# PeihaoChen/RSPNet

Measured on AMD Instinct MI355X. Metric: clips/sec pretext step (c3d 16x112x112, B=32/GPU), higher is better.
Workload: dtype f32

## Files before the change

include/rspnet_hip.h:

```cpp
#ifndef RSPNET_HIP_H
#define RSPNET_HIP_H

#include <stddef.h>
#include <stdint.h>

#ifdef __cplusplus
extern "C" {
#endif

#define RSP_OK 0
#define RSP_EINVAL (-1)
#define RSP_EWORKSPACE (-2)
#define RSP_ELAUNCH (-3)
#define RSP_EUNSUPPORTED (-4)

const char* rsp_strerror(int code);
const char* rsp_last_error(void);
const char* rsp_last_conv_kernel(void);
int rsp_version(void);

typedef struct rsp_conv3d_desc {
  int32_t N, Di, Hi, Wi, Cin;
  int32_t Do, Ho, Wo, Cout;
  int32_t kT, kH, kW;
  int32_t sT, sH, sW;
  int32_t pT, pH, pW;
  int32_t in_ld;
  int32_t out_ld;
} rsp_conv3d_desc;

size_t rsp_conv3d_packed_fwd_elems(const rsp_conv3d_desc* d);
int rsp_conv3d_pack_fwd(const rsp_conv3d_desc* d, const float* w_ref, float* w_packed, void* stream);

int32_t rsp_conv3d_stat_tiles(const rsp_conv3d_desc* d);
size_t rsp_conv3d_fwd_workspace(const rsp_conv3d_desc* d);
int rsp_conv3d_fwd(const rsp_conv3d_desc* d, const float* x, const float* w_packed, const float* bias, float* y,
                   float* stat_partials, void* workspace, size_t workspace_bytes, void* stream);

size_t rsp_conv3d_dgrad_workspace(const rsp_conv3d_desc* d);
int rsp_conv3d_dgrad(const rsp_conv3d_desc* d, const float* dy, const float* w_ref, float* dx, void* workspace,
                     size_t workspace_bytes, void* stream);

size_t rsp_conv3d_packed_dgrad_elems(const rsp_conv3d_desc* d);
int rsp_conv3d_dgrad_packed(const rsp_conv3d_desc* d, const float* dy, const float* w_packed, float* dx, void* workspace,
                            size_t workspace_bytes, void* stream);

typedef struct rsp_pack_job {
  const void* src;
  void* dst;
  int64_t total;
  int32_t kind, Cout_src, Cin_src, kT, kH, kW;
  int32_t transpose, O, C, Kld, nTd, nTh, nTw, k0d, k0h, k0w, kstepd, ksteph, kstepw, ntaps;
  int32_t blocks, reserved;
} rsp_pack_job;
int32_t rsp_conv3d_pack_jobs(const rsp_conv3d_desc* d, int32_t which, int32_t Cout_src, int32_t Cin_src, const float* w_ref,
                             float* w_packed, rsp_pack_job* jobs, int32_t max_jobs);
int rsp_pack_run(const rsp_pack_job* jobs_device, int32_t n_jobs, int32_t max_blocks, void* stream);
void rsp_conv3d_pack_forget(const void* w_packed);

size_t rsp_conv3d_wgrad_workspace(const rsp_conv3d_desc* d);
size_t rsp_conv3d_rowgeom_bytes(const rsp_conv3d_desc* d);
int rsp_conv3d_rowgeom(const rsp_conv3d_desc* d, void* table, void* stream);
int rsp_conv3d_wgrad(const rsp_conv3d_desc* d, const float* x, const float* dy, float* dw_ref, float* dbias, int32_t cout_valid,
                     int32_t cin_valid, const void* rowgeom_table, void* workspace, size_t workspace_bytes, void* stream);

const char* rsp_conv3d_kernel_name(const rsp_conv3d_desc* d, int which);

double rsp_conv3d_executed_fraction(const rsp_conv3d_desc* d, int which);

int rsp_conv3d_set_option(const char* name, int32_t value);

int rsp_fastdiv_check(int d, int n);

typedef struct rsp_bn_ema_job {
  float* running_mean;
  float* running_var;
  const float* batch_stats;
  int32_t C;
  float momentum;
} rsp_bn_ema_job;
size_t rsp_bn_finalize_workspace(int32_t tiles, int32_t C);
int rsp_bn_finalize(const float* stat_partials, int32_t tiles, int32_t C, int32_t c_valid, int32_t stat_ld, int64_t count,
                    const float* conv_bias, const float* gamma, const float* beta, float eps, float momentum, float* running_mean,
                    float* running_var, float* batch_stats_out, float* mean_invstd , float* scale_shift ,
                    void* workspace, size_t workspace_bytes, void* stream);
int rsp_bn_running_update(const rsp_bn_ema_job* jobs_device, int32_t n_jobs, int32_t max_c, void* stream);

typedef struct rsp_pool3d_desc {
  int32_t N, Di, Hi, Wi, C;
  int32_t Do, Ho, Wo;
  int32_t kT, kH, kW, sT, sH, sW, pT, pH, pW;
  int32_t in_ld, out_ld, res_ld;
} rsp_pool3d_desc;

int rsp_bn_act_pool_fwd(const rsp_pool3d_desc* d, const float* y, const float* scale_shift, const float* residual,
                        int relu, const float* gate, float* out, void* stream);

int rsp_bn_act_maxpool_applicable(const rsp_pool3d_desc* d);
int rsp_bn_act_maxpool_fwd(const rsp_pool3d_desc* d, const float* y, const float* scale_shift, int relu, const float* gate, float* out,
                           int32_t* argmax, void* stream);

size_t rsp_bn_bwd_workspace(const rsp_pool3d_desc* d);
int rsp_bn_act_pool_bwd(const rsp_pool3d_desc* d, const float* y, const float* residual, const float* dout,
                        const float* gamma, const float* mean_invstd, const float* scale_shift, int relu, float* dy,
                        float* dres, float* dgamma, float* dbeta, int32_t c_valid, const float* gate, const float* dmean,
                        void* workspace, size_t workspace_bytes, void* stream);

size_t rsp_bn_eval_bwd_workspace(const rsp_pool3d_desc* d);
int rsp_bn_eval_act_pool_bwd(const rsp_pool3d_desc* d, const float* y, const float* residual, const float* dout,
                             const float* mean_invstd, const float* scale_shift, int relu, float* dy, float* dres,
                             float* dgamma, float* dbeta, int32_t c_valid, void* workspace, size_t workspace_bytes,
                             void* stream);

int rsp_maxpool3d_fwd(const rsp_pool3d_desc* d, const float* x, float* out, int32_t* argmax, void* stream);
int rsp_maxpool3d_bwd(const rsp_pool3d_desc* d, const float* dout, const int32_t* argmax, float* dx, void* stream);

size_t rsp_gate_fwd_workspace(int32_t N, int32_t P, int32_t C);
int rsp_gate_fwd(const float* x, int32_t N, int32_t P, int32_t C, int32_t in_ld, const float* w, const float* b,
                 float* out, int32_t out_ld, float* mean, float* gate, void* workspace, size_t workspace_bytes,
                 void* stream);
int rsp_bn_gate_sums(const float* y, int32_t N, int32_t P, int32_t C, int32_t y_ld, const float* scale_shift, int relu,
                     float* act, int32_t act_ld, const float* w, const float* b, float* mean, float* gate, void* workspace,
                     size_t workspace_bytes, void* stream);
int rsp_gate_apply(const float* x, int32_t N, int32_t P, int32_t C, int32_t in_ld, const float* gate, float* out, int32_t out_ld,
                   void* stream);
int rsp_gate_bwd_params(const float* y, const float* scale_shift, int relu, const float* dout, int32_t N, int32_t P, int32_t C,
                        int32_t y_ld, int32_t dout_ld, const float* w, const float* mean, const float* gate, float* dw, float* db,
                        float* dmean, void* workspace, size_t workspace_bytes, void* stream);
size_t rsp_gate_bwd_workspace(int32_t N, int32_t P, int32_t C);
int rsp_gate_bwd(const float* x, const float* dout, int32_t N, int32_t P, int32_t C, int32_t x_ld, int32_t dout_ld,
                 const float* w, const float* mean, const float* gate, float* dx, int32_t dx_ld, float* dw, float* db,
                 void* workspace, size_t workspace_bytes, void* stream);

int rsp_head_fwd(const float* feat, int32_t B, int32_t P, int32_t C, int32_t feat_ld, const float* w1,
                 const float* b1, const float* w2, const float* b2, int32_t dim, float* out1, float* out2,
                 float* pooled, float* raw, void* stream);
size_t rsp_head_bwd_workspace(int32_t B, int32_t dim);
int rsp_head_bwd(const float* dout1, const float* dout2, const float* pooled, const float* raw, const float* w1,
                 const float* w2, int32_t B, int32_t P, int32_t C, int32_t feat_ld, int32_t dim, float* dw1,
                 float* db1, float* dw2, float* db2, float* dfeat, void* workspace, size_t workspace_bytes,
                 void* stream);

int rsp_spatial_mean_fwd(const float* x, int32_t N, int32_t P, int32_t C, int32_t ld, float* mean, void* stream);
int rsp_spatial_mean_bwd(const float* dmean, int32_t N, int32_t P, int32_t C, int32_t ld, float* dx, void* stream);
int rsp_linear_fwd(const float* x, int32_t B, int32_t Cin, const float* w, const float* bias, int32_t Cout, int relu,
                   float* y, void* stream);
size_t rsp_linear_bwd_workspace(int32_t B, int32_t Cout);
int rsp_linear_bwd(const float* x, const float* y, const float* dy, const float* w, int32_t B, int32_t Cin, int32_t Cout,
                   int relu, float* dx, float* dw, float* db, void* workspace, size_t workspace_bytes, void* stream);
int rsp_l2norm_fwd(const float* x, int32_t B, int32_t dim, float* y, void* stream);
int rsp_l2norm_bwd(const float* x, const float* dy, int32_t B, int32_t dim, float* dx, void* stream);

int rsp_logits_fwd(const float* qA, const float* qM, const float* kA, const float* kM, const float* knegA,
                   const float* knegM, const float* queue, int32_t B, int32_t dim, int32_t dim_m, int32_t K, float inv_T,
                   float* logits1, float* logits2, float* lposM, float* lnegM, void* stream);
size_t rsp_logits_bwd_workspace(int32_t B, int32_t dim, int32_t K);
int rsp_logits_bwd(const float* dlogits1, const float* dlogits2, const float* dlposM, const float* dlnegM,
                   const float* kA, const float* kM, const float* knegA, const float* knegM, const float* queue,
                   int32_t B, int32_t dim, int32_t dim_m, int32_t K, float inv_T, float* dqA, float* dqM, void* workspace,
                   size_t workspace_bytes, void* stream);

int rsp_loss_fwd_bwd(const float* logits1, const float* logits2, const float* lposM, const float* lnegM, int32_t B,
                     int32_t K1 , float margin, float A, float M, float* losses, float* dlogits1,
                     float* dlogits2, float* dlposM, float* dlnegM, float* row_scratch , void* stream);

int rsp_queue_enqueue(float* queue, int32_t dim, int32_t K, int32_t ptr, const float* keys, int32_t n, void* stream);
int rsp_queue_enqueue_dev(float* queue, int32_t dim, int32_t K, int64_t* ptr_dev, const float* keys, int32_t n, void* stream);

int rsp_clip_gather(const float* im, int32_t B_in, int32_t C, int32_t T_in, int32_t H, int32_t W, const int32_t* src,
                    const int32_t* step, int32_t B_out, int32_t T_out, int32_t C_out, float* out, void* stream);
int rsp_clip_gather_multi(int32_t n_jobs, const float* const* ims, const int32_t* const* srcs, const int32_t* const* steps,
                          float* const* outs, int32_t B_in, int32_t C, int32_t T_in, int32_t H, int32_t W, int32_t B_out, int32_t T_out,
                          int32_t C_out, void* stream);

int rsp_momentum_update(float* k, const float* q, int64_t n, float m, void* stream);

int rsp_sgd_step(float* p, const float* g, float* buf, int64_t n, float lr, float mu, float wd, float gscale,
                 int first, void* stream);

#define RSP_ELT_RELU_FWD 0
#define RSP_ELT_RELU_BWD 1
#define RSP_ELT_SIGMOID_FWD 2
#define RSP_ELT_SIGMOID_BWD 3
#define RSP_ELT_ADD 4
int rsp_eltwise(int32_t op, const float* a, const float* b , float* y, int64_t n, void* stream);

int rsp_rows_gather(const float* in, const int32_t* idx, int32_t n, int32_t width, float* out, void* stream);

#define RSP_AUG_BRIGHTNESS 0
#define RSP_AUG_CONTRAST 1
#define RSP_AUG_SATURATION 2
#define RSP_AUG_HUE 3
typedef struct rsp_augment_clip_desc {
  const uint8_t* src;
  int64_t frame_pitch;
  int32_t row_pitch;
  int32_t h, w;
  int32_t gray, flip;
  int32_t n_ops;
  int32_t op[4];
  float factor[4];
  float one_minus[4];
} rsp_augment_clip_desc;
size_t rsp_augment_workspace(int32_t n_clips, int32_t T, int32_t size);
int rsp_augment_batch(const rsp_augment_clip_desc* descs, int32_t n_clips, int32_t T, int32_t size, const float* mean3,
                      const float* std3, const float* blur9, float* out, int64_t out_clip_stride, void* workspace,
                      size_t workspace_bytes, void* stream);

int32_t rsp_cosine_topk_splits(int32_t Nq, int32_t Ng, int32_t splits);
size_t rsp_cosine_topk_workspace(int32_t Nq, int32_t Ng, int32_t D, int32_t k, int32_t splits);
int rsp_cosine_topk(const float* q, int32_t ldq, int32_t Nq, const float* g, int32_t ldg, int32_t Ng, int32_t D, int32_t k,
                    int32_t splits, int32_t* idx, float* dist, void* workspace, size_t workspace_bytes, void* stream);
int rsp_topk_hits(const int32_t* idx, int32_t Nq, int32_t k, const int64_t* y_q, const int64_t* y_g, int32_t Ng,
                  const int32_t* ks_host, int32_t nks, int32_t* counts, void* stream);

typedef struct rsp_cls_meters {
  float val[3];
  float sum[3];
  int32_t count[3];
} rsp_cls_meters;
size_t rsp_xent_metrics_workspace(int32_t rows, int32_t n_crop);
int rsp_xent_metrics(const float* logits, int32_t rows, int32_t classes, int32_t ld, int32_t n_crop, const int64_t* target,
                     int32_t valid, float* avg_logits, float* dlogits, float* loss, float* acc, rsp_cls_meters* meters,
                     void* workspace, size_t workspace_bytes, void* stream);

typedef struct rsp_pretext_meters {
  float val[8];
  float sum[8];
  int32_t count[8];
} rsp_pretext_meters;
size_t rsp_pretext_metrics_workspace(int32_t B);
int rsp_pretext_metrics(const float* logits1, const float* logits2, const float* lposM, const float* lnegM, int32_t B, int32_t K1,
                        const float* losses, float* acc, rsp_pretext_meters* meters, void* workspace, size_t workspace_bytes,
                        void* stream);

size_t rsp_cam_maps_workspace(int32_t B, int32_t C);
int rsp_cam_maps(const float* feat_q, int32_t ld_q, const float* feat_k, int32_t ld_k, const int32_t* k_row, int32_t B, int32_t P,
                 int32_t C, const float* w_qA, const float* w_qM, const float* w_kA, const float* w_kM, int32_t dim_A, int32_t dim_M,
                 float* out, void* workspace, size_t workspace_bytes, void* stream);
int rsp_cam_overlay(const float* maps, int32_t N, int32_t Tp, int32_t Hp, int32_t Wp, const float* clip_a, const float* clip_b,
                    int32_t B, int32_t T, int32_t t, int32_t size, uint8_t* out, void* stream);

#ifdef __cplusplus
}
#endif
#endif
```

rspnet_amd/_lib.py:

```python
from __future__ import annotations

import ctypes as C
import os
from typing import Optional

_HERE = os.path.dirname(os.path.abspath(__file__))
LIB_PATH = os.environ.get("RSPNET_HIP_LIB") or os.path.join(_HERE, "librspnet_hip.so")

c_f32p = C.c_void_p
c_i32p = C.c_void_p
c_stream = C.c_void_p


class ConvDesc(C.Structure):
    _fields_ = [(n, C.c_int32) for n in (
        "N", "Di", "Hi", "Wi", "Cin", "Do", "Ho", "Wo", "Cout", "kT", "kH", "kW", "sT", "sH", "sW",
        "pT", "pH", "pW", "in_ld", "out_ld")]


class PoolDesc(C.Structure):
    _fields_ = [(n, C.c_int32) for n in (
        "N", "Di", "Hi", "Wi", "C", "Do", "Ho", "Wo", "kT", "kH", "kW", "sT", "sH", "sW", "pT", "pH", "pW",
        "in_ld", "out_ld", "res_ld")]


class PackJob(C.Structure):
    _fields_ = [("src", C.c_void_p), ("dst", C.c_void_p), ("total", C.c_int64)] + [(n, C.c_int32) for n in (
        "kind", "Cout_src", "Cin_src", "kT", "kH", "kW", "transpose", "O", "C", "Kld", "nTd", "nTh", "nTw", "k0d", "k0h", "k0w",
        "kstepd", "ksteph", "kstepw", "ntaps", "blocks", "reserved")]


class BnEmaJob(C.Structure):
    _fields_ = [("running_mean", C.c_void_p), ("running_var", C.c_void_p), ("batch_stats", C.c_void_p), ("C", C.c_int32),
                ("momentum", C.c_float)]


class AugmentClipDesc(C.Structure):
    _fields_ = [("src", C.c_void_p), ("frame_pitch", C.c_int64), ("row_pitch", C.c_int32), ("h", C.c_int32), ("w", C.c_int32),
                ("gray", C.c_int32), ("flip", C.c_int32), ("n_ops", C.c_int32), ("op", C.c_int32 * 4),
                ("factor", C.c_float * 4), ("one_minus", C.c_float * 4)]


class ClsMeters(C.Structure):
    _fields_ = [("val", C.c_float * 3), ("sum", C.c_float * 3), ("count", C.c_int32 * 3)]


class PretextMeters(C.Structure):
    _fields_ = [("val", C.c_float * 8), ("sum", C.c_float * 8), ("count", C.c_int32 * 8)]


_PD = C.POINTER(ConvDesc)
_PP = C.POINTER(PoolDesc)
_sz = C.c_size_t
_i32 = C.c_int32
_i64 = C.c_int64
_f = C.c_float
_p = C.c_void_p

SIGNATURES = {
    "rsp_strerror": (C.c_char_p, [C.c_int]),
    "rsp_last_error": (C.c_char_p, []),
    "rsp_last_conv_kernel": (C.c_char_p, []),
    "rsp_version": (C.c_int, []),
    "rsp_conv3d_packed_fwd_elems": (_sz, [_PD]),
    "rsp_conv3d_pack_fwd": (C.c_int, [_PD, _p, _p, _p]),
    "rsp_conv3d_stat_tiles": (_i32, [_PD]),
    "rsp_conv3d_fwd_workspace": (_sz, [_PD]),
    "rsp_conv3d_fwd": (C.c_int, [_PD, _p, _p, _p, _p, _p, _p, _sz, _p]),
    "rsp_conv3d_dgrad_workspace": (_sz, [_PD]),
    "rsp_conv3d_dgrad": (C.c_int, [_PD, _p, _p, _p, _p, _sz, _p]),
    "rsp_conv3d_packed_dgrad_elems": (_sz, [_PD]),
    "rsp_conv3d_dgrad_packed": (C.c_int, [_PD, _p, _p, _p, _p, _sz, _p]),
    "rsp_conv3d_pack_jobs": (_i32, [_PD, _i32, _i32, _i32, _p, _p, _p, _i32]),
    "rsp_pack_run": (C.c_int, [_p, _i32, _i32, _p]),
    "rsp_conv3d_pack_forget": (None, [_p]),
    "rsp_conv3d_wgrad_workspace": (_sz, [_PD]),
    "rsp_conv3d_rowgeom_bytes": (_sz, [_PD]),
    "rsp_conv3d_rowgeom": (C.c_int, [_PD, _p, _p]),
    "rsp_conv3d_wgrad": (C.c_int, [_PD, _p, _p, _p, _p, _i32, _i32, _p, _p, _sz, _p]),
    "rsp_conv3d_kernel_name": (C.c_char_p, [_PD, C.c_int]),
    "rsp_conv3d_executed_fraction": (C.c_double, [_PD, C.c_int]),
    "rsp_conv3d_set_option": (C.c_int, [C.c_char_p, _i32]),
    "rsp_fastdiv_check": (C.c_int, [C.c_int, C.c_int]),
    "rsp_bn_finalize_workspace": (_sz, [_i32, _i32]),
    "rsp_bn_finalize": (C.c_int, [_p, _i32, _i32, _i32, _i32, _i64, _p, _p, _p, _f, _f, _p, _p, _p, _p, _p, _p, _sz, _p]),
    "rsp_bn_running_update": (C.c_int, [_p, _i32, _i32, _p]),
    "rsp_bn_act_pool_fwd": (C.c_int, [_PP, _p, _p, _p, C.c_int, _p, _p, _p]),
    "rsp_bn_act_maxpool_applicable": (C.c_int, [_PP]),
    "rsp_bn_act_maxpool_fwd": (C.c_int, [_PP, _p, _p, C.c_int, _p, _p, _p, _p]),
    "rsp_bn_bwd_workspace": (_sz, [_PP]),
    "rsp_bn_act_pool_bwd": (C.c_int, [_PP, _p, _p, _p, _p, _p, _p, C.c_int, _p, _p, _p, _p, _i32, _p, _p, _p, _sz, _p]),
    "rsp_bn_eval_bwd_workspace": (_sz, [_PP]),
    "rsp_bn_eval_act_pool_bwd": (C.c_int, [_PP, _p, _p, _p, _p, _p, C.c_int, _p, _p, _p, _p, _i32, _p, _sz, _p]),
    "rsp_maxpool3d_fwd": (C.c_int, [_PP, _p, _p, _p, _p]),
    "rsp_maxpool3d_bwd": (C.c_int, [_PP, _p, _p, _p, _p]),
    "rsp_gate_fwd_workspace": (_sz, [_i32, _i32, _i32]),
    "rsp_gate_fwd": (C.c_int, [_p, _i32, _i32, _i32, _i32, _p, _p, _p, _i32, _p, _p, _p, _sz, _p]),
    "rsp_bn_gate_sums": (C.c_int, [_p, _i32, _i32, _i32, _i32, _p, C.c_int, _p, _i32, _p, _p, _p, _p, _p, _sz, _p]),
    "rsp_gate_apply": (C.c_int, [_p, _i32, _i32, _i32, _i32, _p, _p, _i32, _p]),
    "rsp_gate_bwd_params": (C.c_int, [_p, _p, C.c_int, _p, _i32, _i32, _i32, _i32, _i32, _p, _p, _p, _p, _p, _p, _p, _sz, _p]),
    "rsp_gate_bwd_workspace": (_sz, [_i32, _i32, _i32]),
    "rsp_gate_bwd": (C.c_int, [_p, _p, _i32, _i32, _i32, _i32, _i32, _p, _p, _p, _p, _i32, _p, _p, _p, _sz, _p]),
    "rsp_head_fwd": (C.c_int, [_p, _i32, _i32, _i32, _i32, _p, _p, _p, _p, _i32, _p, _p, _p, _p, _p]),
    "rsp_head_bwd_workspace": (_sz, [_i32, _i32]),
    "rsp_head_bwd": (C.c_int, [_p, _p, _p, _p, _p, _p, _i32, _i32, _i32, _i32, _i32, _p, _p, _p, _p, _p, _p, _sz, _p]),
    "rsp_spatial_mean_fwd": (C.c_int, [_p, _i32, _i32, _i32, _i32, _p, _p]),
    "rsp_spatial_mean_bwd": (C.c_int, [_p, _i32, _i32, _i32, _i32, _p, _p]),
    "rsp_linear_fwd": (C.c_int, [_p, _i32, _i32, _p, _p, _i32, C.c_int, _p, _p]),
    "rsp_linear_bwd_workspace": (_sz, [_i32, _i32]),
    "rsp_linear_bwd": (C.c_int, [_p, _p, _p, _p, _i32, _i32, _i32, C.c_int, _p, _p, _p, _p, _sz, _p]),
    "rsp_l2norm_fwd": (C.c_int, [_p, _i32, _i32, _p, _p]),
    "rsp_l2norm_bwd": (C.c_int, [_p, _p, _i32, _i32, _p, _p]),
    "rsp_logits_fwd": (C.c_int, [_p, _p, _p, _p, _p, _p, _p, _i32, _i32, _i32, _i32, _f, _p, _p, _p, _p, _p]),
    "rsp_logits_bwd_workspace": (_sz, [_i32, _i32, _i32]),
    "rsp_logits_bwd": (C.c_int, [_p, _p, _p, _p, _p, _p, _p, _p, _p, _i32, _i32, _i32, _i32, _f, _p, _p, _p, _sz, _p]),
    "rsp_loss_fwd_bwd": (C.c_int, [_p, _p, _p, _p, _i32, _i32, _f, _f, _f, _p, _p, _p, _p, _p, _p, _p]),
    "rsp_queue_enqueue": (C.c_int, [_p, _i32, _i32, _i32, _p, _i32, _p]),
    "rsp_queue_enqueue_dev": (C.c_int, [_p, _i32, _i32, _p, _p, _i32, _p]),
    "rsp_clip_gather": (C.c_int, [_p, _i32, _i32, _i32, _i32, _i32, _p, _p, _i32, _i32, _i32, _p, _p]),
    "rsp_clip_gather_multi": (C.c_int, [_i32, _p, _p, _p, _p, _i32, _i32, _i32, _i32, _i32, _i32, _i32, _i32, _p]),
    "rsp_momentum_update": (C.c_int, [_p, _p, _i64, _f, _p]),
    "rsp_sgd_step": (C.c_int, [_p, _p, _p, _i64, _f, _f, _f, _f, C.c_int, _p]),
    "rsp_rows_gather": (C.c_int, [_p, _p, _i32, _i32, _p, _p]),
    "rsp_eltwise": (C.c_int, [_i32, _p, _p, _p, _i64, _p]),
    "rsp_augment_workspace": (_sz, [_i32, _i32, _i32]),
    "rsp_augment_batch": (C.c_int, [_p, _i32, _i32, _i32, C.POINTER(C.c_float), C.POINTER(C.c_float), C.POINTER(C.c_float), _p, _i64,
                                    _p, _sz, _p]),
    "rsp_cosine_topk_splits": (_i32, [_i32, _i32, _i32]),
    "rsp_cosine_topk_workspace": (_sz, [_i32, _i32, _i32, _i32, _i32]),
    "rsp_cosine_topk": (C.c_int, [_p, _i32, _i32, _p, _i32, _i32, _i32, _i32, _i32, _p, _p, _p, _sz, _p]),
    "rsp_topk_hits": (C.c_int, [_p, _i32, _i32, _p, _p, _i32, C.POINTER(C.c_int32), _i32, _p, _p]),
    "rsp_xent_metrics_workspace": (_sz, [_i32, _i32]),
    "rsp_xent_metrics": (C.c_int, [_p, _i32, _i32, _i32, _i32, _p, _i32, _p, _p, _p, _p, _p, _p, _sz, _p]),
    "rsp_pretext_metrics_workspace": (_sz, [_i32]),
    "rsp_pretext_metrics": (C.c_int, [_p, _p, _p, _p, _i32, _i32, _p, _p, _p, _p, _sz, _p]),
    "rsp_cam_maps_workspace": (_sz, [_i32, _i32]),
    "rsp_cam_maps": (C.c_int, [_p, _i32, _p, _i32, _p, _i32, _i32, _i32, _p, _p, _p, _p, _i32, _i32, _p, _p, _sz, _p]),
    "rsp_cam_overlay": (C.c_int, [_p, _i32, _i32, _i32, _i32, _p, _p, _i32, _i32, _i32, _i32, _p, _p]),
}

_lib: Optional[C.CDLL] = None


class RspError(RuntimeError):
    pass


def load(init_gpu: bool = False) -> C.CDLL:
    global _lib
    if init_gpu:
        _init_gpu()
    if _lib is not None:
        return _lib
    if not os.path.exists(LIB_PATH):
        raise RspError(
            f"{LIB_PATH} not found: build it with rspnet_amd/csrc/build.sh (or __graft_entry__.build()). "
            "rspnet_amd has no CPU or eager fallback.")
    try:
        import torch
    except ImportError:
        pass
    lib = C.CDLL(LIB_PATH)
    for name, (res, args) in SIGNATURES.items():
        fn = getattr(lib, name)
        fn.restype = res
        fn.argtypes = args
    _lib = lib
    return lib


_gpu_ready = False


def _init_gpu():
    global _gpu_ready
    if _gpu_ready:
        return
    import torch
    if torch.cuda.is_available():
        torch.cuda.init()
        _gpu_ready = True


def check(rc: int, what: str):
    if rc != 0:
        lib = load()
        raise RspError(f"{what} failed: {lib.rsp_strerror(rc).decode()} ({lib.rsp_last_error().decode()})")


def source_hash() -> str:
    import glob
    import hashlib
    here = os.path.dirname(os.path.abspath(__file__))
    files = sorted(glob.glob(os.path.join(here, "csrc", "*.hip")) + glob.glob(os.path.join(here, "csrc", "*.h"))
                   + glob.glob(os.path.join(os.path.dirname(here), "include", "*.h")))
    h = hashlib.sha256()
    for f in files:
        h.update(os.path.basename(f).encode())
        with open(f, "rb") as fh:
            h.update(fh.read())
    return h.hexdigest()
```

rspnet_amd/csrc/bn_pool.hip:

```cpp
#include "common.h"

namespace {

__global__ __launch_bounds__(256) void bn_finalize_stage1(const float* __restrict__ part, int tiles, int C, int ld, int S,
                                                          double* __restrict__ out) {
  __shared__ double red[4][64][2];
  const int c = blockIdx.x * 64 + (threadIdx.x & 63);
  const int rl = threadIdx.x >> 6;
  const int per = (tiles + S - 1) / S;
  const int t0 = blockIdx.y * per, t1 = min(tiles, t0 + per);
  double s = 0.0, ss = 0.0;
  if (c < C)
    for (int t = t0 + rl; t < t1; t += 4) {
      const float2 v = *reinterpret_cast<const float2*>(part + ((long long)t * ld + c) * 2);
      s += (double)v.x;
      ss += (double)v.y;
    }
  red[rl][threadIdx.x & 63][0] = s;
  red[rl][threadIdx.x & 63][1] = ss;
  __syncthreads();
  if (rl == 0 && c < C) {
    const int l = threadIdx.x;
    out[((long long)blockIdx.y * C + c) * 2 + 0] = red[0][l][0] + red[1][l][0] + red[2][l][0] + red[3][l][0];
    out[((long long)blockIdx.y * C + c) * 2 + 1] = red[0][l][1] + red[1][l][1] + red[2][l][1] + red[3][l][1];
  }
}

__global__ __launch_bounds__(1024) void bn_finalize_stage2(const double* __restrict__ part, int S, int C, int Cv, long long count,
                                                           const float* __restrict__ conv_bias, const float* __restrict__ gamma,
                                                           const float* __restrict__ beta, float eps, float momentum,
                                                           float* __restrict__ running_mean, float* __restrict__ running_var,
                                                           float* __restrict__ mean_invstd, float* __restrict__ scale_shift,
                                                           float* __restrict__ bstat) {
  __shared__ double red[16][64][2];
  const int cl = threadIdx.x & 63, rl = threadIdx.x >> 6;
  const int c = blockIdx.x * 64 + cl;
  double s = 0.0, ss = 0.0;
  if (c < C)
    for (int i = rl; i < S; i += 16) {
      s += part[((long long)i * C + c) * 2 + 0];
      ss += part[((long long)i * C + c) * 2 + 1];
    }
  red[rl][cl][0] = s;
  red[rl][cl][1] = ss;
  __syncthreads();
  if (rl != 0 || c >= C) return;
  s = 0.0;
  ss = 0.0;
#pragma unroll
  for (int i = 0; i < 16; ++i) {
    s += red[i][cl][0];
    ss += red[i][cl][1];
  }
  const double n = (double)count;
  const double mean0 = s / n;
  double var = ss / n - mean0 * mean0;
  var = var > 0.0 ? var : 0.0;
  const bool valid = c < Cv;
  const double mean = mean0 + ((conv_bias && valid) ? (double)conv_bias[c] : 0.0);
  const float invstd = (float)(1.0 / sqrt(var + (double)eps));
  mean_invstd[c] = (float)mean;
  mean_invstd[C + c] = invstd;
  const float g = valid ? (gamma ? gamma[c] : 1.f) : 0.f, b = (valid && beta) ? beta[c] : 0.f;
  const float sc = g * invstd;
  scale_shift[c] = sc;
  scale_shift[C + c] = b - (float)mean * sc;
  if (!valid) return;
  const double unbiased = count > 1 ? var * n / (n - 1.0) : var;
  if (bstat) {
    bstat[c] = (float)mean;
    bstat[Cv + c] = (float)unbiased;
    return;
  }
  if (running_mean) running_mean[c] = (1.f - momentum) * running_mean[c] + momentum * (float)mean;
  if (running_var) running_var[c] = (1.f - momentum) * running_var[c] + momentum * (float)unbiased;
}

constexpr int FIN_CH = 16, FIN_LANES = 1024 / FIN_CH;

__device__ __forceinline__ bool fin_sum_partials(const float* __restrict__ part, int n, int C, int ld, double& s, double& ss) {
  __shared__ double red[FIN_LANES][FIN_CH][2];
  const int cl = threadIdx.x & (FIN_CH - 1), rl = threadIdx.x / FIN_CH;
  const int c = blockIdx.x * FIN_CH + cl;
  s = 0.0;
  ss = 0.0;
  if (c < C)
    for (int t = rl; t < n; t += FIN_LANES) {
      const float2 v = *reinterpret_cast<const float2*>(part + ((long long)t * ld + c) * 2);
      s += (double)v.x;
      ss += (double)v.y;
    }
  red[rl][cl][0] = s;
  red[rl][cl][1] = ss;
  __syncthreads();
  if (rl < 8) {
    s = 0.0;
    ss = 0.0;
#pragma unroll
    for (int i = 0; i < FIN_LANES / 8; ++i) {
      s += red[rl * (FIN_LANES / 8) + i][cl][0];
      ss += red[rl * (FIN_LANES / 8) + i][cl][1];
    }
  }
  __syncthreads();
  if (rl < 8) {
    red[rl][cl][0] = s;
    red[rl][cl][1] = ss;
  }
  __syncthreads();
  if (rl != 0 || c >= C) return false;
  s = 0.0;
  ss = 0.0;
#pragma unroll
  for (int i = 0; i < 8; ++i) {
    s += red[i][cl][0];
    ss += red[i][cl][1];
  }
  return true;
}

__global__ __launch_bounds__(1024) void bn_finalize_one_kernel(const float* __restrict__ part, int tiles, int C, int Cv, int ld, long long count,
                                                               const float* __restrict__ conv_bias, const float* __restrict__ gamma,
                                                               const float* __restrict__ beta, float eps, float momentum,
                                                               float* __restrict__ running_mean, float* __restrict__ running_var,
                                                               float* __restrict__ mean_invstd, float* __restrict__ scale_shift,
                                                               float* __restrict__ bstat) {
  const int c = blockIdx.x * FIN_CH + (threadIdx.x & (FIN_CH - 1));
  double s, ss;
  if (!fin_sum_partials(part, tiles, C, ld, s, ss)) return;
  const double n = (double)count;
  const double mean0 = s / n;
  double var = ss / n - mean0 * mean0;
  var = var > 0.0 ? var : 0.0;
  const bool valid = c < Cv;
  const double mean = mean0 + ((conv_bias && valid) ? (double)conv_bias[c] : 0.0);
  const float invstd = (float)(1.0 / sqrt(var + (double)eps));
  mean_invstd[c] = (float)mean;
  mean_invstd[C + c] = invstd;
  const float g = valid ? (gamma ? gamma[c] : 1.f) : 0.f, b = (valid && beta) ? beta[c] : 0.f;
  const float sc = g * invstd;
  scale_shift[c] = sc;
  scale_shift[C + c] = b - (float)mean * sc;
  if (!valid) return;
  const double unbiased = count > 1 ? var * n / (n - 1.0) : var;
  if (bstat) {
    bstat[c] = (float)mean;
    bstat[Cv + c] = (float)unbiased;
    return;
  }
  if (running_mean) running_mean[c] = (1.f - momentum) * running_mean[c] + momentum * (float)mean;
  if (running_var) running_var[c] = (1.f - momentum) * running_var[c] + momentum * (float)unbiased;
}

// ... 335 lines not shown
#pragma unroll
          for (int e = 0; e < VEC; ++e) { best[e] = -INFINITY; by[e] = 0.f; }
#pragma unroll
          for (int w = 0; w < NW; ++w)
#pragma unroll
            for (int e = 0; e < VEC; ++e) {
              float z = fmaf(yv[w][e], sc[e], sh[e]);
              if (p.res) z += r[w][e];
              const float zz = p.relu ? fmaxf(z, 0.f) : z;
              if (zz > best[e]) { best[e] = zz; by[e] = yv[w][e]; }
            }
#pragma unroll
          for (int e = 0; e < VEC; ++e) {
            const float dz = (p.relu && !(best[e] > 0.f)) ? 0.f : g[e];
            s1[e] += dz;
            s2[e] = fmaf(dz, (by[e] - mean[e]) * invstd[e], s2[e]);
          }
        }
      }
      op_end = 0;
    }
    for (; op < op_end; op += stride) {
      const int q1 = fastdiv((int)op, p.dWo), ow = (int)op - q1 * d.Wo;
      const int q2 = fastdiv(q1, p.dHo), oh = q1 - q2 * d.Ho;
      const int n = fastdiv(q2, p.dDo), od = q2 - n * d.Do;
      float best[VEC], by[VEC];
#pragma unroll
      for (int e = 0; e < VEC; ++e) { best[e] = -INFINITY; by[e] = 0.f; }
      for (int kt = 0; kt < d.kT; ++kt) {
        const int id = od * d.sT - d.pT + kt;
        if ((unsigned)id >= (unsigned)d.Di) continue;
        for (int kh = 0; kh < d.kH; ++kh) {
          const int ih = oh * d.sH - d.pH + kh;
          if ((unsigned)ih >= (unsigned)d.Hi) continue;
          for (int kw = 0; kw < d.kW; ++kw) {
            const int iw = ow * d.sW - d.pW + kw;
            if ((unsigned)iw >= (unsigned)d.Wi) continue;
            const long long pos = (((long long)n * d.Di + id) * d.Hi + ih) * d.Wi + iw;
            float yv[VEC], z[VEC];
            zval<VEC>(p, pos, c, sc, sh, yv, z);
#pragma unroll
            for (int e = 0; e < VEC; ++e) {
              const float zz = p.relu ? fmaxf(z[e], 0.f) : z[e];
              if (zz > best[e]) { best[e] = zz; by[e] = yv[e]; }
            }
          }
        }
      }
      float g[VEC];
      load_vec<VEC>(p.dout + op * d.out_ld + c, g);
      if (p.gate) gated_grad<VEC>(p, n, c, g);
#pragma unroll
      for (int e = 0; e < VEC; ++e) {
        const float dz = (p.relu && !(best[e] > 0.f)) ? 0.f : g[e];
        s1[e] += dz;
        s2[e] = fmaf(dz, (by[e] - mean[e]) * invstd[e], s2[e]);
      }
    }
  }
#pragma unroll
  for (int e = 0; e < VEC; ++e) { red[t][e] = s1[e]; red[t][VEC + e] = s2[e]; }
  __syncthreads();
  if (t < cgc) {
    float a1[VEC], a2[VEC];
#pragma unroll
    for (int e = 0; e < VEC; ++e) a1[e] = a2[e] = 0.f;
    for (int l = 0; l < ppi; ++l)
#pragma unroll
      for (int e = 0; e < VEC; ++e) { a1[e] += red[l * cgc + t][e]; a2[e] += red[l * cgc + t][VEC + e]; }
    float* o = p.partial + ((long long)blockIdx.x * d.C + (cg0 + t) * VEC) * 2;
#pragma unroll
    for (int e = 0; e < VEC; ++e) { o[2 * e] = a1[e]; o[2 * e + 1] = a2[e]; }
  }
}

__global__ __launch_bounds__(1024) void bn_bwd_finalize_kernel(const float* __restrict__ partial, int nblocks, int C, int Cv,
                                                               double* __restrict__ sums, float* __restrict__ dgamma,
                                                               float* __restrict__ dbeta) {
  const int c = blockIdx.x * FIN_CH + (threadIdx.x & (FIN_CH - 1));
  double a, b;
  if (!fin_sum_partials(partial, nblocks, C, C, a, b)) return;
  sums[2 * c] = a;
  sums[2 * c + 1] = b;
  if (dbeta && c < Cv) dbeta[c] = (float)a;
  if (dgamma && c < Cv) dgamma[c] = (float)b;
}

template <int VEC>
__global__ __launch_bounds__(256) void bn_bwd_apply_kernel(const BwdParams p) {
  const rsp_pool3d_desc& d = p.d;
  const long long total = (long long)d.N * d.Di * d.Hi * d.Wi * p.cg;
  const double invn = 1.0 / (double)p.count;
  for (long long idx = blockIdx.x * 256ll + threadIdx.x; idx < total; idx += 256ll * gridDim.x) {
    const int cgi = (int)(idx % p.cg);
    long long q = idx / p.cg;
    const long long pos = q;
    const int iw = (int)(q % d.Wi); q /= d.Wi;
    const int ih = (int)(q % d.Hi); q /= d.Hi;
    const int id = (int)(q % d.Di);
    const int n = (int)(q / d.Di);
    const int c = cgi * VEC;
    float sc[VEC], sh[VEC], mean[VEC], invstd[VEC], gam[VEC];
    load_vec<VEC>(p.ss + c, sc);
    load_vec<VEC>(p.ss + d.C + c, sh);
    load_vec<VEC>(p.mi + c, mean);
    load_vec<VEC>(p.mi + d.C + c, invstd);
    load_gamma<VEC>(p, c, gam);
    float yv[VEC], z[VEC], dz[VEC];
    zval<VEC>(p, pos, c, sc, sh, yv, z);
#pragma unroll
    for (int e = 0; e < VEC; ++e) dz[e] = 0.f;
    const int od = id / d.sT, oh = ih / d.sH, ow = iw / d.sW;
    if (od < d.Do && oh < d.Ho && ow < d.Wo) {
      bool win[VEC];
      float mine[VEC];
#pragma unroll
      for (int e = 0; e < VEC; ++e) { mine[e] = p.relu ? fmaxf(z[e], 0.f) : z[e]; win[e] = true; }
      const int my = ((id - od * d.sT) * d.kH + (ih - oh * d.sH)) * d.kW + (iw - ow * d.sW);
      if (d.kT * d.kH * d.kW > 1) {
        for (int kt = 0; kt < d.kT; ++kt)
          for (int kh = 0; kh < d.kH; ++kh)
            for (int kw = 0; kw < d.kW; ++kw) {
              const int o = (kt * d.kH + kh) * d.kW + kw;
              if (o == my) continue;
              const long long pp = (((long long)n * d.Di + od * d.sT + kt) * d.Hi + oh * d.sH + kh) * d.Wi + ow * d.sW + kw;
              float y2[VEC], z2[VEC];
              zval<VEC>(p, pp, c, sc, sh, y2, z2);
#pragma unroll
              for (int e = 0; e < VEC; ++e) {
                const float v = p.relu ? fmaxf(z2[e], 0.f) : z2[e];
                if (o < my ? (v >= mine[e]) : (v > mine[e])) win[e] = false;
              }
            }
      }
      const long long op = (((long long)n * d.Do + od) * d.Ho + oh) * d.Wo + ow;
      float g[VEC];
      load_vec<VEC>(p.dout + op * d.out_ld + c, g);
#pragma unroll
      for (int e = 0; e < VEC; ++e) dz[e] = (win[e] && !(p.relu && !(mine[e] > 0.f))) ? g[e] : 0.f;
    }
    float o[VEC];
#pragma unroll
    for (int e = 0; e < VEC; ++e) {
      const float m1 = (float)(p.sums[2 * (c + e)] * invn);
      const float m2 = (float)(p.sums[2 * (c + e) + 1] * invn);
      const float xhat = (yv[e] - mean[e]) * invstd[e];
      o[e] = gam[e] * invstd[e] * (dz[e] - m1 - xhat * m2);
    }
    store_vec<VEC>(p.dy + pos * d.in_ld + c, o);
    if (p.dres) store_vec<VEC>(p.dres + pos * d.res_ld + c, dz);
  }
}

template <int VEC, int MODE>
__global__ __launch_bounds__(256) void bn_bwd_apply_win_kernel(const BwdParams p) {
  const rsp_pool3d_desc& d = p.d;
  const int t = threadIdx.x;
  const int pl = fastdiv(t, p.dcgc);
  const int cgi = blockIdx.y * 256 + (t - pl * p.cgc);
  if (pl >= p.ppi || cgi >= p.cg) return;
  const int c = cgi * VEC;
  const int nwin = d.kT * d.kH * d.kW;
  float sc[VEC], sh[VEC], mean[VEC], invstd[VEC], gam[VEC], m1[VEC], m2[VEC];
  load_vec<VEC>(p.ss + c, sc);
  load_vec<VEC>(p.ss + d.C + c, sh);
  load_vec<VEC>(p.mi + c, mean);
  load_vec<VEC>(p.mi + d.C + c, invstd);
  load_gamma<VEC>(p, c, gam);
  const double invn = 1.0 / (double)p.count;
#pragma unroll
  for (int e = 0; e < VEC; ++e) {
    m1[e] = (float)(p.sums[2 * (c + e)] * invn);
    m2[e] = (float)(p.sums[2 * (c + e) + 1] * invn);
  }
  long long o = (long long)blockIdx.x * p.ppi + pl;
  long long stride = (long long)gridDim.x * p.ppi;
  long long o_end = p.npos;
  if constexpr (MODE == 1) {
    const long long step = p.ppi;
    stride *= 4;
    o = (long long)blockIdx.x * p.ppi * 4 + pl;
    for (; o + 3 * step < p.npos; o += stride) {
      float yv[4][VEC], r[4][VEC], g[4][VEC];
#pragma unroll
      for (int u = 0; u < 4; ++u) {
        load_vec<VEC>(p.y + (o + u * step) * d.in_ld + c, yv[u]);
        if (p.res) load_vec<VEC>(p.res + (o + u * step) * d.res_ld + c, r[u]);
        load_vec<VEC>(p.dout + (o + u * step) * d.out_ld + c, g[u]);
      }
#pragma unroll
      for (int u = 0; u < 4; ++u) {
        float ov[VEC], dz[VEC];
#pragma unroll
        for (int e = 0; e < VEC; ++e) {
          float z = fmaf(yv[u][e], sc[e], sh[e]);
          if (p.res) z += r[u][e];
          dz[e] = (p.relu && !(z > 0.f)) ? 0.f : g[u][e];
          const float xhat = (yv[u][e] - mean[e]) * invstd[e];
          ov[e] = gam[e] * invstd[e] * (dz[e] - m1[e] - xhat * m2[e]);
        }
        store_vec<VEC>(p.dy + (o + u * step) * d.in_ld + c, ov);
        if (p.dres) store_vec<VEC>(p.dres + (o + u * step) * d.res_ld + c, dz);
      }
    }
    stride = step;
    o_end = min(p.npos, o + 4 * step);
  }
  if constexpr (MODE == 2 || MODE == 3) {
    {
      constexpr int NW = MODE == 2 ? 4 : 8;
      long long off[NW];
      window_offsets<NW>(d, off);
      for (; o < o_end; o += stride) {
        const int op = (int)o;
        const int q1 = fastdiv(op, p.dWo), ow = op - q1 * d.Wo;
        const int q2 = fastdiv(q1, p.dHo), oh = q1 - q2 * d.Ho;
        const int n = fastdiv(q2, p.dDo), od = q2 - n * d.Do;
        const long long base = (((long long)n * d.Di + od * d.sT) * d.Hi + oh * d.sH) * d.Wi + ow * d.sW;
        float yv[NW][VEC], r[NW][VEC], g[VEC], best[VEC];
        int bi[VEC];
#pragma unroll
        for (int w = 0; w < NW; ++w) {
          load_vec<VEC>(p.y + (base + off[w]) * d.in_ld + c, yv[w]);
          if (p.res) load_vec<VEC>(p.res + (base + off[w]) * d.res_ld + c, r[w]);
        }
        load_vec<VEC>(p.dout + o * d.out_ld + c, g);
#pragma unroll
        for (int e = 0; e < VEC; ++e) { best[e] = -INFINITY; bi[e] = 0; }
#pragma unroll
        for (int w = 0; w < NW; ++w)
#pragma unroll
          for (int e = 0; e < VEC; ++e) {
            float z = fmaf(yv[w][e], sc[e], sh[e]);
            if (p.res) z += r[w][e];
            const float v = p.relu ? fmaxf(z, 0.f) : z;
            if (v > best[e]) { best[e] = v; bi[e] = w; }
          }
#pragma unroll
        for (int w = 0; w < NW; ++w) {
          float ov[VEC], dz[VEC];
#pragma unroll
          for (int e = 0; e < VEC; ++e) {
            dz[e] = (bi[e] == w && !(p.relu && !(best[e] > 0.f))) ? g[e] : 0.f;
            const float xhat = (yv[w][e] - mean[e]) * invstd[e];
            ov[e] = gam[e] * invstd[e] * (dz[e] - m1[e] - xhat * m2[e]);
          }
          store_vec<VEC>(p.dy + (base + off[w]) * d.in_ld + c, ov);
          if (p.dres) store_vec<VEC>(p.dres + (base + off[w]) * d.res_ld + c, dz);
        }
      }
    }
    return;
  }
  for (; o < o_end; o += stride) {
    float g[VEC];
    load_vec<VEC>(p.dout + o * d.out_ld + c, g);
    if (MODE == 1 || nwin == 1) {
      if (p.gate) gated_grad<VEC>(p, fastdiv(fastdiv(fastdiv((int)o, p.dWo), p.dHo), p.dDo), c, g);
      float yv[VEC], z[VEC], ov[VEC], dz[VEC];
      zval<VEC>(p, o, c, sc, sh, yv, z);
#pragma unroll
      for (int e = 0; e < VEC; ++e) {
        dz[e] = (p.relu && !(z[e] > 0.f)) ? 0.f : g[e];
        const float xhat = (yv[e] - mean[e]) * invstd[e];
        ov[e] = gam[e] * invstd[e] * (dz[e] - m1[e] - xhat * m2[e]);
      }
      store_vec<VEC>(p.dy + o * d.in_ld + c, ov);
      if (p.dres) store_vec<VEC>(p.dres + o * d.res_ld + c, dz);
      continue;
    }
    const int op = (int)o;
    const int q1 = fastdiv(op, p.dWo), ow = op - q1 * d.Wo;
    const int q2 = fastdiv(q1, p.dHo), oh = q1 - q2 * d.Ho;
    const int n = fastdiv(q2, p.dDo), od = q2 - n * d.Do;
    const long long base = (((long long)n * d.Di + od * d.sT) * d.Hi + oh * d.sH) * d.Wi + ow * d.sW;
    float yv[8][VEC], zv[8][VEC], best[VEC];
    int bi[VEC];
#pragma unroll
    for (int e = 0; e < VEC; ++e) { best[e] = -INFINITY; bi[e] = 0; }
    int kw = 0, kh = 0, kt = 0;
#pragma unroll
    for (int wdx = 0; wdx < 8; ++wdx) {
      if (wdx < nwin) {
        const long long pos = base + ((long long)kt * d.Hi + kh) * d.Wi + kw;
        zval<VEC>(p, pos, c, sc, sh, yv[wdx], zv[wdx]);
#pragma unroll
        for (int e = 0; e < VEC; ++e) {
          const float v = p.relu ? fmaxf(zv[wdx][e], 0.f) : zv[wdx][e];
          if (v > best[e]) { best[e] = v; bi[e] = wdx; }
        }
        if (++kw == d.kW) { kw = 0; if (++kh == d.kH) { kh = 0; ++kt; } }
      }
    }
    kw = 0; kh = 0; kt = 0;
#pragma unroll
    for (int wdx = 0; wdx < 8; ++wdx) {
      if (wdx < nwin) {
        const long long pos = base + ((long long)kt * d.Hi + kh) * d.Wi + kw;
        float ov[VEC], dz[VEC];
#pragma unroll
        for (int e = 0; e < VEC; ++e) {
          dz[e] = (bi[e] == wdx && !(p.relu && !(best[e] > 0.f))) ? g[e] : 0.f;
          const float xhat = (yv[wdx][e] - mean[e]) * invstd[e];
          ov[e] = gam[e] * invstd[e] * (dz[e] - m1[e] - xhat * m2[e]);
        }
        store_vec<VEC>(p.dy + pos * d.in_ld + c, ov);
        if (p.dres) store_vec<VEC>(p.dres + pos * d.res_ld + c, dz);
        if (++kw == d.kW) { kw = 0; if (++kh == d.kH) { kh = 0; ++kt; } }
      }
    }
  }
}

struct EvalBwdParams {
  rsp_pool3d_desc d;
  const float* __restrict__ y;
  const float* __restrict__ res;
  const float* __restrict__ dout;
  const float* __restrict__ mi;
  const float* __restrict__ ss;
  float* __restrict__ partial;
  float* __restrict__ dy;
  float* __restrict__ dres;
  int relu;
  int cg;
  int Cv;
  int cgc, ppi;
  long long npos;
  int De, He, We;
  FastDiv dcgc, dW, dH, dD;
};

template <int VEC, int MODE, bool SUMS>
__global__ __launch_bounds__(256) void bn_eval_bwd_kernel(const EvalBwdParams p) {
  const rsp_pool3d_desc& d = p.d;
  const int cg0 = blockIdx.y * 256;
  const int cgc = min(p.cg - cg0, 256);
  const int t = threadIdx.x;
  const int pl = fastdiv(t, p.dcgc);
  const int cl = t - pl * p.cgc;
  const bool active = pl < p.ppi && cl < cgc;
  const int c = (cg0 + cl) * VEC;
  float s1[VEC], s2[VEC];
#pragma unroll
  for (int e = 0; e < VEC; ++e) s1[e] = s2[e] = 0.f;
  if (active) {
    float sc[VEC], sh[VEC], scd[VEC], mean[VEC], invstd[VEC];
    load_vec<VEC>(p.ss + c, sc);
    load_vec<VEC>(p.ss + d.C + c, sh);
#pragma unroll
    for (int e = 0; e < VEC; ++e) { scd[e] = c + e < p.Cv ? sc[e] : 0.f; mean[e] = 0.f; invstd[e] = 0.f; }
    if constexpr (SUMS) {
      load_vec<VEC>(p.mi + c, mean);
      load_vec<VEC>(p.mi + d.C + c, invstd);
    }
    long long o = (long long)blockIdx.x * p.ppi + pl;
    const long long stride = (long long)gridDim.x * p.ppi;
    if constexpr (MODE == 1) {
      const long long step = p.ppi;
      o = (long long)blockIdx.x * p.ppi * 4 + pl;
      for (; o + 3 * step < p.npos; o += stride * 4) {
        float yv[4][VEC], r[4][VEC], g[4][VEC];
#pragma unroll
        for (int u = 0; u < 4; ++u) {
          load_vec<VEC>(p.y + (o + u * step) * d.in_ld + c, yv[u]);
          if (p.res) load_vec<VEC>(p.res + (o + u * step) * d.res_ld + c, r[u]);
          load_vec<VEC>(p.dout + (o + u * step) * d.out_ld + c, g[u]);
        }
#pragma unroll
        for (int u = 0; u < 4; ++u) {
          float ov[VEC], dz[VEC];
#pragma unroll
          for (int e = 0; e < VEC; ++e) {
            float z = fmaf(yv[u][e], sc[e], sh[e]);
            if (p.res) z += r[u][e];
            dz[e] = (p.relu && !(z > 0.f)) ? 0.f : g[u][e];
            ov[e] = scd[e] * dz[e];
            if constexpr (SUMS) {
              s1[e] += dz[e];
              s2[e] = fmaf(dz[e], (yv[u][e] - mean[e]) * invstd[e], s2[e]);
            }
          }
          store_vec<VEC>(p.dy + (o + u * step) * d.in_ld + c, ov);
          if (p.dres) store_vec<VEC>(p.dres + (o + u * step) * d.res_ld + c, dz);
        }
      }
      for (int u = 0; u < 4 && o < p.npos; ++u, o += step) {
        float yv[VEC], z[VEC], g[VEC], ov[VEC], dz[VEC];
        load_vec<VEC>(p.y + o * d.in_ld + c, yv);
        if (p.res) load_vec<VEC>(p.res + o * d.res_ld + c, z);
        load_vec<VEC>(p.dout + o * d.out_ld + c, g);
#pragma unroll
        for (int e = 0; e < VEC; ++e) {
          const float zz = fmaf(yv[e], sc[e], sh[e]) + (p.res ? z[e] : 0.f);
          dz[e] = (p.relu && !(zz > 0.f)) ? 0.f : g[e];
          ov[e] = scd[e] * dz[e];
          if constexpr (SUMS) {
            s1[e] += dz[e];
            s2[e] = fmaf(dz[e], (yv[e] - mean[e]) * invstd[e], s2[e]);
          }
        }
        store_vec<VEC>(p.dy + o * d.in_ld + c, ov);
        if (p.dres) store_vec<VEC>(p.dres + o * d.res_ld + c, dz);
      }
    } else if constexpr (MODE == 2 || MODE == 3) {
      constexpr int NW = MODE == 2 ? 4 : 8;
      long long off[NW];
      window_offsets<NW>(d, off);
      for (; o < p.npos; o += stride) {
        const int op = (int)o;
        const int q1 = fastdiv(op, p.dW), ow = op - q1 * d.Wo;
        const int q2 = fastdiv(q1, p.dH), oh = q1 - q2 * d.Ho;
        const int n = fastdiv(q2, p.dD), od = q2 - n * d.Do;
        const long long base = (((long long)n * d.Di + od * d.sT) * d.Hi + oh * d.sH) * d.Wi + ow * d.sW;
        float yv[NW][VEC], r[NW][VEC], g[VEC], best[VEC], by[VEC];
        int bi[VEC];
#pragma unroll
        for (int w = 0; w < NW; ++w) {
          load_vec<VEC>(p.y + (base + off[w]) * d.in_ld + c, yv[w]);
          if (p.res) load_vec<VEC>(p.res + (base + off[w]) * d.res_ld + c, r[w]);
        }
        load_vec<VEC>(p.dout + o * d.out_ld + c, g);
#pragma unroll
        for (int e = 0; e < VEC; ++e) { best[e] = -INFINITY; bi[e] = 0; by[e] = 0.f; }
#pragma unroll
        for (int w = 0; w < NW; ++w)
#pragma unroll
          for (int e = 0; e < VEC; ++e) {
            float z = fmaf(yv[w][e], sc[e], sh[e]);
            if (p.res) z += r[w][e];
            const float v = p.relu ? fmaxf(z, 0.f) : z;
            if (v > best[e]) { best[e] = v; bi[e] = w; by[e] = yv[w][e]; }
          }
        float dzo[VEC];
#pragma unroll
        for (int e = 0; e < VEC; ++e) {
          dzo[e] = (p.relu && !(best[e] > 0.f)) ? 0.f : g[e];
          if constexpr (SUMS) {
            s1[e] += dzo[e];
            s2[e] = fmaf(dzo[e], (by[e] - mean[e]) * invstd[e], s2[e]);
          }
        }
#pragma unroll
        for (int w = 0; w < NW; ++w) {
          float ov[VEC], dz[VEC];
#pragma unroll
          for (int e = 0; e < VEC; ++e) {
            dz[e] = bi[e] == w ? dzo[e] : 0.f;
            ov[e] = scd[e] * dz[e];
          }
          store_vec<VEC>(p.dy + (base + off[w]) * d.in_ld + c, ov);
          if (p.dres) store_vec<VEC>(p.dres + (base + off[w]) * d.res_ld + c, dz);
        }
      }
    } else {
      for (; o < p.npos; o += stride) {
        const int op = (int)o;
        const int q1 = fastdiv(op, p.dW), ow = op - q1 * p.We;
        const int q2 = fastdiv(q1, p.dH), oh = q1 - q2 * p.He;
        const int n = fastdiv(q2, p.dD), od = q2 - n * p.De;
        const bool whole = od < d.Do && oh < d.Ho && ow < d.Wo;
        const int t0 = od * d.sT, h0 = oh * d.sH, w0 = ow * d.sW;
        const int nt = min(d.kT, d.Di - t0), nh = min(d.kH, d.Hi - h0), nw = min(d.kW, d.Wi - w0);
        float best[VEC], by[VEC], dzo[VEC];
// ... 52 lines not shown
    __syncthreads();
    if (t < cgc) {
      float a1[VEC], a2[VEC];
#pragma unroll
      for (int e = 0; e < VEC; ++e) a1[e] = a2[e] = 0.f;
      for (int l = 0; l < p.ppi; ++l)
#pragma unroll
        for (int e = 0; e < VEC; ++e) { a1[e] += red[l * p.cgc + t][e]; a2[e] += red[l * p.cgc + t][VEC + e]; }
      float* o = p.partial + ((long long)blockIdx.x * d.C + (cg0 + t) * VEC) * 2;
#pragma unroll
      for (int e = 0; e < VEC; ++e) { o[2 * e] = a1[e]; o[2 * e + 1] = a2[e]; }
    }
  }
}

__global__ __launch_bounds__(1024) void bn_eval_bwd_finalize_kernel(const float* __restrict__ partial, int nblocks, int C, int Cv,
                                                                    float* __restrict__ dgamma, float* __restrict__ dbeta) {
  const int c = blockIdx.x * FIN_CH + (threadIdx.x & (FIN_CH - 1));
  double a, b;
  if (!fin_sum_partials(partial, nblocks, C, C, a, b)) return;
  if (dbeta && c < Cv) dbeta[c] = (float)a;
  if (dgamma && c < Cv) dgamma[c] = (float)b;
}

constexpr int EVAL_BWD_MAX_BLOCKS = 4096;

bool pool_ok(const rsp_pool3d_desc* d, bool need_disjoint) {
  if (!d) return false;
  if (d->N <= 0 || d->C <= 0 || d->kT <= 0 || d->kH <= 0 || d->kW <= 0) return false;
  if (d->sT <= 0 || d->sH <= 0 || d->sW <= 0 || d->pT < 0 || d->pH < 0 || d->pW < 0) return false;
  if (d->Do != (d->Di + 2 * d->pT - d->kT) / d->sT + 1) return false;
  if (d->Ho != (d->Hi + 2 * d->pH - d->kH) / d->sH + 1) return false;
  if (d->Wo != (d->Wi + 2 * d->pW - d->kW) / d->sW + 1) return false;
  if (d->in_ld < d->C || d->out_ld < d->C) return false;
  if (need_disjoint) {
    if (d->kT != d->sT || d->kH != d->sH || d->kW != d->sW || d->pT || d->pH || d->pW) return false;
  }
  return true;
}

int bn_mode(const rsp_pool3d_desc* d, bool gated) {
  const int nwin = d->kT * d->kH * d->kW;
  const bool unit = nwin == 1 && d->sT == 1 && d->sH == 1 && d->sW == 1 && !(d->pT | d->pH | d->pW);
  if (unit) return gated ? 0 : 1;
  const bool tile = d->kT == d->sT && d->kH == d->sH && d->kW == d->sW && !(d->pT | d->pH | d->pW);
  return tile && nwin == 4 ? 2 : (tile && nwin == 8 ? 3 : 0);
}

#define RSP_BN_LAUNCH_V(K, V, mode, grid, stream, p)                                                   \
  do {                                                                                                 \
    switch (mode) {                                                                                    \
      case 1: hipLaunchKernelGGL((K<V, 1>), grid, dim3(256), 0, stream, p); break;                     \
      case 2: hipLaunchKernelGGL((K<V, 2>), grid, dim3(256), 0, stream, p); break;                     \
      case 3: hipLaunchKernelGGL((K<V, 3>), grid, dim3(256), 0, stream, p); break;                     \
      default: hipLaunchKernelGGL((K<V, 0>), grid, dim3(256), 0, stream, p); break;                    \
    }                                                                                                  \
  } while (0)
#define RSP_BN_LAUNCH(K, vec, mode, grid, stream, p)                                                   \
  do {                                                                                                 \
    if (vec) RSP_BN_LAUNCH_V(K, 4, mode, grid, stream, p);                                             \
    else RSP_BN_LAUNCH_V(K, 1, mode, grid, stream, p);                                                 \
  } while (0)

int grid_for(long long total) {
  long long b = (total + 255) / 256;
  return (int)(b > 8192 ? 8192 : (b < 1 ? 1 : b));
}

int reduce_blocks(const rsp_pool3d_desc* d, int cg) {
  const int cgc = cg < 256 ? cg : 256;
  const int ppi = 256 / cgc;
  const long long npos = (long long)d->N * d->Do * d->Ho * d->Wo;
  long long b = (npos + (long long)ppi * 8 - 1) / ((long long)ppi * 8);
  return (int)(b > 2048 ? 2048 : (b < 1 ? 1 : b));
}

}

extern "C" {

static int finalize_slices(int tiles) { return tiles >= 8192 ? 256 : (tiles >= 4096 ? 64 : (tiles >= 64 ? 16 : 1)); }

size_t rsp_bn_finalize_workspace(int32_t tiles, int32_t C) {
  const int S = finalize_slices(tiles);
  return (size_t)S * C * 2 * sizeof(double);
}

__global__ __launch_bounds__(256) void bn_ema_kernel(const rsp_bn_ema_job* __restrict__ jobs) {
  const rsp_bn_ema_job j = jobs[blockIdx.y];
  const int c = blockIdx.x * 256 + threadIdx.x;
  if (c >= j.C) return;
  j.running_mean[c] = (1.f - j.momentum) * j.running_mean[c] + j.momentum * j.batch_stats[c];
  j.running_var[c] = (1.f - j.momentum) * j.running_var[c] + j.momentum * j.batch_stats[j.C + c];
}

int rsp_bn_running_update(const rsp_bn_ema_job* jobs_device, int32_t n_jobs, int32_t max_c, void* stream) {
  RSP_REQUIRE(jobs_device && n_jobs > 0 && n_jobs <= 65535 && max_c > 0, "rsp_bn_running_update: bad argument");
  hipLaunchKernelGGL(bn_ema_kernel, dim3(rsp_cdiv(max_c, 256), n_jobs), dim3(256), 0, (hipStream_t)stream, jobs_device);
  return rsp_check_launch("bn_ema_kernel");
}

int rsp_bn_finalize(const float* stat_partials, int32_t tiles, int32_t C, int32_t c_valid, int32_t stat_ld, int64_t count,
                    const float* conv_bias, const float* gamma, const float* beta, float eps, float momentum, float* running_mean,
                    float* running_var, float* batch_stats_out, float* mean_invstd, float* scale_shift, void* workspace,
                    size_t workspace_bytes, void* stream) {
  RSP_REQUIRE(stat_partials && mean_invstd && scale_shift && workspace, "rsp_bn_finalize: null pointer");
  RSP_REQUIRE(tiles > 0 && C > 0 && count > 0 && stat_ld >= C && c_valid > 0 && c_valid <= C, "rsp_bn_finalize: bad size");
  const int S = finalize_slices(tiles);
  if (workspace_bytes < (size_t)S * C * 2 * sizeof(double)) {
    rsp_set_error("rsp_bn_finalize: workspace too small");
    return RSP_EWORKSPACE;
  }
  hipStream_t s = (hipStream_t)stream;
  if (tiles <= 2048) {
    hipLaunchKernelGGL(bn_finalize_one_kernel, dim3(rsp_cdiv(C, FIN_CH)), dim3(1024), 0, s, stat_partials, tiles, C, c_valid, stat_ld, (long long)count,
                       conv_bias, gamma, beta, eps, momentum, running_mean, running_var, mean_invstd, scale_shift, batch_stats_out);
    return rsp_check_launch("bn_finalize_one_kernel");
  }
  double* part = reinterpret_cast<double*>(workspace);
  hipLaunchKernelGGL(bn_finalize_stage1, dim3(rsp_cdiv(C, 64), S), dim3(256), 0, s, stat_partials, tiles, C, stat_ld, S, part);
  int rc = rsp_check_launch("bn_finalize_stage1");
  if (rc != RSP_OK) return rc;
  hipLaunchKernelGGL(bn_finalize_stage2, dim3(rsp_cdiv(C, 64)), dim3(1024), 0, s, part, S, C, c_valid, (long long)count, conv_bias,
                     gamma, beta, eps, momentum, running_mean, running_var, mean_invstd, scale_shift, batch_stats_out);
  return rsp_check_launch("bn_finalize_stage2");
}

int rsp_bn_act_pool_fwd(const rsp_pool3d_desc* d, const float* y, const float* scale_shift, const float* residual,
                        int relu, const float* gate, float* out, void* stream) {
  RSP_REQUIRE(pool_ok(d, false), "rsp_bn_act_pool_fwd: bad descriptor");
  RSP_REQUIRE(y && scale_shift && out, "rsp_bn_act_pool_fwd: null pointer");
  if (!residual && (d->kT != d->sT || d->kH != d->sH || d->kW != d->sW || d->pT || d->pH || d->pW) &&
      rsp_bn_act_maxpool_applicable(d) && rsp_aligned16(y) && rsp_aligned16(out) && rsp_aligned16(scale_shift) &&
      (!gate || rsp_aligned16(gate)))
    return rsp_bn_act_maxpool_fwd(d, y, scale_shift, relu, gate, out, nullptr, stream);
  PoolParams p;
  p.d = *d; p.y = y; p.ss = scale_shift; p.res = residual; p.gate = gate; p.out = out; p.relu = relu;
  const bool vec = d->C % 4 == 0 && d->in_ld % 4 == 0 && d->out_ld % 4 == 0 && rsp_aligned16(y) && rsp_aligned16(out) &&
                   rsp_aligned16(scale_shift) && (!residual || (d->res_ld % 4 == 0 && rsp_aligned16(residual))) &&
                   (!gate || rsp_aligned16(gate));
  p.cg = vec ? d->C / 4 : d->C;
  const Layout L = make_layout(d, p.cg, 4);
  RSP_REQUIRE(L.npos < (1ll << 31), "rsp_bn_act_pool_fwd: more than 2^31 - 1 output positions");
  set_layout(p, L);
  RSP_BN_LAUNCH(bn_act_pool_fwd_kernel, vec, bn_mode(d, gate != nullptr), L.grid, (hipStream_t)stream, p);
  return rsp_check_launch("bn_act_pool_fwd_kernel");
}

size_t rsp_bn_bwd_workspace(const rsp_pool3d_desc* d) {
  if (!pool_ok(d, true)) return 0;
  return rsp_align_up((size_t)2048 * d->C * 2 * sizeof(float), 256) + (size_t)d->C * 2 * sizeof(double);
}

int rsp_bn_act_pool_bwd(const rsp_pool3d_desc* d, const float* y, const float* residual, const float* dout,
                        const float* gamma, const float* mean_invstd, const float* scale_shift, int relu, float* dy,
                        float* dres, float* dgamma, float* dbeta, int32_t c_valid, const float* gate, const float* dmean,
                        void* workspace, size_t workspace_bytes, void* stream) {
  RSP_REQUIRE(pool_ok(d, true), "rsp_bn_act_pool_bwd: needs disjoint windows (kernel == stride, no padding)");
  RSP_REQUIRE(!gate || (dmean && d->kT * d->kH * d->kW == 1 && d->sT * d->sH * d->sW == 1 && !residual),
              "rsp_bn_act_pool_bwd: a gated unit has a unit window, no residual, and needs dmean");
  RSP_REQUIRE(c_valid > 0 && c_valid <= d->C, "rsp_bn_act_pool_bwd: bad valid channel count");
  RSP_REQUIRE(y && dout && mean_invstd && scale_shift && dy && workspace, "rsp_bn_act_pool_bwd: null pointer");
  if (workspace_bytes < rsp_bn_bwd_workspace(d)) {
    rsp_set_error("rsp_bn_act_pool_bwd: workspace too small");
    return RSP_EWORKSPACE;
  }
  hipStream_t s = (hipStream_t)stream;
  BwdParams p;
  memset(&p, 0, sizeof p);
  p.d = *d; p.y = y; p.res = residual; p.dout = dout; p.gamma = gamma; p.mi = mean_invstd; p.ss = scale_shift;
  p.dy = dy; p.dres = dres; p.relu = relu;
  p.Cv = c_valid;
  p.gate = gate; p.dmean = dmean;
  p.invP = 1.f / (float)((long long)d->Di * d->Hi * d->Wi);
  p.count = (long long)d->N * d->Di * d->Hi * d->Wi;
  const bool vec = d->C % 4 == 0 && d->in_ld % 4 == 0 && d->out_ld % 4 == 0 && rsp_aligned16(y) && rsp_aligned16(dout) &&
                   rsp_aligned16(dy) && rsp_aligned16(scale_shift) && rsp_aligned16(mean_invstd) &&
                   (!gamma || c_valid != d->C || rsp_aligned16(gamma)) &&
                   (!residual || (d->res_ld % 4 == 0 && rsp_aligned16(residual) && (!dres || rsp_aligned16(dres)))) &&
                   (!gate || (rsp_aligned16(gate) && rsp_aligned16(dmean)));
  p.cg = vec ? d->C / 4 : d->C;
  p.partial = reinterpret_cast<float*>(workspace);
  double* sums = reinterpret_cast<double*>(reinterpret_cast<unsigned char*>(workspace) +
                                           rsp_align_up((size_t)2048 * d->C * 2 * sizeof(float), 256));
  p.sums = sums;
  const Layout L = make_layout(d, p.cg, 4);
  RSP_REQUIRE(L.npos < (1ll << 31), "rsp_bn_act_pool_bwd: more than 2^31 - 1 output positions");
  set_layout(p, L);
  p.nblocks = reduce_blocks(d, p.cg);
  dim3 rgrid(p.nblocks, rsp_cdiv(p.cg, 256));
  const int mode = bn_mode(d, gate != nullptr);
  RSP_BN_LAUNCH(bn_bwd_reduce_kernel, vec, mode, rgrid, s, p);
  int rc = rsp_check_launch("bn_bwd_reduce_kernel");
  if (rc != RSP_OK) return rc;
  hipLaunchKernelGGL(bn_bwd_finalize_kernel, dim3(rsp_cdiv(d->C, FIN_CH)), dim3(1024), 0, s, p.partial, p.nblocks, d->C, c_valid, sums,
                     dgamma, dbeta);
  rc = rsp_check_launch("bn_bwd_finalize_kernel");
  if (rc != RSP_OK) return rc;
  const bool exact = d->Di % d->sT == 0 && d->Hi % d->sH == 0 && d->Wi % d->sW == 0 && d->kT * d->kH * d->kW <= 8;
  if (exact) {
    RSP_BN_LAUNCH(bn_bwd_apply_win_kernel, vec, mode, L.grid, s, p);
    return rsp_check_launch("bn_bwd_apply_win_kernel");
  }
  const long long total = (long long)d->N * d->Di * d->Hi * d->Wi * p.cg;
  if (vec) hipLaunchKernelGGL(bn_bwd_apply_kernel<4>, dim3(grid_for(total)), dim3(256), 0, s, p);
  else hipLaunchKernelGGL(bn_bwd_apply_kernel<1>, dim3(grid_for(total)), dim3(256), 0, s, p);
  return rsp_check_launch("bn_bwd_apply_kernel");
}

static int eval_bwd_mode(const rsp_pool3d_desc* d) {
  const int m = bn_mode(d, false);
  if (m == 1) return 1;
  const bool exact = d->Di % d->sT == 0 && d->Hi % d->sH == 0 && d->Wi % d->sW == 0;
  return exact ? m : 0;
}

static long long eval_bwd_npos(const rsp_pool3d_desc* d, int mode) {
  if (mode != 0) return (long long)d->N * d->Do * d->Ho * d->Wo;
  return (long long)d->N * rsp_cdiv(d->Di, d->sT) * rsp_cdiv(d->Hi, d->sH) * rsp_cdiv(d->Wi, d->sW);
}

size_t rsp_bn_eval_bwd_workspace(const rsp_pool3d_desc* d) {
  if (!pool_ok(d, true)) return 0;
  const long long npos = eval_bwd_npos(d, eval_bwd_mode(d));
  const long long rows = npos < EVAL_BWD_MAX_BLOCKS ? npos : EVAL_BWD_MAX_BLOCKS;
  return (size_t)rows * d->C * 2 * sizeof(float);
}

#define RSP_BN_EVAL_LAUNCH_S(V, M, grid, stream, p)                                                                       \
  do {                                                                                                                    \
    if (sums) hipLaunchKernelGGL((bn_eval_bwd_kernel<V, M, true>), grid, dim3(256), 0, stream, p);                        \
    else hipLaunchKernelGGL((bn_eval_bwd_kernel<V, M, false>), grid, dim3(256), 0, stream, p);                            \
  } while (0)
#define RSP_BN_EVAL_LAUNCH_V(V, mode, grid, stream, p)                                                                    \
  do {                                                                                                                    \
    switch (mode) {                                                                                                       \
      case 1: RSP_BN_EVAL_LAUNCH_S(V, 1, grid, stream, p); break;                                                         \
      case 2: RSP_BN_EVAL_LAUNCH_S(V, 2, grid, stream, p); break;                                                         \
      case 3: RSP_BN_EVAL_LAUNCH_S(V, 3, grid, stream, p); break;                                                         \
      default: RSP_BN_EVAL_LAUNCH_S(V, 0, grid, stream, p); break;                                                        \
    }                                                                                                                     \
  } while (0)

int rsp_bn_eval_act_pool_bwd(const rsp_pool3d_desc* d, const float* y, const float* residual, const float* dout,
                             const float* mean_invstd, const float* scale_shift, int relu, float* dy, float* dres,
                             float* dgamma, float* dbeta, int32_t c_valid, void* workspace, size_t workspace_bytes,
                             void* stream) {
  RSP_REQUIRE(pool_ok(d, true), "rsp_bn_eval_act_pool_bwd: needs disjoint windows (kernel == stride, no padding)");
  RSP_REQUIRE(c_valid > 0 && c_valid <= d->C, "rsp_bn_eval_act_pool_bwd: bad valid channel count");
  RSP_REQUIRE(y && dout && scale_shift && dy, "rsp_bn_eval_act_pool_bwd: null pointer");
  RSP_REQUIRE(!dres || residual, "rsp_bn_eval_act_pool_bwd: dres without a residual");
  RSP_REQUIRE(d->res_ld >= d->C || !residual, "rsp_bn_eval_act_pool_bwd: bad residual pitch");
  const bool sums = dgamma || dbeta;
  RSP_REQUIRE(!sums || (mean_invstd && workspace), "rsp_bn_eval_act_pool_bwd: parameter gradients need mean_invstd and a workspace");
  if (sums && workspace_bytes < rsp_bn_eval_bwd_workspace(d)) {
    rsp_set_error("rsp_bn_eval_act_pool_bwd: workspace too small");
    return RSP_EWORKSPACE;
  }
  hipStream_t s = (hipStream_t)stream;
  EvalBwdParams p;
  memset(&p, 0, sizeof p);
  p.d = *d; p.y = y; p.res = residual; p.dout = dout; p.mi = mean_invstd; p.ss = scale_shift;
  p.partial = sums ? reinterpret_cast<float*>(workspace) : nullptr;
  p.dy = dy; p.dres = dres; p.relu = relu; p.Cv = c_valid;
  const bool vec = d->C % 4 == 0 && d->in_ld % 4 == 0 && d->out_ld % 4 == 0 && rsp_aligned16(y) && rsp_aligned16(dout) &&
                   rsp_aligned16(dy) && rsp_aligned16(scale_shift) && (!sums || rsp_aligned16(mean_invstd)) &&
                   (!residual || (d->res_ld % 4 == 0 && rsp_aligned16(residual) && (!dres || rsp_aligned16(dres))));
  p.cg = vec ? d->C / 4 : d->C;
  const int mode = eval_bwd_mode(d);
  p.npos = eval_bwd_npos(d, mode);
  RSP_REQUIRE(p.npos < (1ll << 31), "rsp_bn_eval_act_pool_bwd: more than 2^31 - 1 positions");
  p.cgc = p.cg < 256 ? p.cg : 256;
  p.ppi = 256 / p.cgc;
  p.dcgc = fastdiv_make(p.cgc);
  p.De = rsp_cdiv(d->Di, d->sT); p.He = rsp_cdiv(d->Hi, d->sH); p.We = rsp_cdiv(d->Wi, d->sW);
  if (mode == 0) { p.dW = fastdiv_make(p.We); p.dH = fastdiv_make(p.He); p.dD = fastdiv_make(p.De); }
  else { p.dW = fastdiv_make(d->Wo); p.dH = fastdiv_make(d->Ho); p.dD = fastdiv_make(d->Do); }
  long long b = (p.npos + (long long)p.ppi * 16 - 1) / ((long long)p.ppi * 16);
  b = b > EVAL_BWD_MAX_BLOCKS ? EVAL_BWD_MAX_BLOCKS : (b < 1 ? 1 : b);
  const dim3 grid((unsigned)b, (unsigned)rsp_cdiv(p.cg, 256));
  if (vec) RSP_BN_EVAL_LAUNCH_V(4, mode, grid, s, p);
  else RSP_BN_EVAL_LAUNCH_V(1, mode, grid, s, p);
  int rc = rsp_check_launch("bn_eval_bwd_kernel");
  if (rc != RSP_OK || !sums) return rc;
  hipLaunchKernelGGL(bn_eval_bwd_finalize_kernel, dim3(rsp_cdiv(d->C, FIN_CH)), dim3(1024), 0, s, p.partial, (int)b, d->C, c_valid,
                     dgamma, dbeta);
  return rsp_check_launch("bn_eval_bwd_finalize_kernel");
}

}
```

rspnet_amd/csrc/common.h:

```cpp
#pragma once
#include <hip/hip_runtime.h>
#include <stdint.h>
#include <stdio.h>
#include <stdlib.h>
#include <string.h>
#include <tuple>

#include "rspnet_hip.h"

typedef float floatx16 __attribute__((ext_vector_type(16)));
typedef float floatx4 __attribute__((ext_vector_type(4)));

#define RSP_WAVE 64

void rsp_set_error(const char* msg);
void rsp_note_reset(void);
void rsp_note_kernel(const char* fmt, ...);

static inline int rsp_check_launch(const char* what) {
  hipError_t e = hipGetLastError();
  if (e != hipSuccess) {
    char buf[256];
    snprintf(buf, sizeof buf, "%.*s: %s", (int)strcspn(what, "<"), what, hipGetErrorString(e));
    rsp_set_error(buf);
    return RSP_ELAUNCH;
  }
  return RSP_OK;
}

#define RSP_CONV_OPTIONS(X)                                                             \
  X(OPT_NARROW_MAX_TILES, "narrow_max_tiles", "RSP_NARROW_MAX_TILES", 0, 512)           \
  X(OPT_NARROW32_MAX_UNITS, "narrow32_max_units", "RSP_NARROW32_MAX_UNITS", 0, 256)     \
  X(OPT_TALL_MIN_TILES, "tall_min_tiles", "RSP_TALL_MIN_TILES", 0, 0)                   \
  X(OPT_TWO_LEVEL_MIN_CHUNKS, "two_level_min_chunks", "RSP_TWO_LEVEL_MIN_CHUNKS", 0, 0) \
  X(OPT_DIRECT_MAX_TILES, "direct_max_tiles", "RSP_DIRECT_MAX_TILES", 0, 0)             \
  X(OPT_NO_PERSIST, "no_persist", "RSP_NO_PERSIST", 1, 0)                               \
  X(OPT_NO_HALF_BLOCK, "no_half_block", "RSP_NO_HALF_BLOCK", 1, 0)                      \
  X(OPT_NO_PAD_SKIP, "no_pad_skip", "RSP_NO_PAD_SKIP", 1, 0)                            \
  X(OPT_NO_DMAJOR, "no_dmajor", "RSP_NO_DMAJOR", 1, 0)                                  \
  X(OPT_NO_TM_SKIP, "no_tm_skip", "RSP_NO_TM_SKIP", 1, 0)                               \
  X(OPT_NO_MULTI_SPLIT, "no_multi_split", "RSP_NO_MULTI_SPLIT", 1, 0)
#define RSP_OPTION_ID(id, name, env, flag, dflt) id,
enum RspConvOption { RSP_CONV_OPTIONS(RSP_OPTION_ID) RSP_OPT_COUNT };
#undef RSP_OPTION_ID
int rsp_conv_option(RspConvOption id);

template <auto KERNEL, class... Args, class... Note>
int rsp_launch_lds(dim3 grid, size_t lds, size_t lds_max, hipStream_t s, const std::tuple<Args...>& args, const char* fmt, Note... note) {
  static bool attr_set = false;
  if (!attr_set) {
    (void)hipFuncSetAttribute(reinterpret_cast<const void*>(KERNEL), hipFuncAttributeMaxDynamicSharedMemorySize, (int)lds_max);
    attr_set = true;
  }
  rsp_note_kernel(fmt, note...);
  std::apply([&](const auto&... a) { hipLaunchKernelGGL(KERNEL, grid, dim3(256), lds, s, a...); }, args);
  return rsp_check_launch(fmt);
}

#define RSP_REQUIRE(cond, msg)     \
  do {                             \
    if (!(cond)) {                 \
      rsp_set_error(msg);          \
      return RSP_EINVAL;           \
    }                              \
  } while (0)

static inline size_t rsp_align_up(size_t v, size_t a) { return (v + a - 1) / a * a; }
static inline int rsp_cdiv(int64_t a, int64_t b) { return (int)((a + b - 1) / b); }
static inline bool rsp_aligned16(const void* p) { return (((uintptr_t)p) & 15) == 0; }

__device__ __forceinline__ int rsp_xcd_remap(int bid, int nwg) {
  const int q = nwg >> 3, r = nwg & 7;
  const int xcd = bid & 7;
  const int base = xcd < r ? xcd * (q + 1) : r * (q + 1) + (xcd - r) * q;
  return base + (bid >> 3);
}

__device__ __forceinline__ float rsp_wave_sum(float v) {
#pragma unroll
  for (int o = 32; o > 0; o >>= 1) v += __shfl_xor(v, o);
  return v;
}
__device__ __forceinline__ double rsp_wave_sum_d(double v) {
#pragma unroll
  for (int o = 32; o > 0; o >>= 1) v += __shfl_xor(v, o);
  return v;
}
__device__ __forceinline__ float rsp_wave_max(float v) {
#pragma unroll
  for (int o = 32; o > 0; o >>= 1) v = fmaxf(v, __shfl_xor(v, o));
  return v;
}

struct FastDiv {
  unsigned mul;
  unsigned shr;
  int d;
};

static inline FastDiv fastdiv_make(int d) {
  FastDiv f = {0u, 0u, d};
  if (d <= 1) return f;
  int s = 0;
  while ((1ll << s) < d) ++s;
  const unsigned long long pw = 1ull << (31 + s);
  f.mul = (unsigned)((pw + (unsigned long long)d - 1) / (unsigned long long)d);
  f.shr = (unsigned)(s - 1);
  return f;
}

__device__ __forceinline__ int fastdiv(int n, const FastDiv f) {
  return f.mul ? (int)(__umulhi((unsigned)n, f.mul) >> f.shr) : n;
}
```

rspnet_amd/csrc/conv_stem.h:

```cpp
#pragma once
#include "common.h"

bool rsp_conv_desc_ok(const rsp_conv3d_desc* d);
bool rsp_stem_applicable(const rsp_conv3d_desc* d);
int rsp_stem_tiles(const rsp_conv3d_desc* d);
size_t rsp_stem_packed_elems(const rsp_conv3d_desc* d);
int rsp_stem_pack(const rsp_conv3d_desc* d, const float* w_ref, float* w_packed, hipStream_t s);
int rsp_stem_fwd(const rsp_conv3d_desc* d, const float* x, const float* w_packed, const float* bias, float* y,
                 float* stat_partials, hipStream_t s);
const char* rsp_stem_kernel_name(const rsp_conv3d_desc* d);
void rsp_stem_note_packed(const void* w_packed, bool three_channels);
void rsp_stem_forget_packed(const void* w_packed);
const char* rsp_wgrad_kernel_name(const rsp_conv3d_desc* d);
double rsp_wgrad_executed_fraction(const rsp_conv3d_desc* d);
```

rspnet_amd/csrc/conv_wgrad.hip:

```cpp
#include "common.h"
#include "conv_stem.h"

namespace {

constexpr int RK = 32;
constexpr int MAX_TAPS = 343;

__device__ __attribute__((aligned(64))) float g_wzero[16];

struct WgradParams {
  const float* __restrict__ x;
  const float* __restrict__ dy;
  float* __restrict__ partial;
  int M, Gd, Gh, Gw;
  int Di, Hi, Wi, in_ld, Cin;
  int sD, sH, sW;
  int kT, kH, kW, pT, pH, pW;
  int dy_ld, Cout;
  int K, Kld;
  int rows_per_split, splitm;
  int co_tiles, k_tiles;
  const float* __restrict__ zero;
  unsigned x_bytes, dy_bytes;
  const uint2* __restrict__ rowgeom;
// ... 386 lines not shown
  const int r16 = lane & 15, g16 = lane >> 4;

  const int nchunk = (row_end - row_begin + RK - 1) / RK;
  const int khw = p.kH * p.kW;
  const int kt_lo = (k0 / p.Cin) / khw, kt_hi = ((min(k0 + BN, p.K) - 1) / p.Cin) / khw;
  auto frame_live = [&](int q) {
    const int g = q - fastdiv(q, p.dGd) * p.Gd;
    const int lo = g * p.sD - p.pT + kt_lo, hi = g * p.sD - p.pT + kt_hi;
    return hi >= 0 && lo < p.Di;
  };
  auto next_live = [&](int c) {
    if (!p.skip_pad) return c < nchunk ? c : nchunk;
    for (; c < nchunk; ++c) {
      const int r0 = row_begin + c * RK, r1 = min(r0 + RK, row_end) - 1;
      const int q0 = fastdiv(r0, p.dP), q1 = fastdiv(r1, p.dP);
      if (q1 - q0 > 1 || frame_live(q0) || frame_live(q1)) break;
    }
    return c;
  };
  int buf = 0;
  auto chunk = [&](int slot_next, int slot_fetch, int c_fetch, int c_issue, bool more, auto beside) {
    if (more) read_rowtab(slot_next);
    const float* a = At + buf * RK * BM + wm * WM + TM * l32;
    const float* b = Bt + buf * RK * BN + wn * WN + TN * l32;
    typename FragVec<TM>::type af[RK / 2];
    typename FragVec<TN>::type bf[RK / 2];
    float a16[RK / 4], b16[2][RK / 4];
    if (H16) {
      const float* ah = At + buf * RK * BM + r16;
      const float* bh = Bt + buf * RK * BN + wn * WN + r16;
#pragma unroll
      for (int s4 = 0; s4 < RK / 4; ++s4) {
        a16[s4] = ah[(4 * s4 + g16) * BM];
        b16[0][s4] = bh[(4 * s4 + g16) * BN];
        b16[1][s4] = bh[(4 * s4 + g16) * BN + 16];
      }
    } else {
#pragma unroll
      for (int s2 = 0; s2 < RK / 2; ++s2) {
        af[s2] = *reinterpret_cast<const typename FragVec<TM>::type*>(a + (2 * s2 + h) * BM);
        bf[s2] = *reinterpret_cast<const typename FragVec<TN>::type*>(b + (2 * s2 + h) * BN);
      }
    }
    fetch_rows(c_fetch, slot_fetch);
    if (more) issue(c_issue, buf ^ 1);
    beside();
    if (H16) {
#pragma unroll
      for (int s4 = 0; s4 < RK / 4; ++s4)
#pragma unroll
        for (int j = 0; j < 2; ++j) acc16[j] = __builtin_amdgcn_mfma_f32_16x16x4f32(a16[s4], b16[j][s4], acc16[j], 0, 0, 0);
    } else {
#pragma unroll
      for (int s2 = 0; s2 < RK / 2; ++s2)
#pragma unroll
        for (int i = 0; i < TM; ++i)
#pragma unroll
          for (int j = 0; j < TN; ++j)
            acc[i][j] = __builtin_amdgcn_mfma_f32_32x32x2f32(FragVec<TM>::get(af[s2], i), FragVec<TN>::get(bf[s2], j), acc[i][j], 0, 0, 0);
    }
    __builtin_amdgcn_sched_barrier(0);
    __syncthreads();
    buf ^= 1;
  };
  if (!p.skip_pad) {
    fetch_rows(0, 0);
    fetch_rows(1, 1);
    __syncthreads();
    if (nchunk > 0) {
      read_rowtab(0);
      issue(0, 0);
    }
    __syncthreads();
    for (int c = 0; c < nchunk; ++c) chunk((c + 1) % 3, (c + 2) % 3, c + 2, c + 1, c + 1 < nchunk, [] {});
  } else {
    int c0 = next_live(0);
    int c1 = next_live(c0 + 1);
    int c2 = next_live(c1 + 1);
    fetch_rows(c0, 0);
    fetch_rows(c1, 1);
    __syncthreads();
    if (c0 < nchunk) {
      read_rowtab(0);
      issue(c0, 0);
    }
    __syncthreads();
    int slot = 0;
    for (int c3 = 0; c0 < nchunk; c0 = c1, c1 = c2, c2 = c3, slot = slot == 2 ? 0 : slot + 1)
      chunk(slot == 2 ? 0 : slot + 1, slot == 0 ? 2 : slot - 1, c2, c1, c1 < nchunk, [&] { c3 = next_live(c2 + 1); });
  }

  float* dst = p.partial + (long long)z * p.Cout * p.Kld;
  if (H16) {
#pragma unroll
    for (int j = 0; j < 2; ++j) {
      const int kc = k0 + wn * WN + 16 * j + r16;
#pragma unroll
      for (int r = 0; r < 4; ++r) {
        const int co = co0 + 4 * g16 + r;
        if (kc < p.Kld && co < p.Cout) dst[(long long)co * p.Kld + kc] = acc16[j][r];
      }
    }
    return;
  }
  const int k = k0 + wn * WN + TN * l32;
  if (k < p.Kld) {
#pragma unroll
    for (int i = 0; i < TM; ++i)
#pragma unroll
      for (int e = 0; e < 16; ++e) {
        const int co = co0 + wm * WM + TM * ((e >> 2) * 8 + h * 4 + (e & 3)) + i;
        if (co < p.Cout) {
          typename FragVec<TN>::type v;
#pragma unroll
          for (int j = 0; j < TN; ++j) FragVec<TN>::set(v, j, acc[i][j][e]);
          *reinterpret_cast<typename FragVec<TN>::type*>(dst + (long long)co * p.Kld + k) = v;
        }
      }
  }
}

template <int BM, int BN, int WAVES_M, int WAVES_N>
__global__ __launch_bounds__(256, 2) void wgrad_dma_kernel(const WgradParams p) {
  wgrad_dma_body<BM, BN, WAVES_M, WAVES_N, false>(p);
}
__global__ __launch_bounds__(256, 2) void wgrad_dma_h16_kernel(const WgradParams p) { wgrad_dma_body<32, 128, 1, 4, true>(p); }

__global__ __launch_bounds__(256) void wgrad_reduce_kernel(const float* __restrict__ partial, float* __restrict__ dw,
                                                           int splitm, int Cout, int Cin, int taps, int Kld, int Cin_v) {
  extern __shared__ float wr_tile[];
  const int cit = Cin < 32 ? Cin : 32;
  const int ci0 = blockIdx.x * cit, co = blockIdx.y;
  const int nci = min(cit, Cin_v - ci0);
  if (nci <= 0) return;
  const long long slab = (long long)Cout * Kld;
  const float* base = partial + (long long)co * Kld;
  for (int e = threadIdx.x; e < nci * taps; e += 256) {
    const int tap = e / nci, cil = e - tap * nci;
    const float* src = base + tap * Cin + ci0 + cil;
    float s0 = 0.f, s1 = 0.f, s2 = 0.f, s3 = 0.f;
    int z = 0;
    for (; z + 4 <= splitm; z += 4) {
      s0 += src[(long long)z * slab];
      s1 += src[(long long)(z + 1) * slab];
      s2 += src[(long long)(z + 2) * slab];
      s3 += src[(long long)(z + 3) * slab];
    }
    for (; z < splitm; ++z) s0 += src[(long long)z * slab];
    wr_tile[cil * taps + tap] = (s0 + s1) + (s2 + s3);
  }
  __syncthreads();
  float* out = dw + ((long long)co * Cin_v + ci0) * taps;
  for (int e = threadIdx.x; e < nci * taps; e += 256) out[e] = wr_tile[e];
}

__global__ __launch_bounds__(256) void colsum_stage1(const float* __restrict__ a, long long rows, int C, int ld,
                                                     float* __restrict__ part, int rows_per_block) {
  __shared__ float red[4][64];
  const int c = blockIdx.y * 64 + (threadIdx.x & 63);
  const int rl = threadIdx.x >> 6;
  const long long r0 = (long long)blockIdx.x * rows_per_block;
  const long long r1 = r0 + rows_per_block < rows ? r0 + rows_per_block : rows;
  float s = 0.f;
  if (c < C)
    for (long long r = r0 + rl; r < r1; r += 4) s += a[r * ld + c];
  red[rl][threadIdx.x & 63] = s;
  __syncthreads();
  if (rl == 0 && c < C) part[(long long)blockIdx.x * C + c] = red[0][threadIdx.x] + red[1][threadIdx.x] + red[2][threadIdx.x] + red[3][threadIdx.x];
}
__global__ void colsum_stage2(const float* __restrict__ part, int nblk, int C, float* __restrict__ out) {
  const int c = blockIdx.x * blockDim.x + threadIdx.x;
  if (c >= C) return;
  double s = 0.0;
  for (int b = 0; b < nblk; ++b) s += (double)part[(long long)b * C + c];
  out[c] = (float)s;
}

constexpr size_t wgrad_lds(int bm, int bn, bool dma) { return (size_t)2 * RK * (bm + bn) * sizeof(float) + (dma ? 3 * RK * sizeof(uint2) : 0); }
inline dim3 wgrad_grid(const WgradParams& p) { return dim3((unsigned)(p.co_tiles * p.k_tiles) * (unsigned)p.splitm); }

template <int BM, int BN, int WAVES_M, int WAVES_N, bool VECA, bool VECB>
int launch_w(const WgradParams& p, hipStream_t s) {
  constexpr size_t lds = wgrad_lds(BM, BN, false);
  return rsp_launch_lds<&wgrad_kernel<BM, BN, WAVES_M, WAVES_N, VECA, VECB>>(wgrad_grid(p), lds, lds, s, std::tie(p),
                                                                             "wgrad_kernel<%d, %d, %d, %d, *>", BM, BN, WAVES_M, WAVES_N);
}

template <int BM, int BN, int WAVES_M, int WAVES_N>
int launch_w_dma(const WgradParams& p, hipStream_t s) {
  constexpr size_t lds = wgrad_lds(BM, BN, true);
  return rsp_launch_lds<&wgrad_dma_kernel<BM, BN, WAVES_M, WAVES_N>>(wgrad_grid(p), lds, lds, s, std::tie(p),
                                                                     "wgrad_dma_kernel<%d, %d, %d, %d>", BM, BN, WAVES_M, WAVES_N);
}

int launch_w_dma_h16(const WgradParams& p, hipStream_t s) {
  rsp_note_kernel("wgrad_dma_h16_kernel");
  hipLaunchKernelGGL(wgrad_dma_h16_kernel, wgrad_grid(p), dim3(256), wgrad_lds(32, 128, true), s, p);
  return rsp_check_launch("wgrad_dma_h16_kernel");
}

static bool wgrad_h16(int cout) { return !rsp_conv_option(OPT_NO_HALF_BLOCK) && cout <= 16; }

template <int BM, int BN, int WAVES_M, int WAVES_N>
int launch_w_vec(const WgradParams& p, bool va, bool vb, hipStream_t s) {
  if (va && vb) return launch_w<BM, BN, WAVES_M, WAVES_N, true, true>(p, s);
  if (va) return launch_w<BM, BN, WAVES_M, WAVES_N, true, false>(p, s);
  if (vb) return launch_w<BM, BN, WAVES_M, WAVES_N, false, true>(p, s);
  return launch_w<BM, BN, WAVES_M, WAVES_N, false, false>(p, s);
}

bool wdesc_ok(const rsp_conv3d_desc* d) { return rsp_conv_desc_ok(d); }

struct WPlan {
  int bm, bn, co_tiles, k_tiles, splitm, rows_per_split, Kld;
  size_t partial_bytes, colsum_bytes, rowgeom_bytes;
  bool dma;
  bool h16;
};

WPlan wplan(const rsp_conv3d_desc* d) {
  WPlan w;
  const long long M = (long long)d->N * d->Do * d->Ho * d->Wo;
  const int K = d->kT * d->kH * d->kW * d->Cin;
  w.Kld = (int)rsp_align_up((size_t)K, 4);
  w.bm = d->Cout > 64 ? 128 : (d->Cout > 32 ? 64 : 32);
  w.bn = K > 64 ? 128 : 64;
  if (w.bm == 32 && w.bn == 64) w.bm = 64;
  w.co_tiles = rsp_cdiv(d->Cout, w.bm);
  w.k_tiles = rsp_cdiv(K, w.bn);
  const int tiles = w.co_tiles * w.k_tiles;
  const long long max_sp = M / 256 > 0 ? M / 256 : 1;
  long long sp = 1;
  {
    const long long lds = 2ll * RK * (w.bm + w.bn) * 4 + 1024;
    const long long slots = 256 * (160 * 1024 / lds > 4 ? 4 : 160 * 1024 / lds);
    double best = -1.0;
    for (long long c = 1; c <= max_sp && c * tiles <= 8192; ++c) {
      const long long units = c * tiles, rounds = (units + slots - 1) / slots;
      const double score = (double)units / (double)(rounds * slots) - 0.004 * (double)rounds;
      if (score > best) {
        best = score;
        sp = c;
      }
    }
    if (sp > max_sp) sp = max_sp;
  }
  long long rps = (M + sp - 1) / sp;
  rps = (rps + RK - 1) / RK * RK;
  w.rows_per_split = (int)rps;
  w.splitm = (int)((M + rps - 1) / rps);
  w.partial_bytes = rsp_align_up((size_t)w.splitm * d->Cout * w.Kld * sizeof(float), 256);
  w.colsum_bytes = rsp_align_up((size_t)rsp_cdiv(M, 1024) * d->Cout * sizeof(float), 256);
  w.rowgeom_bytes = rsp_align_up((size_t)M * sizeof(uint2), 256);
  w.dma = d->Cout % 4 == 0 && d->out_ld % 4 == 0 && d->Cin % 4 == 0 && d->in_ld % 4 == 0 && d->kT <= 8 && d->kH <= 8 && d->kW <= 8;
  w.h16 = w.bm == 32 && wgrad_h16(d->Cout);
  return w;
}

}

struct WSegs { int n, at[2], width[2]; };
WSegs wgrad_segments(const rsp_conv3d_desc* d);

const char* rsp_wgrad_kernel_name(const rsp_conv3d_desc* d0) {
  if (!wdesc_ok(d0)) return "invalid";
  rsp_conv3d_desc first = *d0;
  first.Cout = wgrad_segments(d0).width[0];
  const rsp_conv3d_desc* d = &first;
  const WPlan w = wplan(d);
  if (w.bm == 32) return w.dma ? (w.h16 ? "wgrad_dma_h16_kernel" : "wgrad_dma_kernel<32, 128, 1, 4>") : "wgrad_kernel<32, 128, 1, 4, *>";
  if (w.dma) return w.bm == 128 ? (w.bn == 128 ? "wgrad_dma_kernel<128, 128, 2, 2>" : "wgrad_dma_kernel<128, 64, 2, 2>")
                              : (w.bn == 128 ? "wgrad_dma_kernel<64, 128, 2, 2>" : "wgrad_dma_kernel<64, 64, 2, 2>");
  return w.bm == 128 ? (w.bn == 128 ? "wgrad_kernel<128, 128, 2, 2, *>" : "wgrad_kernel<128, 64, 2, 2, *>")
                     : (w.bn == 128 ? "wgrad_kernel<64, 128, 2, 2, *>" : "wgrad_kernel<64, 64, 2, 2, *>");
}

WSegs wgrad_segments(const rsp_conv3d_desc* d) {
  WSegs g;
  memset(&g, 0, sizeof g);
  const int C = d->Cout;
  int full = C / 128 * 128, r = C - full;
  if (r > 64) { full = C; r = 0; }
  if (full > 0) { g.at[g.n] = 0; g.width[g.n++] = full; }
  if (r > 0) { g.at[g.n] = full; g.width[g.n++] = r; }
  return g;
}

namespace {

size_t wgrad_ws_one(const rsp_conv3d_desc* d) {
  const WPlan w = wplan(d);
  return w.partial_bytes + w.colsum_bytes + w.rowgeom_bytes;
}

struct WSkip {
  int skip_pad, kh0, kh1, lpt;
  long long dead_frames;
};

WSkip wgrad_skip_plan(const rsp_conv3d_desc* d, const WPlan& w) {
  WSkip k = {0, 0, 0, 0, 0};
  const bool no_skip = rsp_conv_option(OPT_NO_PAD_SKIP);
  k.skip_pad = (!no_skip && d->kT > 1 && d->pT > 0 && d->Ho * d->Wo >= RK) ? 1 : 0;
  const int K = d->kT * d->kH * d->kW * d->Cin;
  const int khw = d->kH * d->kW;
  bool open = false;
  for (int j = 0; j < w.k_tiles; ++j) {
    const int k0 = j * w.bn, k1 = (k0 + w.bn < K ? k0 + w.bn : K) - 1;
    const int kt_lo = (k0 / d->Cin) / khw, kt_hi = (k1 / d->Cin) / khw;
    int dead = 0;
    for (int g = 0; g < d->Do; ++g) dead += (g * d->sT - d->pT + kt_hi < 0 || g * d->sT - d->pT + kt_lo >= d->Di) ? 1 : 0;
    k.dead_frames += dead;
    if (!dead && !open) { k.kh0 = j; open = true; }
    if (!dead) k.kh1 = j + 1;
  }
  if (k.dead_frames * 100 < 6ll * w.k_tiles * d->Do) k.skip_pad = 0;
  if (k.kh0 == 0 && k.kh1 == w.k_tiles) k.skip_pad = 0;
  const long long lds = 2ll * RK * (w.bm + w.bn) * 4 + 1024;
  const long long slots = 256 * (160 * 1024 / lds > 4 ? 4 : 160 * 1024 / lds);
  k.lpt = (k.skip_pad && (long long)w.splitm * w.co_tiles * w.k_tiles * 2 > slots * 3) ? 1 : 0;
  k.skip_pad = k.lpt;
  return k;
}

int wgrad_one(const rsp_conv3d_desc* d, const float* x, const float* dy, float* dw_ref, float* dbias, void* workspace,
              size_t workspace_bytes, void* stream, bool rowgeom_ready, int cout_valid, int cin_valid, const uint2* ext_rowgeom);
int rowgeom_fill(const rsp_conv3d_desc* d, void* table, hipStream_t s);

}

double rsp_wgrad_executed_fraction(const rsp_conv3d_desc* d0) {
  if (!wdesc_ok(d0)) return 1.0;
  const WSegs g = wgrad_segments(d0);
  double live = 0.0, tot = 0.0;
  for (int i = 0; i < g.n; ++i) {
    rsp_conv3d_desc seg = *d0;
    seg.Cout = g.width[i];
    const WPlan w = wplan(&seg);
    const WSkip k = wgrad_skip_plan(&seg, w);
    const double f = (w.dma && k.skip_pad) ? 1.0 - (double)k.dead_frames / ((double)w.k_tiles * seg.Do) : 1.0;
    live += f * seg.Cout;
    tot += seg.Cout;
  }
  return tot > 0 ? live / tot : 1.0;
}


extern "C" {

size_t rsp_conv3d_wgrad_workspace(const rsp_conv3d_desc* d) {
  if (!wdesc_ok(d)) return 0;
  const WSegs g = wgrad_segments(d);
  size_t best = 0;
  for (int i = 0; i < g.n; ++i) {
    rsp_conv3d_desc a = *d;
    a.Cout = g.width[i];
    const size_t b = wgrad_ws_one(&a);
    best = b > best ? b : best;
  }
  return best;
}

static int wgrad_all(const rsp_conv3d_desc* d, const float* x, const float* dy, float* dw_ref, float* dbias, int cout_valid,
                     int cin_valid, void* workspace, size_t workspace_bytes, void* stream, const uint2* ext_rowgeom) {
  rsp_note_reset();
  const WSegs g = wgrad_segments(d);
  const long long per_co = (long long)cin_valid * d->kT * d->kH * d->kW;
  for (int i = 0; i < g.n; ++i) {
    rsp_conv3d_desc a = *d;
    a.Cout = g.width[i];
    const int at = g.at[i];
    int cov = cout_valid - at;
    cov = cov < 0 ? 0 : (cov > a.Cout ? a.Cout : cov);
    if (cov == 0) continue;
    const int rc = wgrad_one(&a, x, dy + at, dw_ref + at * per_co, dbias ? dbias + at : nullptr, workspace, workspace_bytes, stream,
                             i > 0, cov, cin_valid, ext_rowgeom);
    if (rc != RSP_OK) return rc;
  }
  return RSP_OK;
}

size_t rsp_conv3d_rowgeom_bytes(const rsp_conv3d_desc* d) {
  if (!wdesc_ok(d)) return 0;
  return (size_t)d->N * d->Do * d->Ho * d->Wo * sizeof(uint2);
}

int rsp_conv3d_rowgeom(const rsp_conv3d_desc* d, void* table, void* stream) {
  RSP_REQUIRE(wdesc_ok(d) && table && rsp_aligned16(table), "rsp_conv3d_rowgeom: bad argument");
  RSP_REQUIRE(d->kT <= 8 && d->kH <= 8 && d->kW <= 8, "rsp_conv3d_rowgeom: kernel dims above 8 take the table-free path");
  return rowgeom_fill(d, table, (hipStream_t)stream);
}

int rsp_conv3d_wgrad(const rsp_conv3d_desc* d, const float* x, const float* dy, float* dw_ref, float* dbias, int32_t cout_valid,
                     int32_t cin_valid, const void* rowgeom_table, void* workspace, size_t workspace_bytes, void* stream) {
  RSP_REQUIRE(wdesc_ok(d), "rsp_conv3d_wgrad: bad descriptor");
  RSP_REQUIRE(x && dy && dw_ref && workspace, "rsp_conv3d_wgrad: null pointer");
  RSP_REQUIRE(rsp_aligned16(workspace) && (!rowgeom_table || rsp_aligned16(rowgeom_table)), "rsp_conv3d_wgrad: workspace / table must be 16-byte aligned");
  RSP_REQUIRE(cout_valid > 0 && cout_valid <= d->Cout && cin_valid > 0 && cin_valid <= d->Cin, "rsp_conv3d_wgrad: bad valid channel counts");
  RSP_REQUIRE(!dbias || (cout_valid == d->Cout && cin_valid == d->Cin), "rsp_conv3d_wgrad: a bias gradient needs unpadded channels");
  return wgrad_all(d, x, dy, dw_ref, dbias, cout_valid, cin_valid, workspace, workspace_bytes, stream,
                   reinterpret_cast<const uint2*>(rowgeom_table));
}

}

namespace {

int rowgeom_fill(const rsp_conv3d_desc* d, void* table, hipStream_t s) {
  RowGeomParams g;
  g.out = reinterpret_cast<uint2*>(table);
  g.M = d->N * d->Do * d->Ho * d->Wo; g.Gd = d->Do; g.Gh = d->Ho; g.Gw = d->Wo; g.Di = d->Di; g.Hi = d->Hi; g.Wi = d->Wi; g.in_ld = d->in_ld;
  g.sD = d->sT; g.sH = d->sH; g.sW = d->sW; g.kT = d->kT; g.kH = d->kH; g.kW = d->kW; g.pT = d->pT; g.pH = d->pH; g.pW = d->pW;
  hipLaunchKernelGGL(rowgeom_kernel, dim3(rsp_cdiv(g.M, 256)), dim3(256), 0, s, g);
  return rsp_check_launch("rowgeom_kernel");
}

int wgrad_one(const rsp_conv3d_desc* d, const float* x, const float* dy, float* dw_ref, float* dbias, void* workspace,
              size_t workspace_bytes, void* stream, bool rowgeom_ready, int cout_valid, int cin_valid, const uint2* ext_rowgeom) {
  const WPlan w = wplan(d);
  if (workspace_bytes < w.partial_bytes + w.colsum_bytes + w.rowgeom_bytes) {
    rsp_set_error("rsp_conv3d_wgrad: workspace too small");
    return RSP_EWORKSPACE;
  }
  hipStream_t s = (hipStream_t)stream;
  static const float* zero_cache[64] = {nullptr};
  int dev_id = 0;
  if (hipGetDevice(&dev_id) != hipSuccess || dev_id < 0 || dev_id >= 64) dev_id = 0;
  if (!zero_cache[dev_id]) {
    void* z = nullptr;
    if (hipGetSymbolAddress(&z, HIP_SYMBOL(g_wzero)) != hipSuccess || !z) {
      rsp_set_error("hipGetSymbolAddress(g_wzero) failed");
      return RSP_ELAUNCH;
    }
    zero_cache[dev_id] = reinterpret_cast<const float*>(z);
  }
  const float* zero_page = zero_cache[dev_id];
  WgradParams p;
  memset(&p, 0, sizeof p);
  p.zero = zero_page;
  p.x = x; p.dy = dy; p.partial = reinterpret_cast<float*>(reinterpret_cast<unsigned char*>(workspace) + w.rowgeom_bytes);
  p.M = d->N * d->Do * d->Ho * d->Wo;
  p.Gd = d->Do; p.Gh = d->Ho; p.Gw = d->Wo;
  p.Di = d->Di; p.Hi = d->Hi; p.Wi = d->Wi; p.in_ld = d->in_ld; p.Cin = d->Cin;
  p.sD = d->sT; p.sH = d->sH; p.sW = d->sW;
  p.kT = d->kT; p.kH = d->kH; p.kW = d->kW; p.pT = d->pT; p.pH = d->pH; p.pW = d->pW;
  p.dy_ld = d->out_ld; p.Cout = d->Cout;
  p.K = d->kT * d->kH * d->kW * d->Cin;
  p.Kld = w.Kld;
  p.rows_per_split = w.rows_per_split; p.splitm = w.splitm;
  p.co_tiles = w.co_tiles; p.k_tiles = w.k_tiles;
  p.dP = fastdiv_make(d->Ho * d->Wo);
  p.dGd = fastdiv_make(d->Do);
  {
    const WSkip sk = wgrad_skip_plan(d, w);
    p.skip_pad = sk.skip_pad; p.kh0 = sk.kh0; p.kh1 = sk.kh1; p.lpt = sk.lpt;
  }
  const bool va = (d->Cout % 4 == 0) && (d->out_ld % 4 == 0) && rsp_aligned16(dy);
  const bool vb = (d->Cin % 4 == 0) && (d->in_ld % 4 == 0) && rsp_aligned16(x);
  const unsigned long long xb = (unsigned long long)d->N * d->Di * d->Hi * d->Wi * d->in_ld * 4ull;
  const unsigned long long dyb = (unsigned long long)p.M * d->out_ld * 4ull;
  p.x_bytes = (unsigned)xb;
  p.dy_bytes = (unsigned)dyb;
  bool dma = w.dma && va && vb && xb < (1ull << 32) && dyb < (1ull << 32) &&
             (unsigned long long)p.M * sizeof(uint2) < (1ull << 32);
  int rc;
  if (dma) {
    if (ext_rowgeom) {
      p.rowgeom = ext_rowgeom;
    } else {
      if (!rowgeom_ready) {
        rc = rowgeom_fill(d, workspace, s);
        if (rc != RSP_OK) return rc;
      }
      p.rowgeom = reinterpret_cast<const uint2*>(workspace);
    }
  }
  if (dma && w.bm == 32) rc = w.h16 ? launch_w_dma_h16(p, s) : launch_w_dma<32, 128, 1, 4>(p, s);
  else if (w.bm == 32) rc = launch_w_vec<32, 128, 1, 4>(p, va, vb, s);
  else if (dma && w.bm == 128 && w.bn == 128) rc = launch_w_dma<128, 128, 2, 2>(p, s);
  else if (dma && w.bm == 128) rc = launch_w_dma<128, 64, 2, 2>(p, s);
  else if (dma && w.bn == 128) rc = launch_w_dma<64, 128, 2, 2>(p, s);
  else if (dma) rc = launch_w_dma<64, 64, 2, 2>(p, s);
  else if (w.bm == 128 && w.bn == 128) rc = launch_w_vec<128, 128, 2, 2>(p, va, vb, s);
// ... 28 lines not shown
```

rspnet_amd/engine.py:

```python
from __future__ import annotations

import contextlib
import os
from dataclasses import dataclass, field
from typing import Dict, List, Optional, Tuple

import torch
from torch import nn

from . import ops as _ops
from .ops import ConvGeom, PoolGeom

Triple = Tuple[int, int, int]


@dataclass
class ConvBN:
    conv: nn.Module
    bn: nn.Module
    src: int
    dst: int
    k: Triple
    s: Triple = (1, 1, 1)
    p: Triple = (0, 0, 0)
# ... 515 lines not shown
            if pnode is not None:
                slots[pnode.dst] = o
                skipped.add(pi)
            elif gnode.into is None:
                slots[gnode.dst] = o
            skipped.add(gi)
            if keep:
                ctx.saved[key] = _Saved(xin, y, mi, ss, cg, pg, None)
                ctx.saved[gi] = (a, mean, gate) if keep_act else ("fused", key, mean, gate)
            return
        pg, res = bn_apply(node, y, ss, cg.Cout, N, do, ho, wo, xin, key)
        if keep:
            ctx.saved[key] = _Saved(xin, y, mi, ss, cg, pg, res, eval_mode=not training)

    def convbn_group(node, ni):
        ms = node.members
        wcat = _adjacent_cat([m.conv.weight.data for m in ms]) if training else None
        if wcat is None:
            for j, m in enumerate(ms):
                convbn(m, (ni, j))
            return
        xin = slots[ms[0].src]
        N, D, H, W, Cin = xin.shape
        if getattr(node, "_cat", None) is None:
            node._cat = _CatConv()
        node._cat.weight = wcat
        cg = ConvGeom(N, D, H, W, Cin, wcat.shape[0], ms[0].k, ms[0].s, ms[0].p)
        y, stats = be.conv_fwd(cg, xin, packed.get(node._cat_node(), cg), None, True)
        do, ho, wo = cg.out_dims
        off, per = 0, []
        for m in ms:
            C = m.conv.weight.shape[0]
            bn = m.bn
            mi, ss = finalize(bn, stats[:, off:off + C], cg.rows, None)
            pg, _ = bn_apply(m, y[..., off:off + C], ss, C, N, do, ho, wo, xin)
            per.append((off, C, mi, ss, pg))
            off += C
        if keep:
            ctx.saved[ni] = ("group", xin, y, cg, per)

    fusion = _gate_fusion(plan) if training else {}

    def run_node(ni, node):
        if ni in skipped:
            return
        if isinstance(node, ConvBN):
            convbn(node, ni, fusion.get(ni))
        elif isinstance(node, ConvBNGroup):
            convbn_group(node, ni)
        elif isinstance(node, ConvBias):
            xin = slots[node.src]
            N, D, H, W, Cin = xin.shape
            w = node.conv.weight
            cg = ConvGeom(N, D, H, W, Cin, w.shape[0], node.k, node.s, node.p)
            y, _ = be.conv_fwd(cg, xin, packed.get(node, cg), node.conv.bias.data, False)
            if node.relu:
                y = be.eltwise("relu_fwd", y, out=y)
            slots[node.dst] = y
            if keep:
                ctx.saved[ni] = (xin, y, cg)
        elif isinstance(node, Pool):
            xin = slots[node.src]
            N, D, H, W, Cc = xin.shape
            pg = PoolGeom(N, D, H, W, Cc, node.k, node.s, node.p)
            slots[node.dst], idx = be.maxpool_fwd(pg, xin, keep)
            if keep:
                ctx.saved[ni] = (pg, idx)
        elif isinstance(node, Gate):
            xin = slots[node.src]
            out = (_view(_slice_of(slots, node.into, tuple(xin.shape[:4]), xin.device), node.into, xin.shape[4])
                   if node.into is not None else None)
            o, mean, gate = be.gate_fwd(xin, node.conv.weight.data, node.conv.bias.data, out=out)
            if node.into is None:
                slots[node.dst] = o
            if keep:
                ctx.saved[ni] = (xin, mean, gate)
        else:
            raise NotImplementedError(f"plan node {type(node).__name__}")

    branches = BranchStreams(x)
    for ni, node in enumerate(plan.nodes):
        branches.run(node, lambda: run_node(ni, node))
    branches.finish()
    out = slots[plan.output_slot]
    if keep:
        ctx.feat_shape = tuple(out.shape)
    return out, ctx


def run_backward(plan: Plan, ctx: ForwardCtx, dfeat: torch.Tensor, grad_of, after_param_grads=None,
                 want_input_grad: bool = False, packed: Optional[PackedWeights] = None):
    it = run_backward_iter(plan, ctx, dfeat, grad_of, after_param_grads, want_input_grad, packed)
    try:
        while True:
            next(it)
    except StopIteration as done:
        return done.value


def run_backward_iter(plan: Plan, ctx: ForwardCtx, dfeat: torch.Tensor, grad_of, after_param_grads=None,
                      want_input_grad: bool = False, packed: Optional[PackedWeights] = None):
    be = _ops.backend()
    packed = packed if packed is not None else ctx.packed
    dslots: Dict[int, torch.Tensor] = {plan.output_slot: dfeat}
    branches = BranchStreams(dfeat)
    fused_gates: Dict[int, Tuple] = {}

    def add_grad(slot, g):
        if g is None:
            return
        if slot in dslots:
            dslots[slot] = be.eltwise("add", dslots[slot].contiguous(), g, out=g)
        else:
            dslots[slot] = g

    def convbn_virtual_bwd(node, sv, ni):
        _, x_e, x_o, y, mi, ss, cg, pg, vs = sv
        assert node.src == plan.input_slot and not want_input_grad, "a virtual-pixel stem reads the clip: no input gradient"
        dout = dslots.pop(node.dst)
        bn = node.bn
        dy, _ = be.bn_act_pool_bwd(pg, y, None, dout, bn.weight.data, mi, ss, node.relu, False, grad_of(bn.weight), grad_of(bn.bias))
        gw = grad_of(node.conv.weight)
        if gw is not None:
            N, do, ho, Wo, Cp = dy.shape
            dyv = dy.view(N, do, ho, Wo // 2, 2 * Cp)
            gflat = gw.view(-1)
            gflat.zero_()
            for c, xc in enumerate((x_e, x_o)):
                gv = torch.empty_like(vs.holders[c].conv.weight)
                be.conv_wgrad(cg, xc, dyv[..., c * Cp:(c + 1) * Cp], gv)
                gflat.index_add_(0, vs.dst[c], gv.view(-1).index_select(0, vs.src[c]))
        if after_param_grads is not None:
            after_param_grads(ni, branches.grads_ready)

    def convbn_bwd(node, key, ni):
        sv = ctx.saved.pop(key)
        if isinstance(sv, tuple) and sv[0] == "vstem":
            return convbn_virtual_bwd(node, sv, ni)
        bn = node.bn
        gated = fused_gates.pop(key, None)
        if gated is not None:
            gi, mean, gate = gated
            gnode = plan.nodes[gi]
            dout = _view(dslots[gnode.into[0]], gnode.into, sv.cg.Cout) if gnode.into is not None else dslots.pop(gnode.dst)
            dy = be.bn_act_gate_bwd(sv.pg, sv.y, dout, bn.weight.data, sv.mi, sv.ss, node.relu, gnode.conv.weight.data, mean, gate,
                                    grad_of(bn.weight), grad_of(bn.bias), grad_of(gnode.conv.weight), grad_of(gnode.conv.bias))
            dres = None
            if after_param_grads is not None:
                after_param_grads(gi, branches.grads_ready)
        elif sv.eval_mode:
            return convbn_eval_bwd(node, sv, ni)
        else:
            dout = _view(dslots[node.into[0]], node.into, sv.cg.Cout) if node.into is not None else dslots.pop(node.dst)
            dy, dres = be.bn_act_pool_bwd(sv.pg, sv.y, sv.res, dout, bn.weight.data, sv.mi, sv.ss, node.relu,
                                          node.residual is not None, grad_of(bn.weight), grad_of(bn.bias))
        convbn_tail(node, sv, ni, dy, dres, True)

    def convbn_eval_bwd(node, sv, ni):
        if not hasattr(be, "bn_eval_act_pool_bwd"):
            raise RuntimeError(EVAL_BACKWARD_MISSING)
        bn = node.bn
        dout = _view(dslots[node.into[0]], node.into, sv.cg.Cout) if node.into is not None else dslots.pop(node.dst)
        bias = getattr(node.conv, "bias", None)
        gbias = grad_of(bias) if bias is not None else None
        dgamma, dbeta = grad_of(bn.weight), grad_of(bn.bias)
        sums = dbeta if (dbeta is not None or gbias is None) else torch.empty_like(bn.bias.data)
        dy, dres = be.bn_eval_act_pool_bwd(sv.pg, sv.y, sv.res, dout, sv.mi, sv.ss, node.relu, node.residual is not None, dgamma, sums)
        if gbias is not None:
            torch.mul(sv.ss[0][:gbias.shape[0]], sums, out=gbias)
        convbn_tail(node, sv, ni, dy, dres, False)

    def convbn_tail(node, sv, ni, dy, dres, zero_bias):
        if node.residual is not None:
            add_grad(node.residual, dres)
        bias = getattr(node.conv, "bias", None)
        if bias is not None and zero_bias:
            gb = grad_of(bias)
            if gb is not None:
                gb.zero_()
        gw = grad_of(node.conv.weight)
        if (sv.cg.flops < BranchStreams.SMALL_WGRAD_FLOPS or
                (sv.cg.flops < BranchStreams.MID_WGRAD_FLOPS and sv.cg.bytes < BranchStreams.MID_WGRAD_BYTES)):
            branches.side_task(lambda: be.conv_wgrad(sv.cg, sv.x, dy, gw), (sv.x, dy), cost=float(sv.cg.flops))
        else:
            be.conv_wgrad(sv.cg, sv.x, dy, gw)
        if after_param_grads is not None:
            after_param_grads(ni, branches.grads_ready)
        if node.src != plan.input_slot or want_input_grad:
            add_grad(node.src, be.conv_dgrad_packed(sv.cg, dy, packed.get_dgrad(node, sv.cg)))

    def convbn_group_bwd(node, ni):
        sv = ctx.saved.pop(ni, None)
        ms = node.members
        if sv is None:
            for j in range(len(ms) - 1, -1, -1):
                convbn_bwd(ms[j], (ni, j), ni)
            return
        _, xin, y, cg, per = sv
        dy_cat = torch.empty_like(y)
        for m, (off, C, mi, ss, pg) in zip(ms, per):
            dout = _view(dslots[m.into[0]], m.into, C) if m.into is not None else dslots.pop(m.dst)
            be.bn_act_pool_bwd(pg, y[..., off:off + C], None, dout, m.bn.weight.data, mi, ss, m.relu, False,
                               grad_of(m.bn.weight), grad_of(m.bn.bias), dy_out=dy_cat[..., off:off + C])
        gws = [grad_of(m.conv.weight) for m in ms]
        gcat = _adjacent_cat(gws) if all(g is not None for g in gws) else None
        if gcat is not None:
            be.conv_wgrad(cg, xin, dy_cat, gcat)
        else:
            tmp = torch.empty_like(node._cat.weight)
            be.conv_wgrad(cg, xin, dy_cat, tmp)
            off = 0
            for m, g in zip(ms, gws):
                if g is not None:
                    g.copy_(tmp[off:off + g.shape[0]])
                off += m.conv.weight.shape[0]
        if after_param_grads is not None:
            after_param_grads(ni, branches.grads_ready)
        if ms[0].src != plan.input_slot or want_input_grad:
            add_grad(ms[0].src, be.conv_dgrad_packed(cg, dy_cat, packed.get_dgrad(node._cat_node(), cg)))

    def run_node(ni, node):
        if isinstance(node, ConvBN):
            convbn_bwd(node, ni, ni)
        elif isinstance(node, ConvBNGroup):
            convbn_group_bwd(node, ni)
        elif isinstance(node, ConvBias):
            xin, y, cg = ctx.saved.pop(ni)
            dout = dslots.pop(node.dst)
            dz = be.eltwise("relu_bwd", y, dout.contiguous()) if node.relu else dout.contiguous()
            be.conv_wgrad(cg, xin, dz, grad_of(node.conv.weight), grad_of(node.conv.bias))
            if after_param_grads is not None:
                after_param_grads(ni, branches.grads_ready)
            if node.src != plan.input_slot or want_input_grad:
                add_grad(node.src, be.conv_dgrad_packed(cg, dz, packed.get_dgrad(node, cg)))
            del dz, dout
        elif isinstance(node, Pool):
            pg, idx = ctx.saved.pop(ni)
            add_grad(node.src, be.maxpool_bwd(pg, dslots.pop(node.dst), idx))
        elif isinstance(node, Gate):
            sv = ctx.saved.pop(ni)
            if sv[0] == "fused":
                fused_gates[sv[1]] = (ni, sv[2], sv[3])
                return
            xin, mean, gate = sv
            dout = (_view(dslots[node.into[0]], node.into, xin.shape[4]) if node.into is not None
                    else dslots.pop(node.dst))
            add_grad(node.src, be.gate_bwd(xin, dout, node.conv.weight.data, mean, gate, grad_of(node.conv.weight),
                                           grad_of(node.conv.bias)))
            if after_param_grads is not None:
                after_param_grads(ni, branches.grads_ready)
        else:
            raise NotImplementedError(f"plan node {type(node).__name__}")

    for ni in range(len(plan.nodes) - 1, -1, -1):
        node = plan.nodes[ni]
        branches.run(node, lambda: run_node(ni, node))
        yield ni
    branches.finish()
    return dslots.get(plan.input_slot) if want_input_grad else None
```

rspnet_amd/ops.py:

```python
from __future__ import annotations

import collections
import contextlib
import ctypes as C
import functools
from dataclasses import dataclass
from typing import Optional, Tuple

import torch

from . import _lib


@dataclass(frozen=True)
class ConvGeom:
    N: int
    Di: int
    Hi: int
    Wi: int
    Cin: int
    Cout: int
    k: Tuple[int, int, int]
    s: Tuple[int, int, int]
    p: Tuple[int, int, int]
    Cin_alg: float = 0

    @property
    def out_dims(self):
        return tuple((i + 2 * p - k) // s + 1 for i, k, s, p in zip((self.Di, self.Hi, self.Wi), self.k, self.s, self.p))

    @property
    def rows(self):
        d, h, w = self.out_dims
        return self.N * d * h * w

    @property
    def flops(self):
        return int(2 * self.rows * self.Cout * (self.Cin_alg or self.Cin) * self.k[0] * self.k[1] * self.k[2])

    @property
    def bytes(self):
        taps = self.k[0] * self.k[1] * self.k[2]
        cin = self.Cin_alg or self.Cin
        return int(4 * (self.N * self.Di * self.Hi * self.Wi * cin + self.rows * self.Cout + self.Cout * cin * taps))

    def desc(self, in_ld=None, out_ld=None) -> _lib.ConvDesc:
        do, ho, wo = self.out_dims
        return _lib.ConvDesc(self.N, self.Di, self.Hi, self.Wi, self.Cin, do, ho, wo, self.Cout, *self.k, *self.s, *self.p,
                             in_ld or self.Cin, out_ld or self.Cout)


@dataclass(frozen=True)
class PoolGeom:
    N: int
    Di: int
    Hi: int
    Wi: int
    C: int
    k: Tuple[int, int, int] = (1, 1, 1)
    s: Tuple[int, int, int] = (1, 1, 1)
    p: Tuple[int, int, int] = (0, 0, 0)

    @property
    def out_dims(self):
        return tuple((i + 2 * p - k) // s + 1 for i, k, s, p in zip((self.Di, self.Hi, self.Wi), self.k, self.s, self.p))

    def desc(self, in_ld=None, out_ld=None, res_ld=None) -> _lib.PoolDesc:
        do, ho, wo = self.out_dims
        return _lib.PoolDesc(self.N, self.Di, self.Hi, self.Wi, self.C, do, ho, wo, *self.k, *self.s, *self.p,
                             in_ld or self.C, out_ld or self.C, res_ld or self.C)


@functools.lru_cache(maxsize=4096)
def _conv_plan(g: "ConvGeom", in_ld, out_ld):
    lib = _lib.load()
    d = g.desc(in_ld=in_ld, out_ld=out_ld)
    ref = C.byref(d)
    names = tuple(lib.rsp_conv3d_kernel_name(ref, which).decode() for which in (0, 1, 2))
    return (d, ref, lib.rsp_conv3d_stat_tiles(ref), lib.rsp_conv3d_fwd_workspace(ref), lib.rsp_conv3d_dgrad_workspace(ref),
            lib.rsp_conv3d_wgrad_workspace(ref), g.out_dims, names)


@functools.lru_cache(maxsize=4096)
def executed_fraction(g: "ConvGeom", which: int) -> float:
    d = g.desc()
    return float(_lib.load().rsp_conv3d_executed_fraction(C.byref(d), which))


@functools.lru_cache(maxsize=8192)
def _pack_signature(g: "ConvGeom", which: int, cout_src: int, cin_src: int):
    lib = _lib.load()
    d = g.desc()
    buf = (_lib.PackJob * 64)()
    cnt = lib.rsp_conv3d_pack_jobs(C.byref(d), which, cout_src, cin_src, C.c_void_p(1 << 20), C.c_void_p(1 << 30), buf, 64)
    lib.rsp_conv3d_pack_forget(C.c_void_p(1 << 30))
    if cnt < 0:
        _lib.check(cnt, "rsp_conv3d_pack_jobs")
    n = (lib.rsp_conv3d_packed_dgrad_elems if which else lib.rsp_conv3d_packed_fwd_elems)(C.byref(d))
    return (int(n), bytes(buf)[:cnt * C.sizeof(_lib.PackJob)])


@functools.lru_cache(maxsize=4096)
def _pool_plan(pg: "PoolGeom", in_ld, out_ld, res_ld):
    lib = _lib.load()
    d = pg.desc(in_ld=in_ld, out_ld=out_ld, res_ld=res_ld)
    ref = C.byref(d)
    return d, ref, lib.rsp_bn_bwd_workspace(ref), pg.out_dims


def _ptr(t: Optional[torch.Tensor]):
    return None if t is None else C.c_void_p(t.data_ptr())


_raw_stream = getattr(torch._C, "_cuda_getCurrentRawStream", None)
_get_device = getattr(torch._C, "_cuda_getDevice", None)


def _stream():
    if _raw_stream is not None and _get_device is not None:
        return C.c_void_p(_raw_stream(_get_device()))
    return C.c_void_p(torch.cuda.current_stream().cuda_stream)


def _chk(t: torch.Tensor, name: str, dtype=torch.float32):
    if not t.is_cuda:
        raise _lib.RspError(f"{name}: expected a HIP device tensor (rspnet_amd has no CPU path)")
    if t.dtype != dtype:
        raise _lib.RspError(f"{name}: expected {dtype}, got {t.dtype}")
    if not t.is_contiguous():
        raise _lib.RspError(f"{name}: expected a contiguous tensor")
    return t


def _rows_ld(t: torch.Tensor, name: str) -> int:
    if not t.is_cuda or t.dtype != torch.float32:
        raise _lib.RspError(f"{name}: expected a float32 HIP device tensor (rspnet_amd has no CPU path)")
    if t.is_contiguous():
        return t.shape[-1]
    ld = t.stride(-2)
    exp, ok = ld, t.stride(-1) == 1
    for dim in range(t.dim() - 2, -1, -1):
        ok = ok and (t.stride(dim) == exp or t.shape[dim] == 1)
        exp *= t.shape[dim]
    if not ok:
        raise _lib.RspError(f"{name}: expected a dense NDHWC tensor or a channel slice of one")
    return ld


def _dy_target(y, in_ld: int, dy_out):
    if dy_out is not None:
        if _rows_ld(dy_out, "dy_out") != in_ld or dy_out.shape != y.shape:
            raise _lib.RspError("dy_out: expected the shape and channel pitch of y")
        return dy_out
    if not y.is_contiguous():
        raise _lib.RspError("y is a channel slice: pass dy_out with the same pitch")
    return torch.empty_like(y)


class HipOps:

    name = "hip"

    def __init__(self):
        self.lib = _lib.load(init_gpu=True)
        self._ws = {}
        self._rowgeom = collections.OrderedDict()
        self._rowgeom_bytes = 0
        self._rowgeom_streams = {}
        self.event_log = None
        self.hbm_log = None

    def _ev(self):
        if self.event_log is None:
            return None
        e = torch.cuda.Event(enable_timing=True)
        e.record()
        return e

    def _log(self, kind, g, e0, kernel=""):
        if e0 is not None:
            e1 = torch.cuda.Event(enable_timing=True)
            e1.record()
            which = {"conv_fwd": 0, "conv_dgrad": 1, "conv_wgrad": 2}[kind]
            self.event_log.append((kind, g.flops, e0, e1, kernel, g.bytes, g, g.flops * executed_fraction(g, which)))

    def _log_hbm(self, kind, nbytes, e0):
        if e0 is not None and self.hbm_log is not None:
            e1 = torch.cuda.Event(enable_timing=True)
            e1.record()
            self.hbm_log.append((kind, int(nbytes), e0, e1))

    def _workspace(self, dev, nbytes: int) -> torch.Tensor:
        if torch.cuda.is_current_stream_capturing():
            return torch.empty(max(int(nbytes), 256), dtype=torch.uint8, device=dev)
        key = (dev, _stream().value)
        buf = self._ws.get(key)
        if buf is None or buf.numel() < nbytes:
            if buf is not None:
                buf.record_stream(torch.cuda.current_stream(dev))
            buf = torch.empty(max(int(nbytes), 1 << 20), dtype=torch.uint8, device=dev)
            self._ws[key] = buf
        return buf

    def set_option(self, name: str, value: int) -> int:
        prev = self.lib.rsp_conv3d_set_option(name.encode(), int(value))
        if prev < 0:
            _lib.check(prev, "rsp_conv3d_set_option")
        _conv_plan.cache_clear()
        executed_fraction.cache_clear()
        return prev

    @contextlib.contextmanager
    def options(self, **kw):
        before = {}
        try:
            for name, value in kw.items():
                prev = self.set_option(name, value)
                self.set_option(name, -1)
                unset = self.set_option(name, value)
                before[name] = -1 if prev == unset else prev
            yield self
        finally:
            for name, value in before.items():
                self.set_option(name, value)

    def conv_pack_fwd(self, g: ConvGeom, w_ref: torch.Tensor) -> torch.Tensor:
        _chk(w_ref, "w_ref")
        d = g.desc()
        n = self.lib.rsp_conv3d_packed_fwd_elems(C.byref(d))
        out = torch.empty(n, dtype=torch.float32, device=w_ref.device)
        _lib.check(self.lib.rsp_conv3d_pack_fwd(C.byref(d), _ptr(w_ref), _ptr(out), _stream()), "rsp_conv3d_pack_fwd")
        return out

    def conv_fwd(self, g: ConvGeom, x, w_packed, bias, want_stats: bool, out: Optional[torch.Tensor] = None,
                 out_ld: Optional[int] = None, in_ld: Optional[int] = None):
        _chk(x, "x")
        d, dref, tiles, wsb, _, _, (do, ho, wo), names = _conv_plan(g, in_ld, out_ld)
        if out is None:
            out = torch.empty((g.N, do, ho, wo, g.Cout), dtype=torch.float32, device=x.device)
        stats = None
        if want_stats:
            stats = torch.empty((tiles, g.Cout, 2), dtype=torch.float32, device=x.device)
        ws = self._workspace(x.device, wsb) if wsb else None
        e0 = self._ev()
        _lib.check(self.lib.rsp_conv3d_fwd(dref, _ptr(x), _ptr(w_packed), _ptr(bias), _ptr(out), _ptr(stats),
                                           _ptr(ws), wsb, _stream()), "rsp_conv3d_fwd")
        self._log("conv_fwd", g, e0, names[0])
        return out, stats

    def conv_dgrad(self, g: ConvGeom, dy, w_ref):
        _chk(dy, "dy")
        _chk(w_ref, "w_ref")
        d, dref, _, _, wsb, _, _, names = _conv_plan(g, None, None)
        dx = torch.empty((g.N, g.Di, g.Hi, g.Wi, g.Cin), dtype=torch.float32, device=dy.device)
        ws = self._workspace(dy.device, wsb)
        e0 = self._ev()
        _lib.check(self.lib.rsp_conv3d_dgrad(dref, _ptr(dy), _ptr(w_ref), _ptr(dx), _ptr(ws), wsb, _stream()),
                   "rsp_conv3d_dgrad")
        self._log("conv_dgrad", g, e0, names[1])
        return dx

    def conv_dgrad_packed(self, g: ConvGeom, dy, w_packed):
        _chk(dy, "dy")
        d, dref, _, _, wsb, _, _, names = _conv_plan(g, None, None)
        dx = torch.empty((g.N, g.Di, g.Hi, g.Wi, g.Cin), dtype=torch.float32, device=dy.device)
        ws = self._workspace(dy.device, wsb)
        e0 = self._ev()
        _lib.check(self.lib.rsp_conv3d_dgrad_packed(dref, _ptr(dy), _ptr(_chk(w_packed, "w_packed")), _ptr(dx), _ptr(ws), wsb,
                                                    _stream()), "rsp_conv3d_dgrad_packed")
        self._log("conv_dgrad", g, e0, names[1])
        return dx

    def pack_signature(self, g: ConvGeom, which: int, w_ref):
        return _pack_signature(g, which, int(w_ref.shape[0]), int(w_ref.shape[1]))

    def pack_set(self, entries):
        return PackSet(self, entries)

    def conv_wgrad(self, g: ConvGeom, x, dy, dw_out: torch.Tensor, dbias_out: Optional[torch.Tensor] = None):
        _chk(x, "x")
        _chk(dw_out, "dw_out")
        dy_ld = _rows_ld(dy, "dy")
        d, dref, _, _, _, wsb, _, names = _conv_plan(g, None, None if dy_ld == g.Cout else dy_ld)
        ws = self._workspace(x.device, wsb)
        if dw_out.shape[0] > g.Cout or dw_out.shape[1] > g.Cin or (dbias_out is not None and tuple(dw_out.shape[:2]) != (g.Cout, g.Cin)):
            raise _lib.RspError("conv_wgrad: dw_out has more channels than the geometry, or a bias gradient with padded channels")
        table = self._rowgeom_table(g, d, dref, x.device)
        e0 = self._ev()
        _lib.check(self.lib.rsp_conv3d_wgrad(dref, _ptr(x), _ptr(dy), _ptr(dw_out), _ptr(dbias_out), dw_out.shape[0], dw_out.shape[1],
                                             _ptr(table), _ptr(ws), wsb, _stream()), "rsp_conv3d_wgrad")
        self._log("conv_wgrad", g, e0, names[2])

    ROWGEOM_MAX_TABLES = 128
    ROWGEOM_MAX_BYTES = 2 << 30

    def _rowgeom_table(self, g: ConvGeom, d, dref, dev):
        if max(g.k) > 8:
            return None
        key = (dev, g.N, g.Di, g.Hi, g.Wi, g.k, g.s, g.p, d.in_ld)
        ent = self._rowgeom.get(key)
        capturing = torch.cuda.is_current_stream_capturing()
        here = _stream().value
        if ent is None:
            if capturing:
                return None
            nbytes = int(self.lib.rsp_conv3d_rowgeom_bytes(dref))
            t = torch.empty(nbytes, dtype=torch.uint8, device=dev)
            _lib.check(self.lib.rsp_conv3d_rowgeom(dref, _ptr(t), _stream()), "rsp_conv3d_rowgeom")
            ev = torch.cuda.Event()
            ev.record()
            ent = self._rowgeom[key] = [t, ev, here, False]
            self._rowgeom_bytes += nbytes
            self._rowgeom_evict(dev)
        else:
            self._rowgeom.move_to_end(key)
            if ent[1] is not None and not capturing:
                if ent[1].query():
                    ent[1] = None
                elif here != ent[2]:
                    torch.cuda.current_stream(dev).wait_event(ent[1])
            if capturing:
                ent[3] = True
        if here not in self._rowgeom_streams and not capturing:
            self._rowgeom_streams[here] = torch.cuda.current_stream(dev)
        return ent[0]

    def _rowgeom_evict(self, dev):
        if len(self._rowgeom) <= self.ROWGEOM_MAX_TABLES and self._rowgeom_bytes <= self.ROWGEOM_MAX_BYTES:
            return
        for key in list(self._rowgeom)[:-1]:
            if len(self._rowgeom) <= self.ROWGEOM_MAX_TABLES and self._rowgeom_bytes <= self.ROWGEOM_MAX_BYTES:
                break
            t, _, _, pinned = self._rowgeom[key]
            if pinned:
                continue
            for st in self._rowgeom_streams.values():
                t.record_stream(st)
            self._rowgeom_bytes -= t.numel()
            del self._rowgeom[key]

    def bn_finalize(self, stats, count: int, conv_bias, gamma, beta, eps: float, momentum: float, running_mean,
                    running_var, batch_stats_out=None):
        tiles, Cc, _ = stats.shape
        if stats.is_contiguous():
            _chk(stats, "stats")
            stat_ld = Cc
        else:
            if not stats.is_cuda or stats.dtype != torch.float32 or stats.stride(2) != 1 or stats.stride(1) != 2 or stats.stride(0) % 2:
                raise _lib.RspError("stats: expected [tiles][C][2] float32 partials or a channel slice of them")
            stat_ld = stats.stride(0) // 2
        mi = torch.empty((2, Cc), dtype=torch.float32, device=stats.device)
        ss = torch.empty((2, Cc), dtype=torch.float32, device=stats.device)
        wsb = int(self.lib.rsp_bn_finalize_workspace(tiles, Cc))
        ws = self._workspace(stats.device, wsb)
        c_valid = Cc if gamma is None else int(gamma.shape[0])
        _lib.check(self.lib.rsp_bn_finalize(_ptr(stats), tiles, Cc, c_valid, stat_ld, count, _ptr(conv_bias), _ptr(gamma), _ptr(beta),
                                            eps, momentum, _ptr(running_mean), _ptr(running_var), _ptr(batch_stats_out), _ptr(mi),
                                            _ptr(ss), _ptr(ws), wsb, _stream()), "rsp_bn_finalize")
        return mi, ss

    def bn_ema_set(self, entries):
        return BnEmaSet(self, entries)

    def bn_act_pool_fwd(self, pg: PoolGeom, y, scale_shift, residual, relu: bool, out=None):
        in_ld = _rows_ld(y, "y")
        if out is None:
            do, ho, wo = pg.out_dims
            out = torch.empty((pg.N, do, ho, wo, pg.C), dtype=torch.float32, device=y.device)
        d, dref, _, _ = _pool_plan(pg, in_ld, _rows_ld(out, "out"), None if residual is None else _rows_ld(residual, "residual"))
        e0 = self._ev()
        _lib.check(self.lib.rsp_bn_act_pool_fwd(dref, _ptr(y), _ptr(scale_shift), _ptr(residual), int(relu), None, _ptr(out),
                                                _stream()), "rsp_bn_act_pool_fwd")
        n_in = pg.N * pg.Di * pg.Hi * pg.Wi * pg.C
        self._log_hbm("bn_act_pool_fwd", 4 * (n_in * (1 if residual is None else 2) + out.numel()), e0)
        return out

    def bn_act_maxpool_fwd(self, pg: PoolGeom, y, scale_shift, relu: bool, keep: bool):
        in_ld = _rows_ld(y, "y")
        do, ho, wo = pg.out_dims
        d = pg.desc(in_ld=in_ld)
        if not self.lib.rsp_bn_act_maxpool_applicable(C.byref(d)) or y.data_ptr() % 16 or scale_shift.data_ptr() % 16:
            return None
        out = torch.empty((pg.N, do, ho, wo, pg.C), dtype=torch.float32, device=y.device)
        idx = torch.empty((pg.N, do, ho, wo, pg.C), dtype=torch.int32, device=y.device) if keep else None
        e0 = self._ev()
        _lib.check(self.lib.rsp_bn_act_maxpool_fwd(C.byref(d), _ptr(y), _ptr(scale_shift), int(relu), None, _ptr(out), _ptr(idx),
                                                   _stream()), "rsp_bn_act_maxpool_fwd")
        self._log_hbm("bn_act_pool_fwd", 4 * (pg.N * pg.Di * pg.Hi * pg.Wi * pg.C + out.numel() * (2 if keep else 1)), e0)
        return out, idx

    def bn_act_pool_bwd(self, pg: PoolGeom, y, residual, dout, gamma, mean_invstd, scale_shift, relu: bool,
                        want_dres: bool, dgamma_out, dbeta_out, dy_out=None):
        in_ld = _rows_ld(y, "y")
        d, dref, wsb, _ = _pool_plan(pg, in_ld, _rows_ld(dout, "dout"), None if residual is None else _rows_ld(residual, "residual"))
        dy = _dy_target(y, in_ld, dy_out)
        dres = torch.empty_like(y) if want_dres else None
        ws = self._workspace(y.device, wsb)
        c_valid = pg.C if gamma is None else int(gamma.shape[0])
        e0 = self._ev()
        _lib.check(self.lib.rsp_bn_act_pool_bwd(dref, _ptr(y), _ptr(residual), _ptr(dout), _ptr(gamma),
                                                _ptr(mean_invstd), _ptr(scale_shift), int(relu), _ptr(dy), _ptr(dres),
                                                _ptr(dgamma_out), _ptr(dbeta_out), c_valid, None, None, _ptr(ws), wsb, _stream()),
                   "rsp_bn_act_pool_bwd")
        n_in = y.numel()
        self._log_hbm("bn_bwd(reduce+apply)", 4 * (2 * (n_in * (1 if residual is None else 2) + dout.numel()) + n_in * (2 if want_dres else 1)), e0)
        return dy, dres

    def bn_eval_act_pool_bwd(self, pg: PoolGeom, y, residual, dout, mean_invstd, scale_shift, relu: bool, want_dres: bool,
                             dgamma_out, dbeta_out, dy_out=None):
        in_ld = _rows_ld(y, "y")
        d, dref, _, _ = _pool_plan(pg, in_ld, _rows_ld(dout, "dout"), None if residual is None else _rows_ld(residual, "residual"))
        dy = _dy_target(y, in_ld, dy_out)
        if want_dres and residual is None:
            raise _lib.RspError("want_dres without a residual")
        dres = torch.empty(y.shape, dtype=torch.float32, device=y.device) if want_dres else None
        if want_dres and d.res_ld != pg.C:
            raise _lib.RspError("residual: a residual whose gradient is wanted must be contiguous")
        sums = dgamma_out is not None or dbeta_out is not None
        c_valid = pg.C
        for v in (dgamma_out, dbeta_out):
            if v is not None:
                c_valid = int(v.shape[0])
        wsb = int(self.lib.rsp_bn_eval_bwd_workspace(dref)) if sums else 0
        ws = self._workspace(y.device, wsb) if sums else None
        e0 = self._ev()
        _lib.check(self.lib.rsp_bn_eval_act_pool_bwd(dref, _ptr(y), _ptr(residual), _ptr(dout), _ptr(mean_invstd), _ptr(scale_shift),
                                                     int(relu), _ptr(dy), _ptr(dres), _ptr(dgamma_out), _ptr(dbeta_out), c_valid,
                                                     _ptr(ws), wsb, _stream()), "rsp_bn_eval_act_pool_bwd")
        n_in = y.numel()
        self._log_hbm("bn_eval_bwd(one pass)", 4 * (n_in * (1 if residual is None else 2) + dout.numel() + n_in * (2 if want_dres else 1)), e0)
        return dy, dres

    def maxpool_fwd(self, pg: PoolGeom, x, keep: bool):
        do, ho, wo = pg.out_dims
        out = torch.empty((pg.N, do, ho, wo, pg.C), dtype=torch.float32, device=x.device)
        idx = torch.empty((pg.N, do, ho, wo, pg.C), dtype=torch.int32, device=x.device) if keep else None
        d = pg.desc(in_ld=_rows_ld(x, "x"))
        _lib.check(self.lib.rsp_maxpool3d_fwd(C.byref(d), _ptr(x), _ptr(out), _ptr(idx), _stream()), "rsp_maxpool3d_fwd")
        return out, idx

    def maxpool_bwd(self, pg: PoolGeom, dout, idx):
        dx = torch.empty((pg.N, pg.Di, pg.Hi, pg.Wi, pg.C), dtype=torch.float32, device=dout.device)
        d = pg.desc(out_ld=_rows_ld(dout, "dout"))
        _lib.check(self.lib.rsp_maxpool3d_bwd(C.byref(d), _ptr(dout), _ptr(idx), _ptr(dx), _stream()), "rsp_maxpool3d_bwd")
        return dx

    def gate_fwd(self, x, w, b, out=None):
        _chk(x, "x")
        N, D, H, W, Cc = x.shape
        P = D * H * W
        if out is None:
            out = torch.empty_like(x)
        mean = torch.empty((N, Cc), dtype=torch.float32, device=x.device)
        gate = torch.empty((N, Cc), dtype=torch.float32, device=x.device)
        wsb = self.lib.rsp_gate_fwd_workspace(N, P, Cc)
        ws = self._workspace(x.device, wsb)
        _lib.check(self.lib.rsp_gate_fwd(_ptr(x), N, P, Cc, Cc, _ptr(_chk(w, "w")), _ptr(_chk(b, "b")), _ptr(out),
                                         _rows_ld(out, "out"), _ptr(mean), _ptr(gate), _ptr(ws), wsb, _stream()),
                   "rsp_gate_fwd")
        return out, mean, gate

    gate_pool_keep = True

    def bn_act_gate_fwd(self, pg: PoolGeom, y, scale_shift, relu: bool, w, b, keep_act: bool, pool: Optional[PoolGeom] = None,
                        out=None, pool_idx: bool = False):
        N, P, Cc = pg.N, pg.Di * pg.Hi * pg.Wi, pg.C
        y_ld = _rows_ld(y, "y")
        if keep_act and pool is not None:
            raise _lib.RspError("bn_act_gate_fwd: the pooled form keeps no activation")
        a = torch.empty((N, pg.Di, pg.Hi, pg.Wi, Cc), dtype=torch.float32, device=y.device) if keep_act else None
        mean = torch.empty((N, Cc), dtype=torch.float32, device=y.device)
        gate = torch.empty((N, Cc), dtype=torch.float32, device=y.device)
        wsb = self.lib.rsp_gate_fwd_workspace(N, P, Cc)
        ws = self._workspace(y.device, wsb)
        _lib.check(self.lib.rsp_bn_gate_sums(_ptr(y), N, P, Cc, y_ld, _ptr(scale_shift), int(relu), _ptr(a), Cc, _ptr(_chk(w, "w")),
                                             _ptr(_chk(b, "b")), _ptr(mean), _ptr(gate), _ptr(ws), wsb, _stream()), "rsp_bn_gate_sums")
        og = pool if pool is not None else pg
        if out is None:
            do, ho, wo = og.out_dims
            out = torch.empty((N, do, ho, wo, Cc), dtype=torch.float32, device=y.device)
        if keep_act:
            _lib.check(self.lib.rsp_gate_apply(_ptr(a), N, P, Cc, Cc, _ptr(gate), _ptr(out), _rows_ld(out, "out"), _stream()),
                       "rsp_gate_apply")
        elif pool_idx:
            d, dref, _, _ = _pool_plan(og, y_ld, _rows_ld(out, "out"), None)
            idx = torch.empty(tuple(out.shape), dtype=torch.int32, device=y.device)
            _lib.check(self.lib.rsp_bn_act_maxpool_fwd(dref, _ptr(y), _ptr(scale_shift), int(relu), _ptr(gate), _ptr(out), _ptr(idx),
                                                       _stream()), "rsp_bn_act_maxpool_fwd")
            return out, a, mean, gate, idx
        else:
            d, dref, _, _ = _pool_plan(og, y_ld, _rows_ld(out, "out"), None)
            _lib.check(self.lib.rsp_bn_act_pool_fwd(dref, _ptr(y), _ptr(scale_shift), None, int(relu), _ptr(gate), _ptr(out),
                                                    _stream()), "rsp_bn_act_pool_fwd")
        return out, a, mean, gate

    def bn_act_gate_pool_idx_ok(self, pool: PoolGeom, y, scale_shift) -> bool:
        d = pool.desc(in_ld=_rows_ld(y, "y"))
        return bool(self.lib.rsp_bn_act_maxpool_applicable(C.byref(d))) and y.data_ptr() % 16 == 0 and scale_shift.data_ptr() % 16 == 0

    def bn_act_gate_bwd(self, pg: PoolGeom, y, dout, gamma, mean_invstd, scale_shift, relu: bool, w, mean, gate,
                        dgamma_out, dbeta_out, dw_out, db_out):
        N, P, Cc = pg.N, pg.Di * pg.Hi * pg.Wi, pg.C
        _chk(y, "y")
        dout_ld = _rows_ld(dout, "dout")
        dmean = torch.empty((N, Cc), dtype=torch.float32, device=y.device)
        wsb = self.lib.rsp_gate_bwd_workspace(N, P, Cc)
        ws = self._workspace(y.device, wsb)
        _lib.check(self.lib.rsp_gate_bwd_params(_ptr(y), _ptr(scale_shift), int(relu), _ptr(dout), N, P, Cc, Cc, dout_ld, _ptr(_chk(w, "w")),
                                                _ptr(mean), _ptr(gate), _ptr(dw_out), _ptr(db_out), _ptr(dmean), _ptr(ws), wsb,
                                                _stream()), "rsp_gate_bwd_params")
        d, dref, wsb2, _ = _pool_plan(pg, Cc, dout_ld, None)
        ws2 = self._workspace(y.device, wsb2)
        dy = torch.empty_like(y)
        c_valid = pg.C if gamma is None else int(gamma.shape[0])
        _lib.check(self.lib.rsp_bn_act_pool_bwd(dref, _ptr(y), None, _ptr(dout), _ptr(gamma), _ptr(mean_invstd), _ptr(scale_shift),
                                                int(relu), _ptr(dy), None, _ptr(dgamma_out), _ptr(dbeta_out), c_valid, _ptr(gate),
                                                _ptr(dmean), _ptr(ws2), wsb2, _stream()), "rsp_bn_act_pool_bwd")
        return dy

    def gate_bwd(self, x, dout, w, mean, gate, dw_out, db_out):
        _chk(x, "x")
        N, D, H, W, Cc = x.shape
        P = D * H * W
        dx = torch.empty_like(x)
        wsb = self.lib.rsp_gate_bwd_workspace(N, P, Cc)
        ws = self._workspace(x.device, wsb)
        _lib.check(self.lib.rsp_gate_bwd(_ptr(x), _ptr(dout), N, P, Cc, Cc, _rows_ld(dout, "dout"), _ptr(w), _ptr(mean),
                                         _ptr(gate), _ptr(dx), Cc, _ptr(dw_out), _ptr(db_out), _ptr(ws), wsb, _stream()),
                   "rsp_gate_bwd")
        return dx

    def head_fwd(self, feat, w1, b1, w2, b2):
        _chk(feat, "feat")
        N, D, H, W, Cc = feat.shape
        P = D * H * W
        dim = w1.shape[0]
        dev = feat.device
        o1 = torch.empty((N, dim), dtype=torch.float32, device=dev)
        o2 = torch.empty((N, dim), dtype=torch.float32, device=dev)
        pooled = torch.empty((N, Cc), dtype=torch.float32, device=dev)
        raw = torch.empty((2, N, dim), dtype=torch.float32, device=dev)
        _lib.check(self.lib.rsp_head_fwd(_ptr(feat), N, P, Cc, Cc, _ptr(w1), _ptr(b1), _ptr(w2), _ptr(b2), dim, _ptr(o1),
                                         _ptr(o2), _ptr(pooled), _ptr(raw), _stream()), "rsp_head_fwd")
        return o1, o2, pooled, raw

    def head_bwd(self, d1, d2, pooled, raw, w1, w2, feat_shape, dw1, db1, dw2, db2):
        N, D, H, W, Cc = feat_shape
        P = D * H * W
        dim = w1.shape[0]
        dfeat = torch.empty(feat_shape, dtype=torch.float32, device=d1.device)
        wsb = self.lib.rsp_head_bwd_workspace(N, dim)
        ws = self._workspace(d1.device, wsb)
        _lib.check(self.lib.rsp_head_bwd(_ptr(_chk(d1, "d1")), _ptr(_chk(d2, "d2")), _ptr(pooled), _ptr(raw), _ptr(w1),
                                         _ptr(w2), N, P, Cc, Cc, dim, _ptr(dw1), _ptr(db1), _ptr(dw2), _ptr(db2),
                                         _ptr(dfeat), _ptr(ws), wsb, _stream()), "rsp_head_bwd")
        return dfeat

    def spatial_mean_fwd(self, x):
        _chk(x, "x")
# ... 368 lines not shown
```

Measured before the change: 353.0.

## Fuse first-layer BN/pool backward apply with conv weight-gradient via MFMA

For the first conv block, whose input needs no gradient, a new kernel recomputes the BN/ReLU/maxpool backward dy in shared memory per tile and feeds it straight into an MFMA weight-gradient accumulation against the input halo. Per-block partials are then summed by a slab-reduce kernel. This avoids writing dy to global memory and reading it back in a separate wgrad pass, but the fused path gives up the side-stream overlap of wgrad and adds a partial-sum reduction. It can be turned off through a new option.

New measurement: 355.6 (median of 6 runs). About the same (+0.7%).

```diff
diff --git a/include/rspnet_hip.h b/include/rspnet_hip.h
--- a/include/rspnet_hip.h
+++ b/include/rspnet_hip.h
@@ -105,6 +105,13 @@
                         const float* gamma, const float* mean_invstd, const float* scale_shift, int relu, float* dy,
                         float* dres, float* dgamma, float* dbeta, int32_t c_valid, const float* gate, const float* dmean,
                         void* workspace, size_t workspace_bytes, void* stream);
+
+int rsp_bn_act_pool_bwd_wgrad_applicable(const rsp_conv3d_desc* c, const rsp_pool3d_desc* d);
+size_t rsp_bn_act_pool_bwd_wgrad_workspace(const rsp_conv3d_desc* c, const rsp_pool3d_desc* d);
+int rsp_bn_act_pool_bwd_wgrad(const rsp_conv3d_desc* c, const rsp_pool3d_desc* d, const float* x, const float* y, const float* dout,
+                              const float* gamma, const float* mean_invstd, const float* scale_shift, int relu, float* dgamma,
+                              float* dbeta, int32_t c_valid, float* dw_ref, int32_t cout_valid, int32_t cin_valid, void* workspace,
+                              size_t workspace_bytes, void* stream);
 
 size_t rsp_bn_eval_bwd_workspace(const rsp_pool3d_desc* d);
 int rsp_bn_eval_act_pool_bwd(const rsp_pool3d_desc* d, const float* y, const float* residual, const float* dout,
diff --git a/rspnet_amd/_lib.py b/rspnet_amd/_lib.py
--- a/rspnet_amd/_lib.py
+++ b/rspnet_amd/_lib.py
@@ -90,6 +90,9 @@
     "rsp_bn_act_maxpool_fwd": (C.c_int, [_PP, _p, _p, C.c_int, _p, _p, _p, _p]),
     "rsp_bn_bwd_workspace": (_sz, [_PP]),
     "rsp_bn_act_pool_bwd": (C.c_int, [_PP, _p, _p, _p, _p, _p, _p, C.c_int, _p, _p, _p, _p, _i32, _p, _p, _p, _sz, _p]),
+    "rsp_bn_act_pool_bwd_wgrad_applicable": (C.c_int, [_PD, _PP]),
+    "rsp_bn_act_pool_bwd_wgrad_workspace": (_sz, [_PD, _PP]),
+    "rsp_bn_act_pool_bwd_wgrad": (C.c_int, [_PD, _PP, _p, _p, _p, _p, _p, _p, C.c_int, _p, _p, _i32, _p, _i32, _i32, _p, _sz, _p]),
     "rsp_bn_eval_bwd_workspace": (_sz, [_PP]),
     "rsp_bn_eval_act_pool_bwd": (C.c_int, [_PP, _p, _p, _p, _p, _p, C.c_int, _p, _p, _p, _p, _i32, _p, _sz, _p]),
     "rsp_maxpool3d_fwd": (C.c_int, [_PP, _p, _p, _p, _p]),
diff --git a/rspnet_amd/csrc/bn_pool.hip b/rspnet_amd/csrc/bn_pool.hip
--- a/rspnet_amd/csrc/bn_pool.hip
+++ b/rspnet_amd/csrc/bn_pool.hip
@@ -1,4 +1,5 @@
 #include "common.h"
+#include "conv_stem.h"
 
 namespace {
 
@@ -640,6 +641,51 @@
   }
 }
 
+template <int VEC>
+__device__ __forceinline__ void load_apply_consts(const BwdParams& p, int c, float (&sc)[VEC], float (&sh)[VEC], float (&mean)[VEC],
+                                                  float (&invstd)[VEC], float (&gam)[VEC], float (&m1)[VEC], float (&m2)[VEC]) {
+  load_vec<VEC>(p.ss + c, sc);
+  load_vec<VEC>(p.ss + p.d.C + c, sh);
+  load_vec<VEC>(p.mi + c, mean);
+  load_vec<VEC>(p.mi + p.d.C + c, invstd);
+  load_gamma<VEC>(p, c, gam);
+  const double invn = 1.0 / (double)p.count;
+#pragma unroll
+  for (int e = 0; e < VEC; ++e) {
+    m1[e] = (float)(p.sums[2 * (c + e)] * invn);
+    m2[e] = (float)(p.sums[2 * (c + e) + 1] * invn);
+  }
+}
+
+template <int VEC, int NW>
+__device__ __forceinline__ void window_argmax(const float (&yv)[NW][VEC], const float (&r)[NW][VEC], bool has_res, int relu,
+                                              const float (&sc)[VEC], const float (&sh)[VEC], float (&best)[VEC], int (&bi)[VEC]) {
+#pragma unroll
+  for (int e = 0; e < VEC; ++e) { best[e] = -INFINITY; bi[e] = 0; }
+#pragma unroll
+  for (int w = 0; w < NW; ++w)
+#pragma unroll
+    for (int e = 0; e < VEC; ++e) {
+      float z = fmaf(yv[w][e], sc[e], sh[e]);
+      if (has_res) z += r[w][e];
+      const float v = relu ? fmaxf(z, 0.f) : z;
+      if (v > best[e]) { best[e] = v; bi[e] = w; }
+    }
+}
+
+template <int VEC>
+__device__ __forceinline__ void window_dy(int w, const float (&yw)[VEC], const float (&g)[VEC], const float (&best)[VEC],
+                                          const int (&bi)[VEC], int relu, const float (&mean)[VEC], const float (&invstd)[VEC],
+                                          const float (&gam)[VEC], const float (&m1)[VEC], const float (&m2)[VEC], float (&ov)[VEC],
+                                          float (&dz)[VEC]) {
+#pragma unroll
+  for (int e = 0; e < VEC; ++e) {
+    dz[e] = (bi[e] == w && !(relu && !(best[e] > 0.f))) ? g[e] : 0.f;
+    const float xhat = (yw[e] - mean[e]) * invstd[e];
+    ov[e] = gam[e] * invstd[e] * (dz[e] - m1[e] - xhat * m2[e]);
+  }
+}
+
 template <int VEC, int MODE>
 __global__ __launch_bounds__(256) void bn_bwd_apply_win_kernel(const BwdParams p) {
   const rsp_pool3d_desc& d = p.d;
@@ -713,26 +759,11 @@
           if (p.res) load_vec<VEC>(p.res + (base + off[w]) * d.res_ld + c, r[w]);
         }
         load_vec<VEC>(p.dout + o * d.out_ld + c, g);
-#pragma unroll
-        for (int e = 0; e < VEC; ++e) { best[e] = -INFINITY; bi[e] = 0; }
-#pragma unroll
-        for (int w = 0; w < NW; ++w)
-#pragma unroll
-          for (int e = 0; e < VEC; ++e) {
-            float z = fmaf(yv[w][e], sc[e], sh[e]);
-            if (p.res) z += r[w][e];
-            const float v = p.relu ? fmaxf(z, 0.f) : z;
-            if (v > best[e]) { best[e] = v; bi[e] = w; }
-          }
+        window_argmax<VEC, NW>(yv, r, p.res != nullptr, p.relu, sc, sh, best, bi);
 #pragma unroll
         for (int w = 0; w < NW; ++w) {
           float ov[VEC], dz[VEC];
-#pragma unroll
-          for (int e = 0; e < VEC; ++e) {
-            dz[e] = (bi[e] == w && !(p.relu && !(best[e] > 0.f))) ? g[e] : 0.f;
-            const float xhat = (yv[w][e] - mean[e]) * invstd[e];
-            ov[e] = gam[e] * invstd[e] * (dz[e] - m1[e] - xhat * m2[e]);
-          }
+          window_dy<VEC>(w, yv[w], g, best, bi, p.relu, mean, invstd, gam, m1, m2, ov, dz);
           store_vec<VEC>(p.dy + (base + off[w]) * d.in_ld + c, ov);
           if (p.dres) store_vec<VEC>(p.dres + (base + off[w]) * d.res_ld + c, dz);
         }
@@ -798,6 +829,185 @@
       }
     }
   }
+}
+
+struct BwdWgradParams {
+  BwdParams b;
+  const float* __restrict__ x;
+  float* __restrict__ partial;
+  int xD, xH, xW;
+  int kT, kH, kW, pT, pH, pW;
+  int taps, K, Kld;
+  int FT, HT, WT, npix;
+  int tiles_w, tiles_h, tiles_d, tiles;
+};
+
+template <int NW, int NB>
+__global__ __launch_bounds__(256, (NW != 8 && NB == 3) ? 2 : 1) void bn_bwd_wgrad_kernel(const BwdWgradParams q) {
+  constexpr int PT = NW == 8 ? 2 : 1;
+  constexpr int PK = NW == 1 ? 1 : 2;
+  constexpr int ROWS = 128 * PT;
+  constexpr int WPR = 16 / PK;
+  constexpr int ITEMS = ROWS / NW * 16 / 256;
+  const BwdParams& p = q.b;
+  const rsp_pool3d_desc& d = p.d;
+  extern __shared__ __attribute__((aligned(16))) unsigned char smem_raw[];
+  float* dyT = reinterpret_cast<float*>(smem_raw);
+  float* halo = dyT + ROWS * 64;
+
+  const int t = threadIdx.x;
+  const int lane = t & 63;
+  const int wave = __builtin_amdgcn_readfirstlane(t >> 6);
+  const int l32 = lane & 31, h = lane >> 5;
+
+  const int c = (t & 15) * 4;
+  const bool c_ok = c < d.C;
+  float sc[4], sh[4], mean[4], invstd[4], gam[4], m1[4], m2[4];
+#pragma unroll
+  for (int e = 0; e < 4; ++e) sc[e] = sh[e] = mean[e] = invstd[e] = gam[e] = m1[e] = m2[e] = 0.f;
+  if (c_ok) load_apply_consts<4>(p, c, sc, sh, mean, invstd, gam, m1, m2);
+  long long off[NW];
+  window_offsets<NW>(d, off);
+  int hy0[ITEMS], wx0[ITEMS];
+#pragma unroll
+  for (int j = 0; j < ITEMS; ++j) {
+    const int win = (t >> 4) + 16 * j;
+    hy0[j] = (win / WPR) * PK;
+    wx0[j] = (win % WPR) * PK;
+  }
+  int hf[3], hh[3], hw[3];
+#pragma unroll
+  for (int u = 0; u < 3; ++u) {
+    const int i = t + 256 * u;
+    hf[u] = -(1 << 20);
+    hh[u] = hw[u] = 0;
+    if (i < q.npix) {
+      hw[u] = i % q.WT;
+      const int r = i / q.WT;
+      hh[u] = r % q.HT;
+      hf[u] = r / q.HT;
+    }
+  }
+  int koff[NB];
+#pragma unroll
+  for (int j = 0; j < NB; ++j) {
+    const int kk = j * 32 + l32;
+    koff[j] = 0;
+    if (kk < q.K) {
+      const int ci = kk / q.taps, tap = kk - ci * q.taps;
+      const int kw = tap % q.kW, r = tap / q.kW;
+      const int kh = r % q.kH, kt = r / q.kH;
+      koff[j] = ((kt * q.HT + kh) * q.WT + kw) * 4 + ci;
+    }
+  }
+
+  float yv[ITEMS][NW][4], g[ITEMS][4];
+  floatx4 hx[3];
+  unsigned okmask = 0;
+  auto load_tile = [&](int tile) {
+    const int tw = tile % q.tiles_w;
+    int q1 = tile / q.tiles_w;
+    const int th = q1 % q.tiles_h;
+    q1 /= q.tiles_h;
+    const int td = q1 % q.tiles_d, n = q1 / q.tiles_d;
+    okmask = 0;
+#pragma unroll
+    for (int j = 0; j < ITEMS; ++j) {
+      const int gh = th * 8 + hy0[j], gw = tw * 16 + wx0[j];
+      if (c_ok && gh < d.Hi && gw < d.Wi) {
+        okmask |= 1u << j;
+        const long long base = (((long long)n * d.Di + td * PT) * d.Hi + gh) * d.Wi + gw;
+#pragma unroll
+        for (int w = 0; w < NW; ++w) load_vec<4>(p.y + (base + off[w]) * d.in_ld + c, yv[j][w]);
+        const long long op = (((long long)n * d.Do + td) * d.Ho + gh / PK) * d.Wo + gw / PK;
+        load_vec<4>(p.dout + op * d.out_ld + c, g[j]);
+      }
+    }
+#pragma unroll
+    for (int u = 0; u < 3; ++u) {
+      const int gf = td * PT - q.pT + hf[u], gy = th * 8 - q.pH + hh[u], gx = tw * 16 - q.pW + hw[u];
+      hx[u] = floatx4{0.f, 0.f, 0.f, 0.f};
+      if ((unsigned)gf < (unsigned)q.xD && (unsigned)gy < (unsigned)q.xH && (unsigned)gx < (unsigned)q.xW)
+        hx[u] = *reinterpret_cast<const floatx4*>(q.x + ((((long long)n * q.xD + gf) * q.xH + gy) * q.xW + gx) * 4);
+    }
+  };
+  auto store_tile = [&]() {
+#pragma unroll
+    for (int j = 0; j < ITEMS; ++j) {
+      float best[4];
+      int bi[4];
+      const bool ok = (okmask >> j) & 1u;
+      if (ok) window_argmax<4, NW>(yv[j], yv[j], false, p.relu, sc, sh, best, bi);
+#pragma unroll
+      for (int w = 0; w < NW; ++w) {
+        float ov[4] = {0.f, 0.f, 0.f, 0.f}, dz[4];
+        if (ok) window_dy<4>(w, yv[j][w], g[j], best, bi, p.relu, mean, invstd, gam, m1, m2, ov, dz);
+        const int row = ((w / (PK * PK)) * 8 + hy0[j] + (w / PK) % PK) * 16 + wx0[j] + w % PK;
+        store_vec<4>(dyT + row * 64 + c, ov);
+      }
+    }
+#pragma unroll
+    for (int u = 0; u < 3; ++u)
+      if (t + 256 * u < q.npix) *reinterpret_cast<floatx4*>(halo + (t + 256 * u) * 4) = hx[u];
+  };
+
+  floatx16 acc[2][NB];
+#pragma unroll
+  for (int i = 0; i < 2; ++i)
+#pragma unroll
+    for (int j = 0; j < NB; ++j)
+#pragma unroll
+      for (int e = 0; e < 16; ++e) acc[i][j][e] = 0.f;
+
+  int tile = blockIdx.x;
+  if (tile < q.tiles) load_tile(tile);
+  for (; tile < q.tiles; tile += gridDim.x) {
+    store_tile();
+    __syncthreads();
+    const int next = tile + gridDim.x;
+    if (next < q.tiles) load_tile(next);
+    __builtin_amdgcn_sched_barrier(0);
+#pragma unroll
+    for (int qq = 0; qq < PT; ++qq) {
+      const int r0 = wave * 32 * PT + qq * 32;
+      const float* a = dyT + (r0 + h) * 64 + l32;
+      const float* b = halo + (((r0 >> 7) * q.HT + ((r0 >> 4) & 7)) * q.WT + h) * 4;
+#pragma unroll
+      for (int s = 0; s < 16; ++s) {
+        float af[2], bf[NB];
+#pragma unroll
+        for (int i = 0; i < 2; ++i) af[i] = a[2 * s * 64 + i * 32];
+        const float* bs = b + ((s >> 3) * q.WT + ((2 * s) & 15)) * 4;
+#pragma unroll
+        for (int j = 0; j < NB; ++j) bf[j] = bs[koff[j]];
+#pragma unroll
+        for (int i = 0; i < 2; ++i)
+#pragma unroll
+          for (int j = 0; j < NB; ++j) acc[i][j] = __builtin_amdgcn_mfma_f32_32x32x2f32(af[i], bf[j], acc[i][j], 0, 0, 0);
+      }
+    }
+    __syncthreads();
+  }
+
+  float* stage = dyT;
+  for (int w = 0; w < 4; ++w) {
+    if (wave == w) {
+#pragma unroll
+      for (int i = 0; i < 2; ++i)
+#pragma unroll
+        for (int j = 0; j < NB; ++j)
+#pragma unroll
+          for (int e = 0; e < 16; ++e) {
+            const int co = i * 32 + (e >> 2) * 8 + h * 4 + (e & 3), kk = j * 32 + l32;
+            float* sp = stage + co * q.Kld + kk;
+            const float v = (w ? *sp : 0.f) + acc[i][j][e];
+            *sp = kk < q.K ? v : 0.f;
+          }
+    }
+    __syncthreads();
+  }
+  floatx4* dst = reinterpret_cast<floatx4*>(q.partial + (long long)blockIdx.x * 64 * q.Kld);
+  for (int i = t; i < 16 * q.Kld; i += 256) dst[i] = reinterpret_cast<const floatx4*>(stage)[i];
 }
 
 struct EvalBwdParams {
@@ -1156,21 +1366,18 @@
   return rsp_align_up((size_t)2048 * d->C * 2 * sizeof(float), 256) + (size_t)d->C * 2 * sizeof(double);
 }
 
-int rsp_bn_act_pool_bwd(const rsp_pool3d_desc* d, const float* y, const float* residual, const float* dout,
-                        const float* gamma, const float* mean_invstd, const float* scale_shift, int relu, float* dy,
-                        float* dres, float* dgamma, float* dbeta, int32_t c_valid, const float* gate, const float* dmean,
-                        void* workspace, size_t workspace_bytes, void* stream) {
-  RSP_REQUIRE(pool_ok(d, true), "rsp_bn_act_pool_bwd: needs disjoint windows (kernel == stride, no padding)");
-  RSP_REQUIRE(!gate || (dmean && d->kT * d->kH * d->kW == 1 && d->sT * d->sH * d->sW == 1 && !residual),
-              "rsp_bn_act_pool_bwd: a gated unit has a unit window, no residual, and needs dmean");
-  RSP_REQUIRE(c_valid > 0 && c_valid <= d->C, "rsp_bn_act_pool_bwd: bad valid channel count");
-  RSP_REQUIRE(y && dout && mean_invstd && scale_shift && dy && workspace, "rsp_bn_act_pool_bwd: null pointer");
-  if (workspace_bytes < rsp_bn_bwd_workspace(d)) {
-    rsp_set_error("rsp_bn_act_pool_bwd: workspace too small");
-    return RSP_EWORKSPACE;
-  }
-  hipStream_t s = (hipStream_t)stream;
+struct BwdLaunch {
   BwdParams p;
+  Layout L;
+  bool vec;
+  int mode;
+};
+
+static int bn_bwd_sums(const rsp_pool3d_desc* d, const float* y, const float* residual, const float* dout, const float* gamma,
+                       const float* mean_invstd, const float* scale_shift, int relu, float* dy, float* dres, float* dgamma,
+                       float* dbeta, int32_t c_valid, const float* gate, const float* dmean, void* workspace, hipStream_t s,
+                       const char* too_many, BwdLaunch& b) {
+  BwdParams& p = b.p;
   memset(&p, 0, sizeof p);
   p.d = *d; p.y = y; p.res = residual; p.dout = dout; p.gamma = gamma; p.mi = mean_invstd; p.ss = scale_shift;
   p.dy = dy; p.dres = dres; p.relu = relu;
@@ -1188,19 +1395,43 @@
   double* sums = reinterpret_cast<double*>(reinterpret_cast<unsigned char*>(workspace) +
                                            rsp_align_up((size_t)2048 * d->C * 2 * sizeof(float), 256));
   p.sums = sums;
-  const Layout L = make_layout(d, p.cg, 4);
-  RSP_REQUIRE(L.npos < (1ll << 31), "rsp_bn_act_pool_bwd: more than 2^31 - 1 output positions");
-  set_layout(p, L);
+  b.L = make_layout(d, p.cg, 4);
+  RSP_REQUIRE(b.L.npos < (1ll << 31), too_many);
+  set_layout(p, b.L);
   p.nblocks = reduce_blocks(d, p.cg);
   dim3 rgrid(p.nblocks, rsp_cdiv(p.cg, 256));
-  const int mode = bn_mode(d, gate != nullptr);
-  RSP_BN_LAUNCH(bn_bwd_reduce_kernel, vec, mode, rgrid, s, p);
+  b.vec = vec;
+  b.mode = bn_mode(d, gate != nullptr);
+  RSP_BN_LAUNCH(bn_bwd_reduce_kernel, vec, b.mode, rgrid, s, p);
   int rc = rsp_check_launch("bn_bwd_reduce_kernel");
   if (rc != RSP_OK) return rc;
   hipLaunchKernelGGL(bn_bwd_finalize_kernel, dim3(rsp_cdiv(d->C, FIN_CH)), dim3(1024), 0, s, p.partial, p.nblocks, d->C, c_valid, sums,
                      dgamma, dbeta);
-  rc = rsp_check_launch("bn_bwd_finalize_kernel");
+  return rsp_check_launch("bn_bwd_finalize_kernel");
+}
+
+int rsp_bn_act_pool_bwd(const rsp_pool3d_desc* d, const float* y, const float* residual, const float* dout,
+                        const float* gamma, const float* mean_invstd, const float* scale_shift, int relu, float* dy,
+                        float* dres, float* dgamma, float* dbeta, int32_t c_valid, const float* gate, const float* dmean,
+                        void* workspace, size_t workspace_bytes, void* stream) {
+  RSP_REQUIRE(pool_ok(d, true), "rsp_bn_act_pool_bwd: needs disjoint windows (kernel == stride, no padding)");
+  RSP_REQUIRE(!gate || (dmean && d->kT * d->kH * d->kW == 1 && d->sT * d->sH * d->sW == 1 && !residual),
+              "rsp_bn_act_pool_bwd: a gated unit has a unit window, no residual, and needs dmean");
+  RSP_REQUIRE(c_valid > 0 && c_valid <= d->C, "rsp_bn_act_pool_bwd: bad valid channel count");
+  RSP_REQUIRE(y && dout && mean_invstd && scale_shift && dy && workspace, "rsp_bn_act_pool_bwd: null pointer");
+  if (workspace_bytes < rsp_bn_bwd_workspace(d)) {
+    rsp_set_error("rsp_bn_act_pool_bwd: workspace too small");
+    return RSP_EWORKSPACE;
+  }
+  hipStream_t s = (hipStream_t)stream;
+  BwdLaunch b;
+  int rc = bn_bwd_sums(d, y, residual, dout, gamma, mean_invstd, scale_shift, relu, dy, dres, dgamma, dbeta, c_valid, gate, dmean,
+                       workspace, s, "rsp_bn_act_pool_bwd: more than 2^31 - 1 output positions", b);
   if (rc != RSP_OK) return rc;
+  const BwdParams& p = b.p;
+  const Layout& L = b.L;
+  const bool vec = b.vec;
+  const int mode = b.mode;
   const bool exact = d->Di % d->sT == 0 && d->Hi % d->sH == 0 && d->Wi % d->sW == 0 && d->kT * d->kH * d->kW <= 8;
   if (exact) {
     RSP_BN_LAUNCH(bn_bwd_apply_win_kernel, vec, mode, L.grid, s, p);
@@ -1210,6 +1441,109 @@
   if (vec) hipLaunchKernelGGL(bn_bwd_apply_kernel<4>, dim3(grid_for(total)), dim3(256), 0, s, p);
   else hipLaunchKernelGGL(bn_bwd_apply_kernel<1>, dim3(grid_for(total)), dim3(256), 0, s, p);
   return rsp_check_launch("bn_bwd_apply_kernel");
+}
+
+}
+
+namespace {
+
+struct BwdWgradPlan {
+  bool ok;
+  int NW, PT, FT, HT, WT, npix, tiles_w, tiles_h, tiles_d, tiles;
+  size_t lds;
+};
+
+constexpr int BWD_WGRAD_MAX_SLABS = 512;
+
+BwdWgradPlan bwd_wgrad_plan(const rsp_conv3d_desc* c, const rsp_pool3d_desc* d) {
+  BwdWgradPlan f;
+  memset(&f, 0, sizeof f);
+  if (!c || !rsp_conv_desc_ok(c) || !pool_ok(d, true) || !rsp_stem_applicable(c)) return f;
+  if (c->sT != 1 || c->sH != 1 || c->sW != 1 || c->Cout % 4 || c->out_ld % 4) return f;
+  if (c->kT * c->kH * c->kW * 4 > 128) return f;
+  if (d->N != c->N || d->Di != c->Do || d->Hi != c->Ho || d->Wi != c->Wo || d->C != c->Cout || d->in_ld != c->out_ld) return f;
+  if (d->out_ld % 4) return f;
+  const bool w1 = d->kT == 1 && d->kH == 1 && d->kW == 1, w4 = d->kT == 1 && d->kH == 2 && d->kW == 2,
+             w8 = d->kT == 2 && d->kH == 2 && d->kW == 2;
+  if (!(w1 || w4 || w8) || d->Di % d->kT || d->Hi % d->kH || d->Wi % d->kW) return f;
+  f.NW = w1 ? 1 : (w4 ? 4 : 8);
+  f.PT = w8 ? 2 : 1;
+  f.FT = f.PT + c->kT - 1; f.HT = 8 + c->kH - 1; f.WT = 16 + c->kW - 1;
+  f.npix = f.FT * f.HT * f.WT;
+  if (f.npix > 768) return f;
+  f.tiles_w = rsp_cdiv(d->Wi, 16); f.tiles_h = rsp_cdiv(d->Hi, 8); f.tiles_d = d->Di / f.PT;
+  const long long tiles = (long long)d->N * f.tiles_d * f.tiles_h * f.tiles_w;
+  if (tiles >= (1ll << 31) || (long long)d->N * d->Di * d->Hi * d->Wi >= (1ll << 31)) return f;
+  f.tiles = (int)tiles;
+  f.lds = ((size_t)128 * f.PT * 64 + (size_t)f.npix * 4) * sizeof(float);
+  f.ok = true;
+  return f;
+}
+
+template <int NW, int NB>
+int launch_bwd_wgrad(const BwdWgradParams& q, int grid, size_t lds, hipStream_t s) {
+  return rsp_launch_lds<&bn_bwd_wgrad_kernel<NW, NB>>(dim3((unsigned)grid), lds, 80 * 1024, s, std::tie(q), "bn_bwd_wgrad_kernel<%d, %d>", NW, NB);
+}
+
+}
+
+extern "C" {
+
+int rsp_bn_act_pool_bwd_wgrad_applicable(const rsp_conv3d_desc* c, const rsp_pool3d_desc* d) {
+  return (!rsp_conv_option(OPT_NO_FIRST_LAYER_FUSION) && bwd_wgrad_plan(c, d).ok) ? 1 : 0;
+}
+
+size_t rsp_bn_act_pool_bwd_wgrad_workspace(const rsp_conv3d_desc* c, const rsp_pool3d_desc* d) {
+  if (!bwd_wgrad_plan(c, d).ok) return 0;
+  return rsp_align_up(rsp_bn_bwd_workspace(d), 256) + (size_t)BWD_WGRAD_MAX_SLABS * 64 * 128 * sizeof(float);
+}
+
+int rsp_bn_act_pool_bwd_wgrad(const rsp_conv3d_desc* c, const rsp_pool3d_desc* d, const float* x, const float* y, const float* dout,
+                              const float* gamma, const float* mean_invstd, const float* scale_shift, int relu, float* dgamma,
+                              float* dbeta, int32_t c_valid, float* dw_ref, int32_t cout_valid, int32_t cin_valid, void* workspace,
+                              size_t workspace_bytes, void* stream) {
+  const BwdWgradPlan f = bwd_wgrad_plan(c, d);
+  RSP_REQUIRE(f.ok, "rsp_bn_act_pool_bwd_wgrad: geometry out of scope (rsp_bn_act_pool_bwd_wgrad_applicable)");
+  RSP_REQUIRE(x && y && dout && mean_invstd && scale_shift && dw_ref && workspace, "rsp_bn_act_pool_bwd_wgrad: null pointer");
+  RSP_REQUIRE(c_valid > 0 && c_valid <= d->C, "rsp_bn_act_pool_bwd_wgrad: bad valid channel count");
+  RSP_REQUIRE(cout_valid > 0 && cout_valid <= c->Cout && cin_valid > 0 && cin_valid <= c->Cin, "rsp_bn_act_pool_bwd_wgrad: bad valid channel counts");
+  RSP_REQUIRE(rsp_aligned16(x) && rsp_aligned16(y) && rsp_aligned16(dout) && rsp_aligned16(mean_invstd) && rsp_aligned16(scale_shift) &&
+              rsp_aligned16(workspace) && (!gamma || c_valid != d->C || rsp_aligned16(gamma)),
+              "rsp_bn_act_pool_bwd_wgrad: tensors must be 16-byte aligned");
+  if (workspace_bytes < rsp_bn_act_pool_bwd_wgrad_workspace(c, d)) {
+    rsp_set_error("rsp_bn_act_pool_bwd_wgrad: workspace too small");
+    return RSP_EWORKSPACE;
+  }
+  hipStream_t s = (hipStream_t)stream;
+  rsp_note_reset();
+  BwdLaunch b;
+  int rc = bn_bwd_sums(d, y, nullptr, dout, gamma, mean_invstd, scale_shift, relu, nullptr, nullptr, dgamma, dbeta, c_valid, nullptr,
+                       nullptr, workspace, s, "rsp_bn_act_pool_bwd_wgrad: more than 2^31 - 1 output positions", b);
+  if (rc != RSP_OK) return rc;
+  BwdWgradParams q;
+  memset(&q, 0, sizeof q);
+  q.b = b.p;
+  q.x = x;
+  q.partial = reinterpret_cast<float*>(reinterpret_cast<unsigned char*>(workspace) + rsp_align_up(rsp_bn_bwd_workspace(d), 256));
+  q.xD = c->Di; q.xH = c->Hi; q.xW = c->Wi;
+  q.kT = c->kT; q.kH = c->kH; q.kW = c->kW; q.pT = c->pT; q.pH = c->pH; q.pW = c->pW;
+  q.taps = c->kT * c->kH * c->kW;
+  q.K = cin_valid * q.taps;
+  const int NB = q.K <= 96 ? 3 : 4;
+  q.Kld = NB * 32;
+  q.FT = f.FT; q.HT = f.HT; q.WT = f.WT; q.npix = f.npix;
+  q.tiles_w = f.tiles_w; q.tiles_h = f.tiles_h; q.tiles_d = f.tiles_d; q.tiles = f.tiles;
+  const int grid = f.tiles < BWD_WGRAD_MAX_SLABS ? f.tiles : BWD_WGRAD_MAX_SLABS;
+  switch (f.NW * 10 + NB) {
+    case 13: rc = launch_bwd_wgrad<1, 3>(q, grid, f.lds, s); break;
+    case 14: rc = launch_bwd_wgrad<1, 4>(q, grid, f.lds, s); break;
+    case 43: rc = launch_bwd_wgrad<4, 3>(q, grid, f.lds, s); break;
+    case 44: rc = launch_bwd_wgrad<4, 4>(q, grid, f.lds, s); break;
+    case 83: rc = launch_bwd_wgrad<8, 3>(q, grid, f.lds, s); break;
+    default: rc = launch_bwd_wgrad<8, 4>(q, grid, f.lds, s); break;
+  }
+  if (rc != RSP_OK) return rc;
+  return rsp_wgrad_reduce_slabs(q.partial, dw_ref, grid, 64, q.Kld, q.K, cout_valid, s);
 }
 
 static int eval_bwd_mode(const rsp_pool3d_desc* d) {
diff --git a/rspnet_amd/csrc/common.h b/rspnet_amd/csrc/common.h
--- a/rspnet_amd/csrc/common.h
+++ b/rspnet_amd/csrc/common.h
@@ -39,7 +39,8 @@
   X(OPT_NO_PAD_SKIP, "no_pad_skip", "RSP_NO_PAD_SKIP", 1, 0)                            \
   X(OPT_NO_DMAJOR, "no_dmajor", "RSP_NO_DMAJOR", 1, 0)                                  \
   X(OPT_NO_TM_SKIP, "no_tm_skip", "RSP_NO_TM_SKIP", 1, 0)                               \
-  X(OPT_NO_MULTI_SPLIT, "no_multi_split", "RSP_NO_MULTI_SPLIT", 1, 0)
+  X(OPT_NO_MULTI_SPLIT, "no_multi_split", "RSP_NO_MULTI_SPLIT", 1, 0)                   \
+  X(OPT_NO_FIRST_LAYER_FUSION, "no_first_layer_fusion", "RSP_NO_FIRST_LAYER_FUSION", 1, 0)
 #define RSP_OPTION_ID(id, name, env, flag, dflt) id,
 enum RspConvOption { RSP_CONV_OPTIONS(RSP_OPTION_ID) RSP_OPT_COUNT };
 #undef RSP_OPTION_ID
diff --git a/rspnet_amd/csrc/conv_stem.h b/rspnet_amd/csrc/conv_stem.h
--- a/rspnet_amd/csrc/conv_stem.h
+++ b/rspnet_amd/csrc/conv_stem.h
@@ -13,3 +13,4 @@
 void rsp_stem_forget_packed(const void* w_packed);
 const char* rsp_wgrad_kernel_name(const rsp_conv3d_desc* d);
 double rsp_wgrad_executed_fraction(const rsp_conv3d_desc* d);
+int rsp_wgrad_reduce_slabs(const float* partial, float* dw, int slabs, int rows_ld, int Kld, int K, int cout_valid, hipStream_t s);
diff --git a/rspnet_amd/csrc/conv_wgrad.hip b/rspnet_amd/csrc/conv_wgrad.hip
--- a/rspnet_amd/csrc/conv_wgrad.hip
+++ b/rspnet_amd/csrc/conv_wgrad.hip
@@ -562,6 +562,31 @@
   __syncthreads();
   float* out = dw + ((long long)co * Cin_v + ci0) * taps;
   for (int e = threadIdx.x; e < nci * taps; e += 256) out[e] = wr_tile[e];
+}
+
+__global__ __launch_bounds__(256) void wgrad_reduce_slabs_kernel(const float* __restrict__ partial, float* __restrict__ dw, int slabs,
+                                                                 long long slab, int Kld, int K) {
+  __shared__ float red[8][32];
+  const int kx = threadIdx.x & 31, zl = threadIdx.x >> 5;
+  const int k = blockIdx.x * 32 + kx, co = blockIdx.y;
+  const float* src = partial + (long long)co * Kld + k;
+  float s0 = 0.f, s1 = 0.f, s2 = 0.f, s3 = 0.f;
+  int z = zl;
+  for (; z + 24 < slabs; z += 32) {
+    s0 += src[(long long)z * slab];
+    s1 += src[(long long)(z + 8) * slab];
+    s2 += src[(long long)(z + 16) * slab];
+    s3 += src[(long long)(z + 24) * slab];
+  }
+  for (; z < slabs; z += 8) s0 += src[(long long)z * slab];
+  red[zl][kx] = (s0 + s1) + (s2 + s3);
+  __syncthreads();
+  if (zl == 0 && k < K) {
+    float s = 0.f;
+#pragma unroll
+    for (int i = 0; i < 8; ++i) s += red[i][kx];
+    dw[(long long)co * K + k] = s;
+  }
 }
 
 __global__ __launch_bounds__(256) void colsum_stage1(const float* __restrict__ a, long long rows, int C, int ld,
@@ -739,6 +764,12 @@
 
 }
 
+int rsp_wgrad_reduce_slabs(const float* partial, float* dw, int slabs, int rows_ld, int Kld, int K, int cout_valid, hipStream_t s) {
+  hipLaunchKernelGGL(wgrad_reduce_slabs_kernel, dim3(Kld / 32, cout_valid), dim3(256), 0, s, partial, dw, slabs, (long long)rows_ld * Kld,
+                     Kld, K);
+  return rsp_check_launch("wgrad_reduce_slabs_kernel");
+}
+
 double rsp_wgrad_executed_fraction(const rsp_conv3d_desc* d0) {
   if (!wdesc_ok(d0)) return 1.0;
   const WSegs g = wgrad_segments(d0);
diff --git a/rspnet_amd/engine.py b/rspnet_amd/engine.py
--- a/rspnet_amd/engine.py
+++ b/rspnet_amd/engine.py
@@ -691,6 +691,17 @@
             return convbn_eval_bwd(node, sv, ni)
         else:
             dout = _view(dslots[node.into[0]], node.into, sv.cg.Cout) if node.into is not None else dslots.pop(node.dst)
+            if (node.src == plan.input_slot and not want_input_grad and node.residual is None and sv.res is None
+                    and not isinstance(key, tuple) and hasattr(be, "bn_act_pool_bwd_wgrad")
+                    and be.bn_act_pool_bwd_wgrad_applicable(sv.cg, sv.pg, sv.x, sv.y, dout)):
+                gw = grad_of(node.conv.weight)
+                if gw is not None:
+                    be.bn_act_pool_bwd_wgrad(sv.cg, sv.pg, sv.x, sv.y, dout, bn.weight.data, sv.mi, sv.ss, node.relu,
+                                             grad_of(bn.weight), grad_of(bn.bias), gw)
+                    return convbn_tail(node, sv, ni, None, None, True, gw)
+                dy, dres = be.bn_act_pool_bwd(sv.pg, sv.y, None, dout, bn.weight.data, sv.mi, sv.ss, node.relu, False,
+                                              grad_of(bn.weight), grad_of(bn.bias))
+                return convbn_tail(node, sv, ni, dy, dres, True, gw)
             dy, dres = be.bn_act_pool_bwd(sv.pg, sv.y, sv.res, dout, bn.weight.data, sv.mi, sv.ss, node.relu,
                                           node.residual is not None, grad_of(bn.weight), grad_of(bn.bias))
         convbn_tail(node, sv, ni, dy, dres, True)
@@ -709,7 +720,7 @@
             torch.mul(sv.ss[0][:gbias.shape[0]], sums, out=gbias)
         convbn_tail(node, sv, ni, dy, dres, False)
 
-    def convbn_tail(node, sv, ni, dy, dres, zero_bias):
+    def convbn_tail(node, sv, ni, dy, dres, zero_bias, *given_gw):
         if node.residual is not None:
             add_grad(node.residual, dres)
         bias = getattr(node.conv, "bias", None)
@@ -717,8 +728,10 @@
             gb = grad_of(bias)
             if gb is not None:
                 gb.zero_()
-        gw = grad_of(node.conv.weight)
-        if (sv.cg.flops < BranchStreams.SMALL_WGRAD_FLOPS or
+        gw = given_gw[0] if given_gw else grad_of(node.conv.weight)
+        if dy is None:
+            pass
+        elif (sv.cg.flops < BranchStreams.SMALL_WGRAD_FLOPS or
                 (sv.cg.flops < BranchStreams.MID_WGRAD_FLOPS and sv.cg.bytes < BranchStreams.MID_WGRAD_BYTES)):
             branches.side_task(lambda: be.conv_wgrad(sv.cg, sv.x, dy, gw), (sv.x, dy), cost=float(sv.cg.flops))
         else:
diff --git a/rspnet_amd/ops.py b/rspnet_amd/ops.py
--- a/rspnet_amd/ops.py
+++ b/rspnet_amd/ops.py
@@ -106,6 +106,15 @@
     d = pg.desc(in_ld=in_ld, out_ld=out_ld, res_ld=res_ld)
     ref = C.byref(d)
     return d, ref, lib.rsp_bn_bwd_workspace(ref), pg.out_dims
+
+
+@functools.lru_cache(maxsize=1024)
+def _first_block_plan(g: "ConvGeom", pg: "PoolGeom", y_ld, dout_ld):
+    lib = _lib.load()
+    cd = g.desc(out_ld=y_ld)
+    pd = pg.desc(in_ld=y_ld, out_ld=dout_ld)
+    ok = bool(lib.rsp_bn_act_pool_bwd_wgrad_applicable(C.byref(cd), C.byref(pd)))
+    return cd, pd, ok, int(lib.rsp_bn_act_pool_bwd_wgrad_workspace(C.byref(cd), C.byref(pd))) if ok else 0
 
 
 def _ptr(t: Optional[torch.Tensor]):
@@ -208,6 +217,7 @@
             _lib.check(prev, "rsp_conv3d_set_option")
         _conv_plan.cache_clear()
         executed_fraction.cache_clear()
+        _first_block_plan.cache_clear()
         return prev
 
     @contextlib.contextmanager
@@ -405,6 +415,31 @@
         n_in = y.numel()
         self._log_hbm("bn_bwd(reduce+apply)", 4 * (2 * (n_in * (1 if residual is None else 2) + dout.numel()) + n_in * (2 if want_dres else 1)), e0)
         return dy, dres
+
+    def bn_act_pool_bwd_wgrad_applicable(self, g: ConvGeom, pg: PoolGeom, x, y, dout) -> bool:
+        if not (x.is_contiguous() and x.data_ptr() % 16 == 0 and y.data_ptr() % 16 == 0 and dout.data_ptr() % 16 == 0):
+            return False
+        return _first_block_plan(g, pg, _rows_ld(y, "y"), _rows_ld(dout, "dout"))[2]
+
+    def bn_act_pool_bwd_wgrad(self, g: ConvGeom, pg: PoolGeom, x, y, dout, gamma, mean_invstd, scale_shift, relu: bool,
+                              dgamma_out, dbeta_out, dw_out: torch.Tensor):
+        _chk(x, "x")
+        _chk(dw_out, "dw_out")
+        if dw_out.shape[0] > g.Cout or dw_out.shape[1] > g.Cin:
+            raise _lib.RspError("bn_act_pool_bwd_wgrad: dw_out has more channels than the geometry")
+        cd, pd, ok, wsb = _first_block_plan(g, pg, _rows_ld(y, "y"), _rows_ld(dout, "dout"))
+        ws = self._workspace(y.device, max(wsb, 256))
+        c_valid = pg.C if gamma is None else int(gamma.shape[0])
+        e0 = self._ev()
+        _lib.check(self.lib.rsp_bn_act_pool_bwd_wgrad(C.byref(cd), C.byref(pd), _ptr(x), _ptr(y), _ptr(dout), _ptr(gamma),
+                                                      _ptr(mean_invstd), _ptr(scale_shift), int(relu), _ptr(dgamma_out),
+                                                      _ptr(dbeta_out), c_valid, _ptr(dw_out), dw_out.shape[0], dw_out.shape[1],
+                                                      _ptr(ws), wsb, _stream()), "rsp_bn_act_pool_bwd_wgrad")
+        nw = pg.k[0] * pg.k[1] * pg.k[2]
+        nb = 3 if dw_out.shape[1] * g.k[0] * g.k[1] * g.k[2] <= 96 else 4
+        self._log("conv_wgrad", g, e0, f"bn_bwd_wgrad_kernel<{nw}, {nb}>")
+        n_in = pg.N * pg.Di * pg.Hi * pg.Wi * pg.C
+        self._log_hbm("bn_bwd(reduce+wgrad)", 4 * (2 * (n_in + dout.numel()) + x.numel()), e0)
 
     def bn_eval_act_pool_bwd(self, pg: PoolGeom, y, residual, dout, mean_invstd, scale_shift, relu: bool, want_dres: bool,
                              dgamma_out, dbeta_out, dy_out=None):
```
